# sandyresearch/chipmunk

Hardware: AMD Instinct MI355X
Metric: DiT denoise steps/sec at fixed sparsity (higher is better)
Workload: dtype bf16

## Files before the change

### chipmunk_amd/_native.py

```python
from __future__ import annotations

import ctypes
import os

_HERE = os.path.dirname(os.path.abspath(__file__))
LIB_PATH = os.environ.get("CHIPMUNK_HIP_LIB") or os.path.join(_HERE, "lib", "libchipmunk_hip.so")

SYMBOLS = [
    "chipmunk_last_error", "chipmunk_abi_version", "chipmunk_set_option", "chipmunk_set_random_seed",
    "chipmunk_csp_attn", "chipmunk_csp_attn_out", "chipmunk_csp_128_attn", "chipmunk_dense_attn", "chipmunk_dense_colsum_attn",
    "chipmunk_csp_mlp_mm1", "chipmunk_csp_mlp_mm1_scatter", "chipmunk_csp_mlp_mm1_fp8", "chipmunk_csp_mlp_mm2_and_scatter_add", "chipmunk_csp_scatter_add", "chipmunk_csp_mlp_mm2",
    "chipmunk_csp_mlp_mm1_ragged", "chipmunk_csp_mlp_mm1_scatter_ragged", "chipmunk_csp_mlp_mm1_fp8_ragged", "chipmunk_csp_mlp_mm2_ragged",
    "chipmunk_csp_mlp_mm2_and_scatter_add_ragged", "chipmunk_csp_scatter_add_ragged", "chipmunk_block_mean_ragged", "chipmunk_transpose16_pitched",
    "chipmunk_csp_mlp_mm1_batched", "chipmunk_csp_mlp_mm1_scatter_batched", "chipmunk_csp_mlp_mm1_fp8_batched", "chipmunk_csp_mlp_mm2_batched",
    "chipmunk_csp_mlp_mm2_and_scatter_add_batched", "chipmunk_csp_scatter_add_batched",
    "chipmunk_csp_mlp_mm1_glu", "chipmunk_csp_mlp_mm1_glu_batched", "chipmunk_csp_mlp_mm1_glu_fp8", "chipmunk_csp_mlp_mm1_glu_fp8_batched",
    "chipmunk_csp_mlp_mm1_act", "chipmunk_csp_mlp_mm1_act_batched", "chipmunk_csp_mlp_mm1_fp8_act", "chipmunk_csp_mlp_mm1_fp8_act_batched",
    "chipmunk_csp_mlp_mm2_w8", "chipmunk_csp_mlp_mm2_w8_batched",
    "chipmunk_csp_mlp_mm1_fp8_act_rs", "chipmunk_csp_mlp_mm1_fp8_act_rs_batched", "chipmunk_quantize_fp8_rowwise",
    "chipmunk_topk_indices", "chipmunk_topk_delta_indices", "chipmunk_topk_indices_p", "chipmunk_topk_delta_indices_p", "chipmunk_topk_mask", "chipmunk_topk_mask_p", "chipmunk_dense_colsum_topk_mask_p_strided", "chipmunk_mask_to_indices", "chipmunk_mask_to_sorted_indices", "chipmunk_packed_mask_to_indices", "chipmunk_mask_row_counts", "chipmunk_mask_to_ragged_indices", "chipmunk_copy_indices",
    "chipmunk_bitpack", "chipmunk_bitunpack", "chipmunk_transpose16", "chipmunk_block_mean", "chipmunk_quantize_fp8", "chipmunk_gather_rows", "chipmunk_qkv_split_norm", "chipmunk_split_heads_rownorm", "chipmunk_dense_colsum_topk_mask", "chipmunk_dense_attn_strided", "chipmunk_csp_attn_out_ragged", "chipmunk_compact_indices", "chipmunk_residual_ln_modulate", "chipmunk_dense_colsum_attn_strided", "chipmunk_dense_colsum_topk_mask_strided", "chipmunk_release_scratch", "chipmunk_big_scratch_fallbacks",
    "chipmunk_dense_attn_varlen", "chipmunk_dense_colsum_attn_varlen", "chipmunk_dense_colsum_topk_mask_varlen",
    "chipmunk_dense_colsum_topk_mask_p_varlen", "chipmunk_topk_mask_varlen", "chipmunk_topk_mask_p_varlen",
    "chipmunk_host_alloc", "chipmunk_host_free", "chipmunk_copy_d2h_async", "chipmunk_copy_h2d_async", "chipmunk_host_bytes",
]

_lib = None


def lib() -> ctypes.CDLL:
    global _lib
    if _lib is None:
        if not os.path.exists(LIB_PATH):
            raise ImportError(
                f"{LIB_PATH} is missing: build it with `python -m chipmunk_amd.build` (hipcc --offload-arch=gfx950). "
                "chipmunk_amd has no CPU fallback.")
        _lib = ctypes.CDLL(LIB_PATH)
        _lib.chipmunk_last_error.restype = ctypes.c_char_p
        _lib.chipmunk_abi_version.restype = ctypes.c_int
        for item in filter(None, os.environ.get("CHIPMUNK_AMD_OPTIONS", "").split(",")):
            name, _, val = item.partition("=")
            if _lib.chipmunk_set_option(name.strip().encode(), int(val)) != 0:
                raise ValueError(f"CHIPMUNK_AMD_OPTIONS: {_lib.chipmunk_last_error().decode()}")
    return _lib


def last_error() -> str:
    return lib().chipmunk_last_error().decode()


def check(rc: int, what: str) -> None:
    if rc != 0:
        raise RuntimeError(f"{what}: {last_error()}")


def set_option(name: str, value: int) -> None:
    check(lib().chipmunk_set_option(name.encode(), int(value)), "chipmunk_set_option")


def manual_seed(seed: int) -> None:
    check(lib().chipmunk_set_random_seed(ctypes.c_uint64(int(seed) & 0xFFFFFFFFFFFFFFFF)), "chipmunk_set_random_seed")


class HostBuffer:

    def __init__(self, numel: int, dtype) -> None:
        import torch
        self.dtype = dtype
        self._numel = int(numel)
        self._itemsize = torch.empty(0, dtype=dtype).element_size()
        self.nbytes = self._numel * self._itemsize
        p = ctypes.c_void_p()
        check(lib().chipmunk_host_alloc(ctypes.c_size_t(max(self.nbytes, 1)), ctypes.byref(p)), "chipmunk_host_alloc")
        self.ptr = p.value

    def numel(self) -> int:
# ... 35 lines not shown
```

### chipmunk_amd/csrc/attn.hip

```cpp
#include "common.h"
#include "attn_params.h"
#include <type_traits>

namespace {

constexpr int QG = 192;
constexpr int QW = 48;
constexpr int KVT = 32;
constexpr int NST = 4;
constexpr int KRING = 8;
constexpr int HD = 128;
constexpr int TILE_BYTES = KVT * HD * 2;
constexpr float SCALE_LOG2E = 0.08838834764f * 1.44269504089f;
constexpr int NSTV = NST + 1;
constexpr int KEY_RING_OFF = (NST + NSTV) * TILE_BYTES;
constexpr int CS_OFF = KEY_RING_OFF + KRING * 256;
constexpr int ATTN_LDS_BYTES = CS_OFF + 2 * 2 * 4 * KVT * 4;

__device__ __forceinline__ f32x4 mfma16(bf16x8 a, bf16x8 b, f32x4 c) {
    return __builtin_amdgcn_mfma_f32_16x16x32_bf16(a, b, c, 0, 0, 0);
}

#ifdef ATTN_PROF
__device__ unsigned long long g_attn_prof[8 * 8];
// ... 1197 lines not shown
                for (int b = 0; b < B; ++b)
                    for (int h0 = 0; h0 < H; h0 += hc) {
                        AttnParams c = p;
                        const int hn = H - h0 < hc ? H - h0 : hc;
                        const int64_t bh0 = (int64_t)b * H + h0;
                        c.q += b * p.qs[0] + h0 * p.qs[1], c.k += b * p.ks[0] + h0 * p.ks[1], c.v += b * p.vs[0] + h0 * p.vs[1];
                        c.o += b * p.os[0] + h0 * p.os[1];
                        c.l_out += bh0 * Nq, c.p_in += bh0 * Nq, c.cs += bh0 * p.G * (int64_t)cs_stride;
                        c.B = 1, c.H = hn;
                        if (c.klens) c.klens += b;
                        if (int e = chipmunk_dense64_colsum_launch(c, part, st)) return e;
                    }
                return CHIPMUNK_OK;
            }
        }
        rc = chipmunk_dense64_launch(q, k, v, o, l, p.qs, p.ks, p.vs, p.os, B, H, Nq, Nk, st, klens);
    } else {
        rc = launch_attn<false, false, true>(p, st);
    }
    if (rc != CHIPMUNK_OK) return rc;
    if (use_colsum64(B, H, Nq, Nk)) return chipmunk_colsum64_launch(p, st);
    return launch_attn<false, false, false, true>(p, st);
}

extern "C" int chipmunk_dense_colsum_attn_strided(const void *q, const void *k, const void *v, const int64_t q_strides[3],
                                                  const int64_t k_strides[3], const int64_t v_strides[3], const float *pin,
                                                  void *o, const int64_t *o_strides, void *cs, float *l, int B, int H, int Nq,
                                                  int Nk, int cs_stride, void *stream) {
    return dense_colsum_attn_impl(q, k, v, q_strides, k_strides, v_strides, pin, o, o_strides, cs, l, nullptr, B, H, Nq, Nk, cs_stride,
                                  stream);
}

extern "C" int chipmunk_dense_colsum_attn_varlen(const void *q, const void *k, const void *v, const int64_t q_strides[3],
                                                 const int64_t k_strides[3], const int64_t v_strides[3], const float *pin,
                                                 void *o, const int64_t *o_strides, void *cs, float *l, const int32_t *k_lens, int B,
                                                 int H, int Nq, int Nk, int cs_stride, void *stream) {
    return dense_colsum_attn_impl(q, k, v, q_strides, k_strides, v_strides, pin, o, o_strides, cs, l, k_lens, B, H, Nq, Nk, cs_stride,
                                  stream);
}

extern "C" int chipmunk_dense_colsum_attn(const void *q, const void *k, const void *v, const int64_t q_strides[3],
                                          const int64_t k_strides[3], const int64_t v_strides[3], const float *pin,
                                          void *o, void *cs, float *l, int B, int H, int Nq, int Nk, int cs_stride,
                                          void *stream) {
    return chipmunk_dense_colsum_attn_strided(q, k, v, q_strides, k_strides, v_strides, pin, o, nullptr, cs, l, B, H, Nq, Nk,
                                              cs_stride, stream);
}

static int dense_colsum_topk_mask_impl(const void *q, const void *k, const void *v, const int64_t q_strides[3],
                                       const int64_t k_strides[3], const int64_t v_strides[3], const float *pin, void *o,
                                       const int64_t *o_strides, float *l, int B, int H, int Nq, int Nk, const void *static_mask,
                                       int64_t static_stride, int static_rows, const void *group_flags, void *mask,
                                       int topk, double random_amount, bool mass, double top_p, int k_min, void *stream,
                                       const int32_t *klens = nullptr) {
    if (int e = check_common(q, k, v, o, B, H, Nq, Nk)) return e;
    CM_CHECK(l && pin && mask, "dense_colsum_topk_mask: p / l / mask missing");
    if (int e = check_strides(q_strides, "q")) return e;
    if (int e = check_strides(k_strides, "k")) return e;
    if (int e = check_strides(v_strides, "v")) return e;
    hipStream_t st = (hipStream_t)stream;
    if (!use_dense64(B, H, Nq, Nk) || chipmunk_get_option("attn_fused_colsum") == 2 || (Nk & 3) || Nk > CHIPMUNK_TOPK_MASK_MAX_N)
        return CHIPMUNK_ERR_UNSUPPORTED;
    AttnParams p = {};
    p.q = (const uint16_t *)q, p.k = (const uint16_t *)k, p.v = (const uint16_t *)v, p.o = (uint16_t *)o;
    for (int i = 0; i < 3; ++i) p.qs[i] = q_strides[i], p.ks[i] = k_strides[i], p.vs[i] = v_strides[i];
    CM_CHECK((int64_t)Nk * p.ks[2] * 2 < (1ll << 32) && (int64_t)Nk * p.vs[2] * 2 < (1ll << 32),
             "attention: one head's K or V spans more than 4 GiB (32-bit DMA offsets)");
    if (int e = output_strides(p.os, o_strides, H, Nq)) return e;
    p.l_out = l, p.p_in = pin, p.cs = nullptr, p.cs_stride = 0, p.klens = klens;
    p.B = B, p.H = H, p.Nq = Nq, p.Nk = Nk, p.G = (Nq + QG - 1) / QG;
    p.o_scale = 1.f;
    uint16_t *part = (uint16_t *)chipmunk_big_scratch(st, chipmunk_colsum_part_bytes(B, H, Nq, Nk));
    if (!part) return CHIPMUNK_ERR_UNSUPPORTED;
    if (int e = chipmunk_dense64_colsum_launch(p, part, st)) return e;
    const int nrb = ((Nq + 255) / 256) * 2;
    if (mass)
        return chipmunk_topk_mask_p_parts(part, chipmunk_colsum_part_stride(Nk), nrb, p.G, Nq, static_mask, static_stride, static_rows, group_flags, mask,
                                          B * H * p.G, Nk, topk, top_p, k_min, random_amount, st, klens, H * p.G);
    return chipmunk_topk_mask_parts(part, chipmunk_colsum_part_stride(Nk), nrb, p.G, Nq, static_mask, static_stride, static_rows, group_flags, mask, B * H * p.G, Nk,
                                    topk, random_amount, st, klens, H * p.G);
}

extern "C" int chipmunk_dense_colsum_topk_mask_strided(const void *q, const void *k, const void *v, const int64_t q_strides[3],
                                               const int64_t k_strides[3], const int64_t v_strides[3], const float *pin, void *o,
                                               const int64_t *o_strides, float *l, int B, int H, int Nq, int Nk, const void *static_mask,
                                               int64_t static_stride, int static_rows, const void *group_flags, void *mask,
                                               int topk, double random_amount, void *stream) {
    return dense_colsum_topk_mask_impl(q, k, v, q_strides, k_strides, v_strides, pin, o, o_strides, l, B, H, Nq, Nk, static_mask, static_stride,
                                       static_rows, group_flags, mask, topk, random_amount, false, 0.0, 0, stream);
}

extern "C" int chipmunk_dense_colsum_topk_mask_p_strided(const void *q, const void *k, const void *v, const int64_t q_strides[3],
                                                 const int64_t k_strides[3], const int64_t v_strides[3], const float *pin, void *o,
                                                 const int64_t *o_strides, float *l, int B, int H, int Nq, int Nk, const void *static_mask,
                                                 int64_t static_stride, int static_rows, const void *group_flags, void *mask,
                                                 int topk, double random_amount, double top_p, int k_min, void *stream) {
    CM_CHECK(top_p > 0.0 && top_p <= 1.0, "dense_colsum_topk_mask_p: top_p must be in (0, 1] (got %g)", top_p);
    CM_CHECK(k_min >= 0, "dense_colsum_topk_mask_p: k_min must be >= 0 (got %d)", k_min);
    return dense_colsum_topk_mask_impl(q, k, v, q_strides, k_strides, v_strides, pin, o, o_strides, l, B, H, Nq, Nk, static_mask, static_stride,
                                       static_rows, group_flags, mask, topk, random_amount, true, top_p, k_min, stream);
}

extern "C" int chipmunk_dense_colsum_topk_mask(const void *q, const void *k, const void *v, const int64_t q_strides[3],
                                               const int64_t k_strides[3], const int64_t v_strides[3], const float *pin, void *o,
                                               float *l, int B, int H, int Nq, int Nk, const void *static_mask,
                                               int64_t static_stride, int static_rows, const void *group_flags, void *mask,
                                               int topk, double random_amount, void *stream) {
    return chipmunk_dense_colsum_topk_mask_strided(q, k, v, q_strides, k_strides, v_strides, pin, o, nullptr, l, B, H, Nq, Nk,
                                                   static_mask, static_stride, static_rows, group_flags, mask, topk, random_amount,
                                                   stream);
}

extern "C" int chipmunk_dense_colsum_topk_mask_varlen(const void *q, const void *k, const void *v, const int64_t q_strides[3],
                                                      const int64_t k_strides[3], const int64_t v_strides[3], const float *pin, void *o,
                                                      const int64_t *o_strides, float *l, const int32_t *k_lens, int B, int H, int Nq,
                                                      int Nk, const void *static_mask, int64_t static_stride, int static_rows,
                                                      const void *group_flags, void *mask, int topk, double random_amount, void *stream) {
    return dense_colsum_topk_mask_impl(q, k, v, q_strides, k_strides, v_strides, pin, o, o_strides, l, B, H, Nq, Nk, static_mask, static_stride,
                                       static_rows, group_flags, mask, topk, random_amount, false, 0.0, 0, stream, k_lens);
}

extern "C" int chipmunk_dense_colsum_topk_mask_p_varlen(const void *q, const void *k, const void *v, const int64_t q_strides[3],
                                                        const int64_t k_strides[3], const int64_t v_strides[3], const float *pin, void *o,
                                                        const int64_t *o_strides, float *l, const int32_t *k_lens, int B, int H, int Nq,
                                                        int Nk, const void *static_mask, int64_t static_stride, int static_rows,
                                                        const void *group_flags, void *mask, int topk, double random_amount, double top_p,
                                                        int k_min, void *stream) {
    CM_CHECK(top_p > 0.0 && top_p <= 1.0, "dense_colsum_topk_mask_p: top_p must be in (0, 1] (got %g)", top_p);
    CM_CHECK(k_min >= 0, "dense_colsum_topk_mask_p: k_min must be >= 0 (got %d)", k_min);
    return dense_colsum_topk_mask_impl(q, k, v, q_strides, k_strides, v_strides, pin, o, o_strides, l, B, H, Nq, Nk, static_mask, static_stride,
                                       static_rows, group_flags, mask, topk, random_amount, true, top_p, k_min, stream, k_lens);
}
```

### chipmunk_amd/csrc/attn_params.h

```cpp
#pragma once
#include <stdint.h>
#include <hip/hip_runtime.h>

struct AttnParams {
    const uint16_t *q, *k, *v;
    uint16_t *o;
    const uint16_t *o_in;
    int64_t qs[3], ks[3], vs[3], os[3];
    const int32_t *indices, *counts;
    const int64_t *idx_off;
    float *l_out;
    const float *p_in;
    uint16_t *cs;
    int cs_stride;
    int B, H, Nq, Nk, G, idx_stride;
    float o_scale;
    int split_full, nsplit;
    float *ws;
    int32_t *tickets;
    const int32_t *plan;
    int xcd_chunks;
    const float *kmax;
    uint16_t *cs_part;
    int cs_pstride;
    int probe;
    const int32_t *klens;
};

__device__ __forceinline__ int item_nk(const int32_t *klens, int b, int Nk) {
    if (!klens) return Nk;
    const int n = klens[b];
    return n < 1 ? 1 : (n < Nk ? n : Nk);
}


int chipmunk_csp64_launch(const AttnParams &p, int inplace, int grid, hipStream_t stream);
int chipmunk_dense64_colsum_launch(const AttnParams &p, uint16_t *part, hipStream_t stream);
int chipmunk_topk_mask_parts(const uint16_t *part, int part_stride, int nrb, int groups_per_bh, int Nq, const void *static_mask, int64_t static_stride,
                             int static_rows, const void *group_flags, void *mask, int rows, int n, int k, double random_amount,
                             hipStream_t stream, const int32_t *klens = nullptr, int seq_rows = 0);
int chipmunk_topk_mask_p_parts(const uint16_t *part, int part_stride, int nrb, int groups_per_bh, int Nq, const void *static_mask, int64_t static_stride,
                               int static_rows, const void *group_flags, void *mask, int rows, int n, int k, double top_p, int k_min,
                               double random_amount, hipStream_t stream, const int32_t *klens = nullptr, int seq_rows = 0);
size_t chipmunk_colsum_part_bytes(int B, int H, int Nq, int Nk);
int chipmunk_colsum_part_stride(int Nk);
int chipmunk_colsum64_launch(const AttnParams &p, hipStream_t stream);
int chipmunk_csp96_launch(const AttnParams &p, int inplace, int grid, hipStream_t stream);
const float *chipmunk_knorm_max(const uint16_t *k, const int64_t ks[3], int B, int H, int Nk, hipStream_t stream, const int32_t *klens = nullptr);

__host__ __device__ inline int colsum_part_rows(int j, int nwg, int &r0, int &r1) {
    const int a = (3 * j) >> 2, w0 = 3 * j - 4 * a;
    r0 = 2 * a + (w0 ? 1 : 0);
    r1 = 2 * (a + 1);
    return (w0 >= 2 && a + 1 < nwg) ? 2 : 1;
}

struct IndexRow {
    const int32_t *ptr;
    int width;
};
__device__ __forceinline__ IndexRow index_row(const AttnParams &p, int64_t item) {
    if (p.idx_off) {
        const int64_t o = p.idx_off[item];
        return {p.indices + o, (int)(p.idx_off[item + 1] - o)};
    }
    return {p.indices + item * p.idx_stride, p.idx_stride};
}
```

### chipmunk_amd/csrc/common.h

```cpp
#pragma once
#include <hip/hip_runtime.h>
#include <stdint.h>
#include <stdio.h>
#include <stdarg.h>

#include "../../include/chipmunk_hip.h"

typedef __attribute__((ext_vector_type(8))) __bf16 bf16x8;
typedef __attribute__((ext_vector_type(4))) __bf16 bf16x4;
typedef __attribute__((ext_vector_type(2))) __bf16 bf16x2;
typedef __attribute__((ext_vector_type(4))) short s16x4;
typedef __attribute__((ext_vector_type(2))) float f32x2;
typedef __attribute__((ext_vector_type(4))) float f32x4;
typedef __attribute__((ext_vector_type(16))) float f32x16;
typedef __attribute__((ext_vector_type(4))) uint32_t u32x4;
typedef __attribute__((ext_vector_type(2))) uint32_t u32x2;

#define LDS_PTR(p) ((__attribute__((address_space(3))) void *)(p))
#define GLB_PTR(p) ((const __attribute__((address_space(1))) void *)(p))

__device__ __forceinline__ void glds16(const void *gsrc, void *lds_wave_base) {
    __builtin_amdgcn_global_load_lds(GLB_PTR(gsrc), LDS_PTR(lds_wave_base), 16, 0, 0);
}

// ... 54 lines not shown

__device__ __forceinline__ void lane_swap32(float &a, float &b) {
    asm volatile("s_nop 1\n\tv_permlane32_swap_b32 %0, %1" : "+v"(a), "+v"(b));
}
__device__ __forceinline__ void lane_swap16(float &a, float &b) {
    asm volatile("s_nop 1\n\tv_permlane16_swap_b32 %0, %1" : "+v"(a), "+v"(b));
}
__device__ __forceinline__ float max_across_rows(float x) {
    float a = x, b = x;
    lane_swap32(a, b);
    float c = fmaxf(a, b), d = c;
    lane_swap16(c, d);
    return fmaxf(c, d);
}
__device__ __forceinline__ float sum_across_rows(float x) {
    float a = x, b = x;
    lane_swap32(a, b);
    float c = a + b, d = c;
    lane_swap16(c, d);
    return c + d;
}

__device__ __forceinline__ int xcd_remap(int bid, int nblocks) {
    const int NX = 8;
    int xcd = bid % NX, slot = bid / NX;
    int q = nblocks / NX, r = nblocks % NX;
    int base = xcd < r ? xcd * (q + 1) : r * (q + 1) + (xcd - r) * q;
    return base + slot;
}

inline int device_cu_count() {
    static int n = 0;
    if (n == 0) {
        int dev = 0, v = 0;
        if (hipGetDevice(&dev) == hipSuccess &&
            hipDeviceGetAttribute(&v, hipDeviceAttributeMultiprocessorCount, dev) == hipSuccess && v > 0)
            n = v;
        else
            n = 256;
    }
    return n;
}

inline void ensure_dynamic_lds(const void *kernel, int bytes, uint64_t &done) {
    int dev = 0;
    if (hipGetDevice(&dev) != hipSuccess || dev < 0 || dev > 63) dev = 0;
    if (!(done >> dev & 1)) {
        (void)hipFuncSetAttribute(kernel, hipFuncAttributeMaxDynamicSharedMemorySize, bytes);
        done |= uint64_t(1) << dev;
    }
}

#define CHIPMUNK_TOPK_MASK_MAX_N (1024 * 512)

void chipmunk_set_error(const char *fmt, ...);
int chipmunk_get_option(const char *name);
uint32_t chipmunk_next_random_salt();
void *chipmunk_scratch(hipStream_t stream, size_t bytes);
void *chipmunk_big_scratch(hipStream_t stream, size_t bytes);
int chipmunk_dense64_launch(const void *q, const void *k, const void *v, void *o, float *l, const int64_t qs[3],
                            const int64_t ks[3], const int64_t vs[3], const int64_t os[3], int B, int H, int Nq, int Nk,
                            hipStream_t stream, const int32_t *klens = nullptr);
#define CM_CHECK(cond, ...)                    \
    do {                                       \
        if (!(cond)) {                         \
            chipmunk_set_error(__VA_ARGS__);   \
            return CHIPMUNK_ERR_INVALID;       \
        }                                      \
    } while (0)
#define CM_LAUNCH_CHECK()                                                          \
    do {                                                                           \
        hipError_t e__ = hipGetLastError();                                        \
        if (e__ != hipSuccess) {                                                   \
            chipmunk_set_error("HIP launch failed: %s", hipGetErrorString(e__));   \
            return CHIPMUNK_ERR_LAUNCH;                                            \
        }                                                                          \
    } while (0)
```

### chipmunk_amd/csrc/indexed_io.hip

```cpp
#include "common.h"
#include "attn_params.h"

namespace {

__device__ __forceinline__ uint32_t wave_incl_scan(uint32_t x) {
    x += (uint32_t)__builtin_amdgcn_update_dpp(0, (int)x, 0x111, 0xf, 0xf, true);
    x += (uint32_t)__builtin_amdgcn_update_dpp(0, (int)x, 0x112, 0xf, 0xf, true);
    x += (uint32_t)__builtin_amdgcn_update_dpp(0, (int)x, 0x114, 0xf, 0xf, true);
    x += (uint32_t)__builtin_amdgcn_update_dpp(0, (int)x, 0x118, 0xf, 0xf, true);
    x += (uint32_t)__builtin_amdgcn_update_dpp(0, (int)x, 0x142, 0xa, 0xf, false);
    x += (uint32_t)__builtin_amdgcn_update_dpp(0, (int)x, 0x143, 0xc, 0xf, false);
    return x;
}
struct M2IParams {
    const uint8_t *mask;
    int32_t *indices;
    int32_t *counts;
    int n, pad_n, multiple_of;
    const int64_t *offsets;
};

template <bool PACKED, bool SORTED = false, bool RAGGED = false>
__global__ __launch_bounds__(256) void mask_to_indices_kernel(const M2IParams p) {
    extern __shared__ __attribute__((aligned(16))) unsigned char smem[];
// ... 170 lines not shown
        for (int i = 0; i < NI && pos < padded; ++i) {
            uint32_t z = ~bits[i];
            const int rem = n - i * 32;
            if (rem < 32) z &= (1u << rem) - 1u;
            while (z && pos < padded) {
                const int bit = __builtin_ctz(z);
                z &= z - 1;
                put(pos++, i * 32 + bit);
            }
        }
        if constexpr (!RAGGED) p.counts[row] = padded;
    }
}

struct RowCountParams {
    const uint8_t *mask;
    int32_t *counts;
    int64_t *lengths;
    int64_t rows;
    int n, pad_n, multiple_of;
};

template <bool PACKED>
__global__ __launch_bounds__(256) void mask_row_counts_kernel(const RowCountParams p) {
    const int lane = threadIdx.x & 63;
    const int64_t row = (int64_t)blockIdx.x * 4 + (threadIdx.x >> 6);
    if (row >= p.rows) return;
    const int nbytes = PACKED ? p.n >> 3 : p.n;
    const uint8_t *src = p.mask + (PACKED ? (row * p.n) >> 3 : row * p.n);
    auto set_in_byte = [](uint32_t b) { return PACKED ? (uint32_t)__popc(b) : (uint32_t)(b != 0); };
    auto set_in_word = [](uint32_t x) {
        if constexpr (!PACKED) x = (x | (x >> 1) | (x >> 2) | (x >> 3) | (x >> 4) | (x >> 5) | (x >> 6) | (x >> 7)) & 0x01010101u;
        return (uint32_t)__popc(x);
    };
    const int head = min(nbytes, (int)((16 - ((uintptr_t)src & 15)) & 15));
    uint32_t cnt = lane < head ? set_in_byte(src[lane]) : 0u;
    const int nvec = (nbytes - head) >> 4;
    const u32x4 *vec = (const u32x4 *)(src + head);
#pragma unroll 4
    for (int i = lane; i < nvec; i += 64) {
        const u32x4 x = vec[i];
        cnt += set_in_word(x[0]) + set_in_word(x[1]) + set_in_word(x[2]) + set_in_word(x[3]);
    }
    const int tail = head + (nvec << 4) + lane;
    if (tail < nbytes) cnt += set_in_byte(src[tail]);
    const int64_t kept = (uint32_t)__builtin_amdgcn_readlane((int)wave_incl_scan(cnt), 63);
    if (lane == 0) {
        const int64_t padded = ((kept + p.multiple_of - 1) / p.multiple_of) * p.multiple_of;
        p.counts[row] = (int32_t)padded;
        p.lengths[row] = (min(padded, (int64_t)p.pad_n) + 31) / 32 * 32;
    }
}

struct TopkParams {
    const void *act;
    void *cache;
    int32_t *indices;
    int32_t *counts;
    int rows, cols, multiple_of;
    float quantile, random_amount;
    uint32_t salt;
};

template <typename T>
__device__ __forceinline__ float load_as_float(const T *p, int i);
template <>
__device__ __forceinline__ float load_as_float<uint16_t>(const uint16_t *p, int i) { return bf16_bits_to_f32(p[i]); }
template <>
__device__ __forceinline__ float load_as_float<_Float16>(const _Float16 *p, int i) { return (float)p[i]; }
template <>
__device__ __forceinline__ float load_as_float<float>(const float *p, int i) { return p[i]; }

template <typename T>
__device__ __forceinline__ float round_to(float x);
template <>
__device__ __forceinline__ float round_to<uint16_t>(float x) { return round_bf16(x); }
template <>
__device__ __forceinline__ float round_to<_Float16>(float x) { return (float)(_Float16)x; }
template <>
__device__ __forceinline__ float round_to<float>(float x) { return x; }

__device__ __forceinline__ float hash_uniform(uint32_t row, uint32_t col, uint32_t salt) {
    uint32_t x = (row * 0x9E3779B9u ^ (col + 0x7F4A7C15u) * 0x85EBCA6Bu) + salt * 0xC2B2AE35u;
    x ^= x >> 16, x *= 0x7feb352du, x ^= x >> 15, x *= 0x846ca68bu, x ^= x >> 16;
    return (float)(x >> 8) * (1.0f / 16777216.0f);
}

__device__ __forceinline__ int compact_slot(bool keep, int lane, int w, uint32_t *wave_tot, int &base) {
    const unsigned long long bal = __ballot(keep);
    const int before = __popcll(bal & ((1ull << lane) - 1ull));
    if (lane == 0) wave_tot[w] = __popcll(bal);
    __syncthreads();
    int off = base, tot = 0;
#pragma unroll
    for (int i = 0; i < 16; ++i) {
        const int c = wave_tot[i];
        off += i < w ? c : 0;
        tot += c;
    }
    __syncthreads();
    base += tot;
    return keep ? off + before : -1;
}

struct TopkPParams : TopkParams {
    float top_p;
// ... 281 lines not shown
    c = c < idx_stride ? c : (int)idx_stride;
    if ((((uintptr_t)src | (uintptr_t)dst) & 15) == 0) {
        const int c4 = c >> 2;
        for (int i = threadIdx.x; i < c4; i += 256) ((u32x4 *)dst)[i] = ((const u32x4 *)src)[i];
        for (int i = (c4 << 2) + threadIdx.x; i < c; i += 256) dst[i] = src[i];
    } else {
        for (int i = threadIdx.x; i < c; i += 256) dst[i] = src[i];
    }
    for (int i = c + threadIdx.x; i < width; i += 256) dst[i] = 0;
}

size_t m2i_lds_bytes(int n, bool sorted) {
    const int NI = (n + 31) >> 5, NB = (NI + 63) >> 6;
    if (sorted) return (size_t)NB * 64 * 4 + (size_t)(NB + 1) * 4 + 16;
    return (size_t)NB * 64 * 4 + (size_t)32 * NB * 8 + (size_t)32 * NB * 4 + 33 * 4 + 16;
}

template <bool PACKED, bool SORTED = false, bool RAGGED = false>
int launch_m2i(const void *mask, int32_t *indices, int32_t *counts, int64_t rows, int n, int pad_n, int multiple_of,
               void *stream, const int64_t *offsets = nullptr) {
    CM_CHECK(mask && indices && (RAGGED ? (const void *)offsets : (const void *)counts), "mask_to_indices: null pointer");
    CM_CHECK(rows >= 0 && n > 0 && pad_n >= n && multiple_of > 0, "mask_to_indices: bad sizes rows=%lld n=%d pad_n=%d multiple_of=%d",
             (long long)rows, n, pad_n, multiple_of);
    CM_CHECK(rows < (1ll << 31), "mask_to_indices: too many rows");
    if (PACKED) CM_CHECK(n % 8 == 0, "packed_mask_to_indices: n must be a multiple of 8 (got %d)", n);
    const size_t lds = m2i_lds_bytes(n, SORTED);
    CM_CHECK(lds <= 160 * 1024, "mask_to_indices: row length %d needs %zu B of LDS (> 160 KiB)", n, lds);
    if (rows == 0) return CHIPMUNK_OK;
    auto kern = mask_to_indices_kernel<PACKED, SORTED, RAGGED>;
    if (lds > 64 * 1024) (void)hipFuncSetAttribute((const void *)kern, hipFuncAttributeMaxDynamicSharedMemorySize, (int)lds);
    M2IParams p = {(const uint8_t *)mask, indices, counts, n, pad_n, multiple_of, offsets};
    hipLaunchKernelGGL(kern, dim3((unsigned)rows), dim3(256), lds, (hipStream_t)stream, p);
    CM_LAUNCH_CHECK();
    return CHIPMUNK_OK;
}


struct TopkMaskParams {
    const uint16_t *cs;
    const uint8_t *stat;
    const uint8_t *groups;
    uint8_t *mask;
    int64_t cs_stride, stat_stride;
    int rows, n, k, stat_rows;
    float random_amount;
    uint32_t salt;
    const uint16_t *parts;
    int64_t pstride;
    int nrb, ngroups, nq;
    float top_p;
    int k_min;
    const int32_t *klens;
    int seq_rows;
};

__device__ __forceinline__ int topk_mask_row_len(const TopkMaskParams &p, int row) {
    if (!p.klens) return p.n;
    const int v = p.klens[row / p.seq_rows];
    return v < 1 ? 1 : (v < p.n ? v : p.n);
}
struct RowCut {
    int tid, step;
    uint32_t keep0, keep1;
};
__device__ __forceinline__ RowCut row_cut(int nv) {
    const int rem = nv & 3;
    RowCut c;
    c.tid = rem ? ((nv - 1) >> 2) & 1023 : -1;
    c.step = (nv - 1) >> 12;
    c.keep0 = rem == 1 ? 0xffffu : 0xffffffffu;
    c.keep1 = rem == 3 ? 0xffffu : (rem ? 0u : 0xffffffffu);
    return c;
}

__device__ __forceinline__ float key_value(uint32_t key) { return __uint_as_float((key ^ 0x8000u) << 16); }
__device__ __forceinline__ void add_mass2(float &m, uint32_t kw, float flo) {
    const uint32_t kx = kw ^ 0x80008000u;
    const float a = __uint_as_float(kx << 16), b = __uint_as_float(kx & 0xffff0000u);
    m += a >= flo ? a : 0.f;
    m += b >= flo ? b : 0.f;
}

__device__ __forceinline__ int topp_count(float total, float target, float above, int gt, int eq, uint32_t thr, int k, int k_min) {
    int kp = 0;
    if (total > 0.f && target > 0.f) {
        const float v = key_value(thr);
        float t = __builtin_ceilf((target - above) / v);
        t = t >= 1.f ? t : 1.f;
        kp = gt + (t < (float)eq ? (int)t : eq);
    }
    const int s = kp > k_min ? kp : k_min;
    return s < k ? s : k;
}

__device__ __forceinline__ uint32_t bf16_key(uint32_t u) {
    return (u & 0x8000u) ? (~u & 0xffffu) : (u | 0x8000u);
}

template <int KPT, bool ALIGNED, bool PARTS = false, bool MASS = false>
__global__ __launch_bounds__(1024) void topk_mask_kernel(const TopkMaskParams p) {
    constexpr int NV = KPT / 4;
    __shared__ int wave_cnt[16];
    const int tid = threadIdx.x, lane = tid & 63, w = tid >> 6;
    const int row = blockIdx.x;
    const int n = p.n;
    const int nv = topk_mask_row_len(p, row);
    const uint16_t *x = nullptr;
    int prow = 1;
    int64_t row1 = 0;
    if constexpr (PARTS) {
        const int bh = row / p.ngroups, g = row - bh * p.ngroups;
        int r0, r1;
        prow = colsum_part_rows(g, p.nrb / 2, r0, r1);
        x = p.parts + ((int64_t)bh * p.nrb + r0) * p.pstride;
        row1 = (int64_t)(r1 - r0) * p.pstride;
    } else {
        x = p.cs + (int64_t)row * p.cs_stride;
    }
    const uint32_t lane_off8 = 8u * (uint32_t)tid;
    const uint32_t lane_off4 = 4u * (uint32_t)tid;
    uint32_t key[NV][2];
    constexpr int LB = NV % 10 == 0 ? 10 : (NV % 8 == 0 ? 8 : (NV % 6 == 0 ? 6 : 4));
    static_assert(NV % LB == 0, "NV must split into whole load batches");
#pragma unroll
    for (int j0 = 0; j0 < NV; j0 += LB) {
        uint32_t raw[LB][2];
#pragma unroll
        for (int jj = 0; jj < LB; ++jj) {
            const int c = 4 * tid + 4096 * (j0 + jj);
            uint32_t v0 = 0xffffffffu, v1 = 0xffffffffu;
            if constexpr (ALIGNED) {
                if (c < nv) {
                    const u32x2 v = *(const u32x2 *)((const unsigned char *)(x + 4096 * (j0 + jj)) + lane_off8);
                    v0 = v[0], v1 = v[1];
                    if constexpr (PARTS) {
                        if (prow == 2) {
                            float a0 = __uint_as_float(v0 << 16), a1 = __uint_as_float(v0 & 0xffff0000u);
                            float a2 = __uint_as_float(v1 << 16), a3 = __uint_as_float(v1 & 0xffff0000u);
                            const u32x2 y = *(const u32x2 *)((const unsigned char *)(x + row1 + 4096 * (j0 + jj)) + lane_off8);
                            a0 += __uint_as_float(y[0] << 16), a1 += __uint_as_float(y[0] & 0xffff0000u);
                            a2 += __uint_as_float(y[1] << 16), a3 += __uint_as_float(y[1] & 0xffff0000u);
                            v0 = pack_bf16x2(a0, a1), v1 = pack_bf16x2(a2, a3);
                        }
                    }
                }
            } else if (c < nv) {
                v0 = v1 = 0;
#pragma unroll
                for (int e = 0; e < 4; ++e) {
                    const uint32_t u = c + e < nv ? x[c + e] : 0xffffu;
                    if (e < 2) v0 |= u << (16 * e);
                    else v1 |= u << (16 * (e - 2));
                }
// ... 127 lines not shown
    }
    int my_ties = 0;
    if (ties_to_take > 0) {
#pragma unroll
        for (int j = 0; j < NV; ++j)
#pragma unroll
            for (int h = 0; h < 2; ++h) {
                uint32_t kw = key[j][h];
                asm volatile("" : "+v"(kw));
                my_ties += ((kw & 0xffffu) == thr ? 1 : 0) + ((kw >> 16) == thr ? 1 : 0);
            }
    }
    int tie_budget = 0;
    {
        int incl = my_ties;
#pragma unroll
        for (int d = 1; d < 64; d <<= 1) {
            const int o = __shfl_up(incl, d);
            if (lane >= d) incl += o;
        }
        if (lane == 63) wave_cnt[w] = incl;
        __syncthreads();
        int before = incl - my_ties;
#pragma unroll
        for (int i = 0; i < 16; ++i) before += i < w ? wave_cnt[i] : 0;
        __syncthreads();
        tie_budget = ties_to_take - before;
    }
    uint8_t *out = p.mask + (int64_t)row * n;
    const uint8_t *st = p.stat ? p.stat + (int64_t)(row % p.stat_rows) * p.stat_stride : nullptr;
    const bool rnd = active && p.random_amount > 0.f;
    auto combined4 = [&](int c0, uint32_t &v0, uint32_t &v1) {
        const u32x2 v = *(const u32x2 *)(x + c0);
        v0 = v[0], v1 = v[1];
        if constexpr (PARTS) {
            float a0 = __uint_as_float(v0 << 16), a1 = __uint_as_float(v0 & 0xffff0000u);
            float a2 = __uint_as_float(v1 << 16), a3 = __uint_as_float(v1 & 0xffff0000u);
            if (prow == 2) {
                const u32x2 y = *(const u32x2 *)(x + row1 + c0);
                a0 += __uint_as_float(y[0] << 16), a1 += __uint_as_float(y[0] & 0xffff0000u);
                a2 += __uint_as_float(y[1] << 16), a3 += __uint_as_float(y[1] & 0xffff0000u);
            }
            v0 = pack_bf16x2(a0, a1), v1 = pack_bf16x2(a2, a3);
        }
    };
    uint32_t first = x[0];
    if constexpr (PARTS) {
        uint32_t f0, f1;
        combined4(0, f0, f1);
        first = f0 & 0xffffu;
    }
    const uint32_t salt = p.salt ^ (first * 0x27D4EB2Fu);
    const int nsteps = (n + 4095) / 4096;
    auto emit = [&](auto keyed, int c, uint32_t v0, uint32_t v1, uint32_t sb) {
        uint32_t bytes = 0;
        if constexpr (decltype(keyed)::value) asm volatile("" : "+v"(v0), "+v"(v1));
#pragma unroll
        for (int e = 0; e < 4; ++e) {
            const uint32_t half = ((e < 2 ? v0 : v1) >> (16 * (e & 1))) & 0xffffu;
            const uint32_t kv = decltype(keyed)::value ? half : bf16_key(half);
            bool keep = kv > thr;
            const bool tie = kv == thr && tie_budget > 0 && c + e < nv;
            tie_budget -= tie ? 1 : 0;
            keep = keep || tie;
            if (rnd && !keep) keep = hash_uniform(row, c + e, salt) < p.random_amount;
            keep = keep || ((sb >> (8 * e)) & 0xffu) != 0;
            keep = keep && c + e < nv;
            bytes |= (keep ? 1u : 0u) << (8 * e);
        }
        if constexpr (ALIGNED) {
            *(uint32_t *)(out + c) = bytes;
        } else {
#pragma unroll
            for (int e = 0; e < 4; ++e)
                if (c + e < n) out[c + e] = (uint8_t)(bytes >> (8 * e));
        }
    };
    if constexpr (ALIGNED) {
        constexpr int OB = 5;
#pragma unroll
        for (int j0 = 0; j0 < NV; j0 += OB) {
            uint32_t sbv[OB];
#pragma unroll
            for (int jj = 0; jj < OB; ++jj) {
                const int c = 4 * tid + 4096 * (j0 + jj);
                sbv[jj] = (j0 + jj < NV && st && c < n) ? *(const uint32_t *)(st + c) : 0u;
            }
            __builtin_amdgcn_sched_barrier(0);
#pragma unroll
            for (int jj = 0; jj < OB; ++jj) {
                if constexpr (true) {
                    const int c = 4 * tid + 4096 * (j0 + jj);
                    if (j0 + jj < NV && c < n) emit(std::integral_constant<int, 1>{}, c, key[(j0 + jj) < NV ? (j0 + jj) : 0][0], key[(j0 + jj) < NV ? (j0 + jj) : 0][1], sbv[jj]);
                    asm volatile("" ::: "memory");
                }
            }
            __builtin_amdgcn_sched_barrier(0);
        }
    } else {
        for (int j = 0; j < nsteps; ++j) {
            const int c = 4 * tid + 4096 * j;
            if (c >= n) break;
            uint32_t v0 = 0, v1 = 0, sb = 0;
#pragma unroll
            for (int e = 0; e < 4; ++e) {
                const uint32_t u = c + e < nv ? x[c + e] : 0xffffu;
                if (e < 2) v0 |= u << (16 * e);
                else v1 |= u << (16 * (e - 2));
                if (st && c + e < n) sb |= (uint32_t)st[c + e] << (8 * e);
            }
            emit(std::integral_constant<int, 0>{}, c, v0, v1, sb);
        }
    }
}

__device__ __forceinline__ uint32_t bf16_key2(uint32_t u) {
    uint32_t s;
    const uint32_t fifteen2 = 0x000f000fu;
    asm("v_pk_ashrrev_i16 %0, %1, %2" : "=v"(s) : "v"(fifteen2), "v"(u));
    return u ^ (s | 0x80008000u);
}

template <bool ALIGNED, bool PARTS, bool MASS = false>
__global__ __launch_bounds__(1024) void topk_mask_stream_kernel(const TopkMaskParams p) {
    __shared__ int wave_cnt[16];
    const int tid = threadIdx.x, lane = tid & 63, w = tid >> 6;
    const int row = blockIdx.x;
    const int n = p.n;
    const int nv = topk_mask_row_len(p, row);
    const uint16_t *x = nullptr;
    int prow = 1;
    int64_t row1 = 0;
    if constexpr (PARTS) {
        const int bh = row / p.ngroups, g = row - bh * p.ngroups;
        int r0, r1;
        prow = colsum_part_rows(g, p.nrb / 2, r0, r1);
        x = p.parts + ((int64_t)bh * p.nrb + r0) * p.pstride;
        row1 = (int64_t)(r1 - r0) * p.pstride;
    } else {
        x = p.cs + (int64_t)row * p.cs_stride;
    }
    const uint32_t lane_off8 = 8u * (uint32_t)tid;
    const int nsteps = (n + 4095) / 4096;
    const bool active = p.groups == nullptr || p.groups[row] != 0;
    int k = p.k < nv ? p.k : nv;
    const RowCut rc = row_cut(nv);
    const int cut_step = ALIGNED && tid == rc.tid ? rc.step : -1;
    bool select = active && k > 0;
    const bool rnd = active && p.random_amount > 0.f;

    auto combined4 = [&](int c0, uint32_t &v0, uint32_t &v1) {
        const u32x2 v = *(const u32x2 *)(x + c0);
        v0 = v[0], v1 = v[1];
        if constexpr (PARTS) {
            if (prow == 2) {
                float a0 = __uint_as_float(v0 << 16), a1 = __uint_as_float(v0 & 0xffff0000u);
                float a2 = __uint_as_float(v1 << 16), a3 = __uint_as_float(v1 & 0xffff0000u);
                const u32x2 y = *(const u32x2 *)(x + row1 + c0);
                a0 += __uint_as_float(y[0] << 16), a1 += __uint_as_float(y[0] & 0xffff0000u);
                a2 += __uint_as_float(y[1] << 16), a3 += __uint_as_float(y[1] & 0xffff0000u);
                v0 = pack_bf16x2(a0, a1), v1 = pack_bf16x2(a2, a3);
            }
        }
    };
    uint32_t first = 0;
// ... 268 lines not shown
    CM_CHECK(sparsity_amount >= 0.0 && sparsity_amount <= 1.0, "%s: sparsity_amount must be in [0,1]", who);
    CM_CHECK(top_p > 0.0 && top_p <= 1.0, "%s: top_p must be in (0, 1] (got %g)", who, top_p);
    CM_CHECK(min_keys >= 0.0 && min_keys <= 1.0 - sparsity_amount + 1e-9, "%s: min_keys must be in [0, 1 - sparsity_amount] (got %g with sparsity_amount %g)",
             who, min_keys, sparsity_amount);
    if (rows == 0) return CHIPMUNK_OK;
    TopkPParams p;
    p.act = activation, p.cache = cache, p.indices = indices, p.counts = counts;
    p.rows = rows, p.cols = cols, p.multiple_of = multiple_of;
    p.quantile = (float)sparsity_amount, p.random_amount = (float)random_amount;
    p.salt = random_amount > 0.0 ? chipmunk_next_random_salt() : 0u;
    p.top_p = (float)top_p;
    p.k_min = min_keys == 0.0 ? 1024 : std::max((int)(1024 * (float)(1.0 - min_keys)), (int)(1024 * p.quantile));
    hipStream_t s = (hipStream_t)stream;
#define LAUNCH_TOPK_P(T)                                                                                         \
    do {                                                                                                         \
        if (cache) hipLaunchKernelGGL((topk_indices_kernel<T, true, true>), dim3(rows), dim3(1024), 0, s, p);    \
        else hipLaunchKernelGGL((topk_indices_kernel<T, false, true>), dim3(rows), dim3(1024), 0, s, p);         \
    } while (0)
    switch (dtype) {
        case CHIPMUNK_DTYPE_BF16: LAUNCH_TOPK_P(uint16_t); break;
        case CHIPMUNK_DTYPE_FP16: LAUNCH_TOPK_P(_Float16); break;
        case CHIPMUNK_DTYPE_FP32: LAUNCH_TOPK_P(float); break;
        default: CM_CHECK(false, "%s: unsupported dtype code %d", who, dtype);
    }
#undef LAUNCH_TOPK_P
    CM_LAUNCH_CHECK();
    return CHIPMUNK_OK;
}

extern "C" int chipmunk_mask_to_sorted_indices(const void *mask, int packed, int32_t *indices, int32_t *counts,
                                               int64_t rows, int n, int pad_n, int multiple_of, void *stream) {
    return packed ? launch_m2i<true, true>(mask, indices, counts, rows, n, pad_n, multiple_of, stream)
                  : launch_m2i<false, true>(mask, indices, counts, rows, n, pad_n, multiple_of, stream);
}

extern "C" int chipmunk_mask_row_counts(const void *mask, int packed, int32_t *counts, int64_t *lengths, int64_t rows, int n,
                                        int pad_n, int multiple_of, void *stream) {
    CM_CHECK(mask && counts && lengths, "mask_row_counts: null pointer");
    CM_CHECK(rows >= 0 && n > 0 && pad_n >= n && multiple_of > 0, "mask_row_counts: bad sizes rows=%lld n=%d pad_n=%d multiple_of=%d",
             (long long)rows, n, pad_n, multiple_of);
    CM_CHECK(rows < (1ll << 31), "mask_row_counts: too many rows");
    CM_CHECK(!packed || n % 8 == 0, "mask_row_counts: n must be a multiple of 8 for a packed mask (got %d)", n);
    const size_t lds = m2i_lds_bytes(n, true);
    CM_CHECK(lds <= 160 * 1024, "mask_to_indices: row length %d needs %zu B of LDS (> 160 KiB)", n, lds);
    if (rows == 0) return CHIPMUNK_OK;
    RowCountParams p = {(const uint8_t *)mask, counts, lengths, rows, n, pad_n, multiple_of};
    const dim3 grid((unsigned)((rows + 3) / 4));
    if (packed) hipLaunchKernelGGL(mask_row_counts_kernel<true>, grid, dim3(256), 0, (hipStream_t)stream, p);
    else hipLaunchKernelGGL(mask_row_counts_kernel<false>, grid, dim3(256), 0, (hipStream_t)stream, p);
    CM_LAUNCH_CHECK();
    return CHIPMUNK_OK;
}

extern "C" int chipmunk_mask_to_ragged_indices(const void *mask, int packed, int sorted, const int64_t *offsets, int32_t *flat,
                                               int64_t rows, int n, int multiple_of, void *stream) {
    if (packed) return sorted ? launch_m2i<true, true, true>(mask, flat, nullptr, rows, n, n, multiple_of, stream, offsets)
                              : launch_m2i<true, false, true>(mask, flat, nullptr, rows, n, n, multiple_of, stream, offsets);
    return sorted ? launch_m2i<false, true, true>(mask, flat, nullptr, rows, n, n, multiple_of, stream, offsets)
                  : launch_m2i<false, false, true>(mask, flat, nullptr, rows, n, n, multiple_of, stream, offsets);
}

extern "C" int chipmunk_topk_indices(const void *activation, int dtype, int32_t *indices, int32_t *counts, int rows,
                                     int cols, double sparsity_amount, int multiple_of, double random_amount,
                                     void *stream) {
    return launch_topk(activation, nullptr, dtype, indices, counts, rows, cols, sparsity_amount, multiple_of,
                       random_amount, stream);
}

extern "C" int chipmunk_topk_delta_indices(const void *activation, void *cache, int dtype, int32_t *indices,
                                           int32_t *counts, int rows, int cols, double sparsity_amount,
                                           int multiple_of, double random_amount, void *stream) {
    CM_CHECK(cache != nullptr, "topk_delta_indices: cache missing");
    return launch_topk(activation, cache, dtype, indices, counts, rows, cols, sparsity_amount, multiple_of,
                       random_amount, stream);
}

extern "C" int chipmunk_topk_indices_p(const void *activation, int dtype, int32_t *indices, int32_t *counts, int rows, int cols,
                                       double sparsity_amount, double top_p, double min_keys, int multiple_of,
                                       double random_amount, void *stream) {
    return launch_topk_p("topk_indices_p", activation, nullptr, dtype, indices, counts, rows, cols, sparsity_amount, top_p, min_keys,
                         multiple_of, random_amount, stream);
}

extern "C" int chipmunk_topk_delta_indices_p(const void *activation, void *cache, int dtype, int32_t *indices, int32_t *counts,
                                             int rows, int cols, double sparsity_amount, double top_p, double min_keys,
                                             int multiple_of, double random_amount, void *stream) {
    CM_CHECK(cache != nullptr, "topk_delta_indices_p: cache missing");
    return launch_topk_p("topk_delta_indices_p", activation, cache, dtype, indices, counts, rows, cols, sparsity_amount, top_p,
                         min_keys, multiple_of, random_amount, stream);
}

extern "C" int chipmunk_copy_indices(const void *src, void *dst, const int32_t *inds, const int32_t *counts, int B,
                                     int M, int R, int F, int elem_size, void *stream) {
    CM_CHECK(src && dst && inds && counts, "copy_indices: null pointer");
    CM_CHECK(B >= 0 && M > 0 && R > 0 && F > 0, "copy_indices: bad sizes");
    CM_CHECK(elem_size == 2 || elem_size == 4, "copy_indices: element size must be 2 or 4 bytes (got %d)", elem_size);
    const int64_t rows = (int64_t)B * M * R;
    if (rows == 0) return CHIPMUNK_OK;
    CM_CHECK(rows < (1ll << 31), "copy_indices: too many rows");
    hipStream_t s = (hipStream_t)stream;
    if (elem_size == 2)
        hipLaunchKernelGGL(copy_indices_kernel<uint16_t>, dim3((unsigned)rows), dim3(256), 0, s, (const uint16_t *)src,
                           (uint16_t *)dst, inds, counts, M, R, F);
    else
        hipLaunchKernelGGL(copy_indices_kernel<uint32_t>, dim3((unsigned)rows), dim3(256), 0, s, (const uint32_t *)src,
                           (uint32_t *)dst, inds, counts, M, R, F);
// ... 61 lines not shown
#define LAUNCH_GATHER(V)                                                                                              \
    do {                                                                                                              \
        const int64_t cpr = row_bytes / (int64_t)sizeof(V), total = outer * n_out * cpr;                               \
        const int64_t blocks = (total + 255) / 256;                                                                    \
        hipLaunchKernelGGL((gather_rows_kernel<V>), dim3((unsigned)(blocks > 65536 * 16 ? 65536 * 16 : blocks)),       \
                           dim3(256), 0, s, (const V *)src, (V *)dst, map, n_out, n_src, cpr, total);                  \
    } while (0)
    if ((align & 15) == 0) LAUNCH_GATHER(u32x4);
    else if ((align & 3) == 0) LAUNCH_GATHER(uint32_t);
    else if ((align & 1) == 0) LAUNCH_GATHER(uint16_t);
    else LAUNCH_GATHER(uint8_t);
#undef LAUNCH_GATHER
    CM_LAUNCH_CHECK();
    return CHIPMUNK_OK;
}

template <bool MASS>
static int topk_mask_parts_impl(const uint16_t *part, int part_stride, int nrb, int groups_per_bh, int Nq, const void *static_mask, int64_t static_stride,
                                int static_rows, const void *group_flags, void *mask, int rows, int n, int k, double random_amount,
                                double top_p, int k_min, hipStream_t s, const int32_t *klens, int seq_rows) {
    CM_CHECK(!klens || seq_rows > 0, "topk_mask_parts: k_lens without the rows per sequence");
    CM_CHECK(part && mask && rows >= 0 && n > 0 && (n & 3) == 0 && n <= CHIPMUNK_TOPK_MASK_MAX_N && k >= 0 && part_stride >= n && (part_stride & 3) == 0, "topk_mask_parts: bad arguments");
    CM_CHECK(!static_mask || (static_rows > 0 && static_stride >= n && (static_stride & 3) == 0 && ((uintptr_t)static_mask & 3) == 0),
             "topk_mask_parts: bad static mask geometry");
    CM_CHECK(((uintptr_t)mask & 3) == 0 && ((uintptr_t)part & 7) == 0, "topk_mask_parts: unaligned buffers");
    if (rows == 0) return CHIPMUNK_OK;
    TopkMaskParams p = {nullptr, (const uint8_t *)static_mask, (const uint8_t *)group_flags, (uint8_t *)mask, 0, static_stride,
                        rows, n, k, static_mask ? static_rows : 1, (float)random_amount,
                        random_amount > 0.0 ? chipmunk_next_random_salt() : 0u};
    p.parts = part, p.pstride = part_stride, p.nrb = nrb, p.ngroups = groups_per_bh, p.nq = Nq;
    p.top_p = (float)top_p, p.k_min = k_min;
    p.klens = klens, p.seq_rows = seq_rows;
    if (n > 1024 * 120 || chipmunk_get_option("topk_mask_stream") == 1) hipLaunchKernelGGL((topk_mask_stream_kernel<true, true, MASS>), dim3(rows), dim3(1024), 0, s, p);
    else if (n <= 1024 * 16) hipLaunchKernelGGL((topk_mask_kernel<16, true, true, MASS>), dim3(rows), dim3(1024), 0, s, p);
    else if (n <= 1024 * 48) hipLaunchKernelGGL((topk_mask_kernel<48, true, true, MASS>), dim3(rows), dim3(1024), 0, s, p);
    else hipLaunchKernelGGL((topk_mask_kernel<120, true, true, MASS>), dim3(rows), dim3(1024), 0, s, p);
    CM_LAUNCH_CHECK();
    return CHIPMUNK_OK;
}

int chipmunk_topk_mask_parts(const uint16_t *part, int part_stride, int nrb, int groups_per_bh, int Nq, const void *static_mask, int64_t static_stride,
                             int static_rows, const void *group_flags, void *mask, int rows, int n, int k, double random_amount,
                             hipStream_t s, const int32_t *klens, int seq_rows) {
    return topk_mask_parts_impl<false>(part, part_stride, nrb, groups_per_bh, Nq, static_mask, static_stride, static_rows, group_flags, mask, rows, n, k,
                                       random_amount, 0.0, 0, s, klens, seq_rows);
}

int chipmunk_topk_mask_p_parts(const uint16_t *part, int part_stride, int nrb, int groups_per_bh, int Nq, const void *static_mask, int64_t static_stride,
                               int static_rows, const void *group_flags, void *mask, int rows, int n, int k, double top_p, int k_min,
                               double random_amount, hipStream_t s, const int32_t *klens, int seq_rows) {
    CM_CHECK(top_p > 0.0 && top_p <= 1.0 && k_min >= 0, "topk_mask_p_parts: top_p must be in (0, 1] and k_min >= 0 (got %g, %d)", top_p, k_min);
    return topk_mask_parts_impl<true>(part, part_stride, nrb, groups_per_bh, Nq, static_mask, static_stride, static_rows, group_flags, mask, rows, n, k,
                                      random_amount, top_p, k_min, s, klens, seq_rows);
}

__global__ __launch_bounds__(256) void qkv_split_norm_kernel(const uint16_t *qkv, int64_t row_stride, const uint16_t *qw,
                                                             const uint16_t *kw, uint16_t *q, uint16_t *k, uint16_t *v, int64_t n,
                                                             int H, float eps, int64_t segments, const float *fcos, const float *fsin,
                                                             int64_t rope_rows) {
    const int l15 = threadIdx.x & 15;
    u32x4 wq = {0x3f803f80u, 0x3f803f80u, 0x3f803f80u, 0x3f803f80u}, wk = wq;
    if (qw) wq = *(const u32x4 *)(qw + l15 * 8);
    if (kw) wk = *(const u32x4 *)(kw + l15 * 8);
    for (int64_t seg = ((int64_t)blockIdx.x * 256 + threadIdx.x) >> 4; seg < segments; seg += ((int64_t)gridDim.x * 256) >> 4) {
        const int64_t tok = seg / (3 * H);
        const int rem = (int)(seg - tok * 3 * H), which = rem / H, h = rem - which * H;
        u32x4 x = *(const u32x4 *)(qkv + tok * row_stride + (int64_t)rem * 128 + l15 * 8);
        uint16_t *dst = (which == 0 ? q : which == 1 ? k : v) + ((int64_t)h * n + tok) * 128 + l15 * 8;
        if (which < 2) {
            float f[8], ss = 0.f;
#pragma unroll
            for (int e = 0; e < 4; ++e) {
                f[2 * e] = __uint_as_float(x[e] << 16), f[2 * e + 1] = __uint_as_float(x[e] & 0xffff0000u);
                ss = __builtin_fmaf(f[2 * e], f[2 * e], ss);
                ss = __builtin_fmaf(f[2 * e + 1], f[2 * e + 1], ss);
            }
            ss = row16_sum(ss);
            const float r = 1.0f / __builtin_sqrtf(ss * (1.0f / 128.0f) + eps);
            const u32x4 w = which == 0 ? wq : wk;
#pragma unroll
            for (int e = 0; e < 4; ++e) {
                float a = f[2 * e] * r, b = f[2 * e + 1] * r;
                round_bf16_pair(a, b);
                x[e] = pack_bf16x2(a * __uint_as_float(w[e] << 16), b * __uint_as_float(w[e] & 0xffff0000u));
            }
            if (fcos && tok < rope_rows) {
                const f32x4 c0 = *(const f32x4 *)(fcos + tok * 128 + l15 * 8), c1 = *(const f32x4 *)(fcos + tok * 128 + l15 * 8 + 4);
                const f32x4 s0 = *(const f32x4 *)(fsin + tok * 128 + l15 * 8), s1 = *(const f32x4 *)(fsin + tok * 128 + l15 * 8 + 4);
#pragma unroll
                for (int e = 0; e < 4; ++e) {
                    const float re = __uint_as_float(x[e] << 16), im = __uint_as_float(x[e] & 0xffff0000u);
                    const float cr = e < 2 ? c0[2 * e] : c1[2 * e - 4], ci = e < 2 ? c0[2 * e + 1] : c1[2 * e - 3];
                    const float sr = e < 2 ? s0[2 * e] : s1[2 * e - 4], si = e < 2 ? s0[2 * e + 1] : s1[2 * e - 3];
                    x[e] = pack_bf16x2(re * cr + (-im) * sr, im * ci + re * si);
                }
            }
        }
        *(u32x4 *)dst = x;
    }
}

extern "C" int chipmunk_qkv_split_norm(const void *qkv, int64_t row_stride, const void *q_weight, const void *k_weight, void *q,
                                       void *k, void *v, int64_t n, int heads, float eps, const float *freqs_cos,
                                       const float *freqs_sin, int64_t rope_rows, void *stream) {
    CM_CHECK(qkv && q && k && v, "qkv_split_norm: null pointer");
    CM_CHECK(n >= 0 && heads > 0 && row_stride >= (int64_t)3 * heads * 128, "qkv_split_norm: bad sizes");
// ... 26 lines not shown
                        cs_stride, static_stride, rows, n, k, static_mask ? static_rows : 1, (float)random_amount,
                        random_amount > 0.0 ? chipmunk_next_random_salt() : 0u};
    p.top_p = (float)top_p, p.k_min = k_min;
    p.klens = klens, p.seq_rows = seq_rows;
    hipStream_t s = (hipStream_t)stream;
    const bool aligned = n % 4 == 0 && (((uintptr_t)cs) & 7) == 0 && (cs_stride * 2) % 8 == 0 && (((uintptr_t)mask) & 3) == 0 &&
                         (!static_mask || ((((uintptr_t)static_mask) & 3) == 0 && static_stride % 4 == 0));
#define LAUNCH_TM(KPT)                                                                                       \
    do {                                                                                                     \
        if (aligned) hipLaunchKernelGGL((topk_mask_kernel<KPT, true, false, MASS>), dim3(rows), dim3(1024), 0, s, p);     \
        else hipLaunchKernelGGL((topk_mask_kernel<KPT, false, false, MASS>), dim3(rows), dim3(1024), 0, s, p);            \
    } while (0)
    if (n > 1024 * 120 || chipmunk_get_option("topk_mask_stream") == 1) {
        if (aligned) hipLaunchKernelGGL((topk_mask_stream_kernel<true, false, MASS>), dim3(rows), dim3(1024), 0, s, p);
        else hipLaunchKernelGGL((topk_mask_stream_kernel<false, false, MASS>), dim3(rows), dim3(1024), 0, s, p);
    } else if (n <= 1024 * 16) LAUNCH_TM(16);
    else if (n <= 1024 * 48) LAUNCH_TM(48);
    else LAUNCH_TM(120);
#undef LAUNCH_TM
    CM_LAUNCH_CHECK();
    return CHIPMUNK_OK;
}

extern "C" int chipmunk_topk_mask(const void *cs, int64_t cs_stride, const void *static_mask, int64_t static_stride,
                                  int static_rows, const void *group_flags, void *mask, int rows, int n, int k,
                                  double random_amount, void *stream) {
    return topk_mask_impl<false>(cs, cs_stride, static_mask, static_stride, static_rows, group_flags, mask, rows, n, k, random_amount, 0.0, 0, stream);
}

extern "C" int chipmunk_topk_mask_p(const void *cs, int64_t cs_stride, const void *static_mask, int64_t static_stride,
                                    int static_rows, const void *group_flags, void *mask, int rows, int n, int k,
                                    double random_amount, double top_p, int k_min, void *stream) {
    CM_CHECK(top_p > 0.0 && top_p <= 1.0, "topk_mask_p: top_p must be in (0, 1] (got %g)", top_p);
    CM_CHECK(k_min >= 0, "topk_mask_p: k_min must be >= 0 (got %d)", k_min);
    return topk_mask_impl<true>(cs, cs_stride, static_mask, static_stride, static_rows, group_flags, mask, rows, n, k, random_amount, top_p, k_min, stream);
}

extern "C" int chipmunk_topk_mask_varlen(const void *cs, int64_t cs_stride, const void *static_mask, int64_t static_stride,
                                         int static_rows, const void *group_flags, void *mask, const int32_t *k_lens, int seq_rows, int rows,
                                         int n, int k, double random_amount, void *stream) {
    return topk_mask_impl<false>(cs, cs_stride, static_mask, static_stride, static_rows, group_flags, mask, rows, n, k, random_amount, 0.0, 0, stream,
                                 k_lens, seq_rows);
}

extern "C" int chipmunk_topk_mask_p_varlen(const void *cs, int64_t cs_stride, const void *static_mask, int64_t static_stride,
                                           int static_rows, const void *group_flags, void *mask, const int32_t *k_lens, int seq_rows, int rows,
                                           int n, int k, double random_amount, double top_p, int k_min, void *stream) {
    CM_CHECK(top_p > 0.0 && top_p <= 1.0, "topk_mask_p: top_p must be in (0, 1] (got %g)", top_p);
    CM_CHECK(k_min >= 0, "topk_mask_p: k_min must be >= 0 (got %d)", k_min);
    return topk_mask_impl<true>(cs, cs_stride, static_mask, static_stride, static_rows, group_flags, mask, rows, n, k, random_amount, top_p, k_min,
                                stream, k_lens, seq_rows);
}

extern "C" int chipmunk_compact_indices(const int32_t *indices, int64_t idx_stride, const int32_t *counts, const int64_t *offsets,
                                        int32_t *flat, int64_t rows, void *stream) {
    CM_CHECK(indices && counts && offsets && flat, "compact_indices: null pointer");
    CM_CHECK(rows >= 0 && rows < (1ll << 31) && idx_stride > 0, "compact_indices: bad sizes rows=%lld idx_stride=%lld", (long long)rows,
             (long long)idx_stride);
    if (rows == 0) return CHIPMUNK_OK;
    hipLaunchKernelGGL(compact_indices_kernel, dim3((unsigned)rows), dim3(256), 0, (hipStream_t)stream, indices, idx_stride, counts,
                       offsets, flat);
    CM_LAUNCH_CHECK();
    return CHIPMUNK_OK;
}
```

### chipmunk_amd/csrc/torch_registry.cpp

```cpp
#include <ATen/ATen.h>
#include <ATen/hip/impl/HIPStreamMasqueradingAsCUDA.h>
#include <Python.h>
#include <c10/core/DeviceGuard.h>
#include <torch/library.h>

#include <vector>

#include "../../include/chipmunk_hip.h"

extern "C" {
PyObject *PyInit_cuda(void) {
    static struct PyModuleDef module_def = {PyModuleDef_HEAD_INIT, "cuda", NULL, -1, NULL};
    return PyModule_Create(&module_def);
}
}

namespace chipmunk {
namespace {

void *cur_stream(const at::Tensor &t) {
    return (void *)c10::hip::getCurrentHIPStreamMasqueradingAsCUDA(t.device().index()).stream();
}
void check(int rc, const char *op) { TORCH_CHECK(rc == 0, "chipmunk::", op, ": ", chipmunk_last_error()); }

// ... 836 lines not shown
            check(chipmunk_block_mean_ragged(x[b].data_ptr(), out[b].data_ptr(), n, (int)x.size(2), (int)mbm, cur_stream(x)), "block_mean");
    }
    return out;
}

at::Tensor quantize_fp8(at::Tensor x, at::Tensor scale, double max_value) {
    CHECK_DEV(x); CHECK_DEV(scale);
    TORCH_CHECK(x.scalar_type() == at::kBFloat16, "quantize_fp8: x must be bfloat16");
    TORCH_CHECK(scale.scalar_type() == at::kFloat && scale.numel() == 1, "quantize_fp8: scale must be a one-element float32 tensor");
    TORCH_CHECK(x.numel() % 8 == 0, "quantize_fp8: the element count must be a multiple of 8");
    x = x.contiguous();
    c10::DeviceGuard guard(x.device());
    at::Tensor out = at::empty(x.sizes(), x.options().dtype(at::kFloat8_e4m3fn));
    check(chipmunk_quantize_fp8(x.data_ptr(), scale.data_ptr<float>(), out.data_ptr(), x.numel(), (float)max_value, cur_stream(x)), "quantize_fp8");
    return out;
}

std::vector<at::Tensor> quantize_fp8_rowwise(at::Tensor x, double max_value) {
    CHECK_DEV(x);
    TORCH_CHECK(x.scalar_type() == at::kBFloat16, "quantize_fp8_rowwise: x must be bfloat16");
    TORCH_CHECK(x.dim() >= 1 && x.size(-1) > 0 && x.size(-1) % 16 == 0 && x.size(-1) <= CHIPMUNK_QUANTIZE_ROWWISE_MAX_K,
                "quantize_fp8_rowwise: the last dimension must be a positive multiple of 16, at most ", CHIPMUNK_QUANTIZE_ROWWISE_MAX_K);
    x = x.contiguous();
    c10::DeviceGuard guard(x.device());
    const int64_t K = x.size(-1), rows = x.numel() / K;
    at::Tensor out = at::empty(x.sizes(), x.options().dtype(at::kFloat8_e4m3fn));
    at::Tensor recip = at::empty(x.sizes().slice(0, x.dim() - 1), x.options().dtype(at::kFloat));
    check(chipmunk_quantize_fp8_rowwise(x.data_ptr(), out.data_ptr(), recip.data_ptr<float>(), rows, (int)K, (float)max_value, cur_stream(x)),
          "quantize_fp8_rowwise");
    return {out, recip};
}

std::vector<at::Tensor> mask_to_sorted_indices(at::Tensor mask, at::IntArrayRef shape, int64_t multiple_of,
                                               int64_t pad_to_multiple_of) {
    CHECK_DEV(mask);
    const bool packed = mask.scalar_type() == at::kByte;
    TORCH_CHECK(packed || mask.scalar_type() == at::kBool, "mask must be bool, or uint8 bit-packed with a shape");
    mask = mask.contiguous();
    std::vector<int64_t> shp = packed ? shape.vec() : mask.sizes().vec();
    TORCH_CHECK(shp.size() == 4, "shape must be [b, h, m, n]");
    const int64_t b = shp[0], h = shp[1], m = shp[2], n = shp[3];
    if (packed) TORCH_CHECK(n % 8 == 0 && mask.numel() * 8 >= b * h * m * n, "bad packed mask");
    const int64_t pad_n = ((n + pad_to_multiple_of - 1) / pad_to_multiple_of) * pad_to_multiple_of;
    c10::DeviceGuard guard(mask.device());
    at::Tensor indices = at::empty({b, h, m, pad_n}, mask.options().dtype(at::kInt));
    at::Tensor counts = at::empty({b, h, m}, mask.options().dtype(at::kInt));
    check(chipmunk_mask_to_sorted_indices(mask.data_ptr(), packed ? 1 : 0, indices.data_ptr<int>(),
                                          counts.data_ptr<int>(), b * h * m, (int)n, (int)pad_n, (int)multiple_of,
                                          cur_stream(mask)),
          "mask_to_sorted_indices");
    return {indices, counts};
}

std::vector<at::Tensor> mask_to_ragged_indices(at::Tensor mask, at::IntArrayRef shape, int64_t multiple_of, int64_t pad_to_multiple_of,
                                               bool sorted) {
    CHECK_DEV(mask);
    const bool packed = mask.scalar_type() == at::kByte;
    TORCH_CHECK(packed || mask.scalar_type() == at::kBool, "mask must be bool, or uint8 bit-packed with a shape");
    TORCH_CHECK(multiple_of > 0 && pad_to_multiple_of > 0, "multiple_of and pad_to_multiple_of must be positive");
    mask = mask.contiguous();
    std::vector<int64_t> shp = packed ? shape.vec() : mask.sizes().vec();
    TORCH_CHECK(shp.size() == 4, "shape must be [b, h, m, n]");
    const int64_t b = shp[0], h = shp[1], m = shp[2], n = shp[3], rows = b * h * m;
    if (packed) TORCH_CHECK(n % 8 == 0 && mask.numel() * 8 >= rows * n, "bad packed mask");
    const int64_t pad_n = ((n + pad_to_multiple_of - 1) / pad_to_multiple_of) * pad_to_multiple_of;
    TORCH_CHECK(n > 0 && pad_n <= INT_MAX, "rows must have between 1 and 2^31 - 1 columns");
    c10::DeviceGuard guard(mask.device());
    at::Tensor counts = at::empty({b, h, m}, mask.options().dtype(at::kInt));
    at::Tensor len = at::empty({rows}, mask.options().dtype(at::kLong));
    check(chipmunk_mask_row_counts(mask.data_ptr(), packed ? 1 : 0, counts.data_ptr<int>(), len.data_ptr<int64_t>(), rows, (int)n,
                                   (int)pad_n, (int)multiple_of, cur_stream(mask)),
          "mask_to_ragged_indices");
    at::Tensor offsets = at::zeros({rows + 1}, len.options());
    if (rows) offsets.narrow(0, 1, rows).copy_(len.cumsum(0));
    const int64_t total = rows ? offsets[rows].item<int64_t>() : 0;
    at::Tensor flat = at::empty({total + 64}, counts.options());
    flat.narrow(0, total, 64).zero_();
    check(chipmunk_mask_to_ragged_indices(mask.data_ptr(), packed ? 1 : 0, sorted ? 1 : 0, offsets.data_ptr<int64_t>(), flat.data_ptr<int>(),
                                          rows, (int)n, (int)multiple_of, cur_stream(mask)),
          "mask_to_ragged_indices");
    return {flat, offsets, counts};
}

std::vector<at::Tensor> dense_colsum_attn_layout(at::Tensor q, at::Tensor k, at::Tensor v, at::Tensor p, bool token_major_o);
static at::Tensor topk_mask_impl(at::Tensor cs, int64_t k, bool mass, double top_p, int64_t k_min, double random_amount,
                                 const c10::optional<at::Tensor> &groups, const c10::optional<at::Tensor> &static_mask,
                                 const OptTensor &k_lens = c10::nullopt);
static std::vector<at::Tensor> dense_colsum_topk_mask_impl(at::Tensor q, at::Tensor k, at::Tensor v, at::Tensor p, int64_t k_top, bool mass, double top_p,
                                                           int64_t k_min, double random_amount, const c10::optional<at::Tensor> &groups,
                                                           const c10::optional<at::Tensor> &static_mask, bool token_major_o,
                                                           const OptTensor &k_lens = c10::nullopt) {
    const int32_t *kl = klens_ptr(k_lens, q, q.dim() == 4 ? q.size(0) : 0);
    if (mass) TORCH_CHECK(top_p > 0.0 && top_p <= 1.0 && k_min >= 0, "top_p must be in (0, 1] and k_min >= 0 (got ", top_p, ", ", k_min, ")");
    CHECK_DEV(q); CHECK_DEV(k); CHECK_DEV(v); CHECK_DEV(p);
    CHECK_BF16(q); CHECK_BF16(k); CHECK_BF16(v);
    const bool shapes_ok = q.dim() == 4 && k.dim() == 4 && v.dim() == 4 && q.size(3) == 128 && q.stride(3) == 1 && k.stride(3) == 1 &&
                           v.stride(3) == 1 && p.scalar_type() == at::kFloat && p.is_contiguous();
    if (shapes_ok) {
        const int64_t B = q.size(0), H = q.size(1), Nq = q.size(2), Nk = k.size(2), G = (Nq + 191) / 192;
        const void *st = nullptr, *gf = nullptr;
        int64_t st_stride = 0, st_rows = 1;
        at::Tensor stc, gfc;
        bool ok = p.numel() == B * H * Nq;
        if (ok && static_mask.has_value() && static_mask->defined()) {
            stc = *static_mask;
            ok = stc.is_cuda() && stc.scalar_type() == at::kBool && stc.dim() == 4 && stc.size(3) == Nk && stc.size(2) == G && stc.size(1) == H &&
                 (stc.size(0) == 1 || stc.size(0) == B) && stc.stride(3) == 1 && stc.stride(1) == G * stc.stride(2) &&
                 (stc.size(0) == 1 || stc.stride(0) == H * stc.stride(1));
            if (ok) st = stc.data_ptr(), st_stride = stc.stride(2), st_rows = stc.size(0) * H * G;
        }
        if (ok && groups.has_value() && groups->defined()) {
            gfc = *groups;
            ok = gfc.is_cuda() && gfc.scalar_type() == at::kBool && gfc.dim() == 4 && gfc.size(3) == 1 && gfc.size(2) == G && gfc.size(1) == H &&
                 (gfc.size(0) == 1 || gfc.size(0) == B);
            if (ok) {
                gfc = gfc.expand({B, H, G, 1}).contiguous();
                gf = gfc.data_ptr();
            }
        }
        if (ok) {
            c10::DeviceGuard guard(q.device());
            at::Tensor o = alloc_o(q, q, token_major_o);
            const int64_t os[3] = {o.stride(0), o.stride(1), o.stride(2)};
            at::Tensor l = at::empty({B, H, Nq, 1}, q.options().dtype(at::kFloat));
            at::Tensor mask = at::empty({B, H, G, Nk}, q.options().dtype(at::kBool));
            const int64_t qs[3] = {q.stride(0), q.stride(1), q.stride(2)}, ks[3] = {k.stride(0), k.stride(1), k.stride(2)},
                          vs[3] = {v.stride(0), v.stride(1), v.stride(2)};
            const int rc = mass ? chipmunk_dense_colsum_topk_mask_p_varlen(q.data_ptr(), k.data_ptr(), v.data_ptr(), qs, ks, vs, p.data_ptr<float>(), o.data_ptr(),
                                                                           os, l.data_ptr<float>(), kl, (int)B, (int)H, (int)Nq, (int)Nk, st, st_stride, (int)st_rows, gf,
                                                                           mask.data_ptr(), (int)k_top, random_amount, top_p, (int)(k_min > Nk ? Nk : k_min), cur_stream(q))
                                : chipmunk_dense_colsum_topk_mask_varlen(q.data_ptr(), k.data_ptr(), v.data_ptr(), qs, ks, vs, p.data_ptr<float>(), o.data_ptr(),
                                                           os, l.data_ptr<float>(), kl, (int)B, (int)H, (int)Nq, (int)Nk, st, st_stride, (int)st_rows, gf,
                                                           mask.data_ptr(), (int)k_top, random_amount, cur_stream(q));
            if (rc == CHIPMUNK_OK) return {o, mask, l};
            if (rc != CHIPMUNK_ERR_UNSUPPORTED) check(rc, "dense_colsum_topk_mask");
        }
    }
    auto ocl = dense_colsum_attn_klens(q, k, v, p, token_major_o, k_lens);
    at::Tensor cs = ocl[1];
    const int64_t Nk = k.size(2), G = (q.size(2) + 191) / 192;
    if (cs.size(-1) != Nk || cs.size(-2) != G) cs = cs.slice(-2, 0, G).slice(-1, 0, Nk);
    return {ocl[0], topk_mask_impl(cs, k_top, mass, top_p, k_min, random_amount, groups, static_mask, k_lens), ocl[2]};
}

std::vector<at::Tensor> dense_colsum_topk_mask_varlen(at::Tensor q, at::Tensor k, at::Tensor v, at::Tensor p, at::Tensor k_lens, int64_t k_top,
                                                      double random_amount, const c10::optional<at::Tensor> &groups,
                                                      const c10::optional<at::Tensor> &static_mask, bool token_major_o) {
    return dense_colsum_topk_mask_impl(q, k, v, p, k_top, false, 0.0, 0, random_amount, groups, static_mask, token_major_o, k_lens);
}

std::vector<at::Tensor> dense_colsum_topk_mask_p_varlen(at::Tensor q, at::Tensor k, at::Tensor v, at::Tensor p, at::Tensor k_lens, int64_t k_top,
                                                        double top_p, int64_t k_min, double random_amount, const c10::optional<at::Tensor> &groups,
                                                        const c10::optional<at::Tensor> &static_mask, bool token_major_o) {
    return dense_colsum_topk_mask_impl(q, k, v, p, k_top, true, top_p, k_min, random_amount, groups, static_mask, token_major_o, k_lens);
}

std::vector<at::Tensor> dense_colsum_topk_mask(at::Tensor q, at::Tensor k, at::Tensor v, at::Tensor p, int64_t k_top, double random_amount,
                                               const c10::optional<at::Tensor> &groups, const c10::optional<at::Tensor> &static_mask,
                                               bool token_major_o) {
    return dense_colsum_topk_mask_impl(q, k, v, p, k_top, false, 0.0, 0, random_amount, groups, static_mask, token_major_o);
}

std::vector<at::Tensor> dense_colsum_topk_mask_p(at::Tensor q, at::Tensor k, at::Tensor v, at::Tensor p, int64_t k_top, double top_p, int64_t k_min,
                                                 double random_amount, const c10::optional<at::Tensor> &groups,
                                                 const c10::optional<at::Tensor> &static_mask, bool token_major_o) {
    return dense_colsum_topk_mask_impl(q, k, v, p, k_top, true, top_p, k_min, random_amount, groups, static_mask, token_major_o);
}

static at::Tensor topk_mask_impl(at::Tensor cs, int64_t k, bool mass, double top_p, int64_t k_min, double random_amount,
                                 const c10::optional<at::Tensor> &groups, const c10::optional<at::Tensor> &static_mask,
                                 const OptTensor &k_lens) {
    CHECK_DEV(cs); CHECK_BF16(cs);
    TORCH_CHECK(cs.dim() == 4 && cs.stride(3) == 1, "cs must be [B, H, G, N] with a contiguous last dim");
    const int64_t B = cs.size(0), H = cs.size(1), G = cs.size(2), N = cs.size(3);
    const int32_t *kl = klens_ptr(k_lens, cs, B);
    if (!(cs.stride(1) == G * cs.stride(2) && (B == 1 || cs.stride(0) == H * cs.stride(1)))) cs = cs.contiguous();
    const int64_t rows = B * H * G;
    c10::DeviceGuard guard(cs.device());
    at::Tensor mask = at::empty({B, H, G, N}, cs.options().dtype(at::kBool));
    const void *st = nullptr, *gf = nullptr;
    int64_t st_stride = 0, st_rows = 1;
    at::Tensor stc, gfc;
    if (static_mask.has_value() && static_mask->defined()) {
        stc = *static_mask;
        CHECK_DEV(stc);
        TORCH_CHECK(stc.scalar_type() == at::kBool && stc.dim() == 4 && stc.size(3) == N && stc.size(2) == G &&
                    stc.size(1) == H && (stc.size(0) == 1 || stc.size(0) == B), "static_mask must be bool [1|B, H, G, N]");
        if (!(stc.stride(3) == 1 && stc.stride(1) == G * stc.stride(2) && (stc.size(0) == 1 || stc.stride(0) == H * stc.stride(1))))
            stc = stc.contiguous();
        st = stc.data_ptr(), st_stride = stc.stride(2), st_rows = stc.size(0) * H * G;
    }
    if (groups.has_value() && groups->defined()) {
        gfc = *groups;
        CHECK_DEV(gfc);
        TORCH_CHECK(gfc.scalar_type() == at::kBool && gfc.dim() == 4 && gfc.size(3) == 1 && gfc.size(2) == G &&
                    gfc.size(1) == H && (gfc.size(0) == 1 || gfc.size(0) == B), "groups must be bool [1|B, H, G, 1]");
        gfc = gfc.expand({B, H, G, 1}).contiguous();
        gf = gfc.data_ptr();
    }
    if (mass)
        check(chipmunk_topk_mask_p_varlen(cs.data_ptr(), cs.stride(2), st, st_stride, (int)st_rows, gf, mask.data_ptr(), kl, (int)(H * G),
                                          (int)rows, (int)N, (int)k, random_amount, top_p, (int)(k_min > N ? N : k_min), cur_stream(cs)),
              "topk_mask_p");
    else
        check(chipmunk_topk_mask_varlen(cs.data_ptr(), cs.stride(2), st, st_stride, (int)st_rows, gf, mask.data_ptr(), kl, (int)(H * G),
                                        (int)rows, (int)N, (int)k, random_amount, cur_stream(cs)),
              "topk_mask");
    return mask;
}

at::Tensor topk_mask_varlen(at::Tensor cs, at::Tensor k_lens, int64_t k, double random_amount, const c10::optional<at::Tensor> &groups,
                            const c10::optional<at::Tensor> &static_mask) {
    return topk_mask_impl(cs, k, false, 0.0, 0, random_amount, groups, static_mask, k_lens);
}

at::Tensor topk_mask_p_varlen(at::Tensor cs, at::Tensor k_lens, int64_t k, double top_p, int64_t k_min, double random_amount,
                              const c10::optional<at::Tensor> &groups, const c10::optional<at::Tensor> &static_mask) {
    return topk_mask_impl(cs, k, true, top_p, k_min, random_amount, groups, static_mask, k_lens);
}
// ... 122 lines not shown
    at::Tensor dst = at::empty(sizes, src.options());
    if (dst.numel() == 0) return dst;
    check(chipmunk_gather_rows(src.data_ptr(), dst.data_ptr(), map.data_ptr<int>(), outer, n_src, n_out,
                               d * (int64_t)src.element_size(), cur_stream(src)),
          "gather_rows");
    return dst;
}

}

TORCH_LIBRARY(chipmunk, m) {
    m.def("csp_mlp_mm1(Tensor a, Tensor b_colmajor, Tensor(c!) c, Tensor bias, Tensor pa_cache_colmajor, Tensor indices, Tensor indices_counts) -> ()");
    m.def("csp_mlp_mm2_and_scatter_add(Tensor packed, Tensor(unpacked_colmajor!) unpacked_colmajor, Tensor sp_inds, Tensor sp_counts, Tensor mma_a, Tensor mma_b, Tensor mma_c, int num_sms_scatter_add, int matmul_kernel) -> ()");

    m.def("csp_attn(Tensor q, Tensor k, Tensor v, Tensor o, Tensor indices, Tensor indices_counts, int o_scale) -> ()");
    m.def("csp_128_attn(Tensor q, Tensor k, Tensor v, Tensor indices, Tensor indices_counts) -> Tensor");
    m.def("dense_attn(Tensor q, Tensor k, Tensor v) -> Tensor[]");
    m.def("dense_colsum_attn(Tensor q, Tensor k, Tensor v, Tensor p) -> Tensor[]");

    m.def("copy_indices(Tensor bmfc1, Tensor(bm_mid_cache!) bm_mid_cache, Tensor sp_inds, Tensor sp_counts) -> ()");
    m.def("topk_indices(Tensor activation, Tensor(indices!) indices, Tensor counts, float sparsity_amount, int multiple_of, float random_amount) -> ()");
    m.def("csp_scatter_add(Tensor packed, Tensor(unpacked_colmajor!) unpacked_colmajor, Tensor sp_inds, Tensor sp_counts, int num_sms) -> ()");
    m.def("mask_to_indices(Tensor mask, int multiple_of, int pad_to_multiple_of) -> Tensor[]");

    m.def("csp_attn_out(Tensor q, Tensor k, Tensor v, Tensor o_in, Tensor indices, Tensor indices_counts, int o_scale) -> Tensor");
    m.def("csp_mlp_mm1_scatter(Tensor a, Tensor b_colmajor, Tensor(c!) c, Tensor bias, Tensor(pa_cache_colmajor!) pa_cache_colmajor, Tensor indices, Tensor indices_counts) -> ()");
    m.def("csp_mlp_mm2(Tensor mma_a, Tensor mma_b, Tensor indices, Tensor counts, Tensor(mma_c!) mma_c) -> ()");
    m.def("csp_mlp_mm2_w8(Tensor mma_a, Tensor mma_b, Tensor scale_b, Tensor indices, Tensor counts, Tensor(mma_c!) mma_c) -> ()");
    m.def("csp_mlp_mm1_fp8(Tensor a, Tensor b, Tensor(c!) c, Tensor bias, Tensor(pa_cache_colmajor!) pa_cache_colmajor, Tensor indices, Tensor indices_counts, Tensor scale_a, Tensor scale_b, bool update_cache) -> ()");
    m.def("csp_mlp_mm1_fp8_scatter(Tensor a, Tensor b, Tensor(c!) c, Tensor bias, Tensor(pa_cache_colmajor!) pa_cache_colmajor, Tensor indices, Tensor indices_counts, Tensor scale_a, Tensor scale_b) -> ()");
    m.def("csp_mlp_mm1_glu(Tensor a, Tensor b_gate, Tensor b_up, Tensor(c!) c, Tensor? bias_gate, Tensor? bias_up, Tensor(pa_cache_colmajor!) pa_cache_colmajor, Tensor indices, Tensor indices_counts, str act, bool update_cache) -> ()");
    m.def("csp_mlp_mm1_glu_fp8(Tensor a, Tensor b_gate, Tensor b_up, Tensor(c!) c, Tensor? bias_gate, Tensor? bias_up, Tensor(pa_cache_colmajor!) pa_cache_colmajor, Tensor indices, Tensor indices_counts, Tensor scale_a, Tensor scale_b_gate, Tensor scale_b_up, str act, bool update_cache) -> ()");
    m.def("csp_mlp_mm1_act(Tensor a, Tensor b, Tensor(c!) c, Tensor? bias, Tensor(pa!) pa_cache, Tensor indices, Tensor counts, str act, bool update_cache) -> ()");
    m.def("csp_mlp_mm1_fp8_act(Tensor a, Tensor b, Tensor(c!) c, Tensor? bias, Tensor(pa!) pa_cache, Tensor indices, Tensor counts, Tensor scale_a, Tensor scale_b, str act, int update_cache) -> ()");
    m.def("topk_delta_indices(Tensor activation, Tensor(cache!) cache, Tensor(indices!) indices, Tensor(counts!) counts, float sparsity_amount, int multiple_of, float random_amount) -> ()");
    m.def("topk_indices_p(Tensor activation, Tensor(indices!) indices, Tensor(counts!) counts, float sparsity_amount, float top_p, float min_keys, int multiple_of, float random_amount) -> ()");
    m.def("topk_delta_indices_p(Tensor activation, Tensor(cache!) cache, Tensor(indices!) indices, Tensor(counts!) counts, float sparsity_amount, float top_p, float min_keys, int multiple_of, float random_amount) -> ()");
    m.def("packed_mask_to_indices(Tensor packed, int[] shape, int multiple_of, int pad_to_multiple_of) -> Tensor[]");
    m.def("mask_to_sorted_indices(Tensor mask, int[] shape, int multiple_of, int pad_to_multiple_of) -> Tensor[]");
    m.def("topk_mask(Tensor cs, int k, float random_amount, Tensor? groups, Tensor? static_mask) -> Tensor");
    m.def("dense_colsum_topk_mask(Tensor q, Tensor k, Tensor v, Tensor p, int k_top, float random_amount, Tensor? groups, Tensor? static_mask, bool token_major_o=False) -> Tensor[]");
    m.def("topk_mask_p(Tensor cs, int k, float top_p, int k_min, float random_amount, Tensor? groups, Tensor? static_mask) -> Tensor");
    m.def("dense_colsum_topk_mask_p(Tensor q, Tensor k, Tensor v, Tensor p, int k_top, float top_p, int k_min, float random_amount, Tensor? groups, Tensor? static_mask, bool token_major_o=False) -> Tensor[]");
    m.def("dense_attn_layout(Tensor q, Tensor k, Tensor v, bool token_major_o) -> Tensor[]");
    m.def("dense_colsum_attn_layout(Tensor q, Tensor k, Tensor v, Tensor p, bool token_major_o) -> Tensor[]");
    m.def("dense_attn_varlen(Tensor q, Tensor k, Tensor v, Tensor k_lens, bool token_major_o=False) -> Tensor[]");
    m.def("dense_colsum_attn_varlen(Tensor q, Tensor k, Tensor v, Tensor p, Tensor k_lens, bool token_major_o=False) -> Tensor[]");
    m.def("topk_mask_varlen(Tensor cs, Tensor k_lens, int k, float random_amount, Tensor? groups, Tensor? static_mask) -> Tensor");
    m.def("topk_mask_p_varlen(Tensor cs, Tensor k_lens, int k, float top_p, int k_min, float random_amount, Tensor? groups, Tensor? static_mask) -> Tensor");
    m.def("dense_colsum_topk_mask_varlen(Tensor q, Tensor k, Tensor v, Tensor p, Tensor k_lens, int k_top, float random_amount, Tensor? groups, Tensor? static_mask, bool token_major_o=False) -> Tensor[]");
    m.def("dense_colsum_topk_mask_p_varlen(Tensor q, Tensor k, Tensor v, Tensor p, Tensor k_lens, int k_top, float top_p, int k_min, float random_amount, Tensor? groups, Tensor? static_mask, bool token_major_o=False) -> Tensor[]");
    m.def("compact_indices(Tensor indices, Tensor counts) -> Tensor[]");
    m.def("mask_to_ragged_indices(Tensor mask, int[] shape, int multiple_of, int pad_to_multiple_of, bool sorted) -> Tensor[]");
    m.def("csp_attn_out_ragged(Tensor q, Tensor k, Tensor v, Tensor o_in, Tensor indices, Tensor offsets, Tensor indices_counts, int o_scale) -> Tensor");
    m.def("residual_ln_modulate(Tensor x, Tensor? y, Tensor? gate, Tensor shift, Tensor scale, float eps) -> Tensor[]");
    m.def("transpose_last2(Tensor x) -> Tensor");
    m.def("transpose_last2_pitched(Tensor x, int ld) -> Tensor");
    m.def("block_mean(Tensor x, int mbm) -> Tensor");
    m.def("quantize_fp8(Tensor x, Tensor scale, float max_value) -> Tensor");
    m.def("quantize_fp8_rowwise(Tensor x, float max_value) -> Tensor[]");
    m.def("csp_mlp_mm1_fp8_act_rs(Tensor a, Tensor b, Tensor(c!) c, Tensor? bias, Tensor(pa!) pa_cache, Tensor indices, Tensor counts, Tensor scale_a, Tensor scale_b, str act, int update_cache) -> ()");
    m.def("bitpack(Tensor mask) -> Tensor");
    m.def("bitunpack(Tensor packed, int[] shape) -> Tensor");
    m.def("gather_rows(Tensor src, Tensor map) -> Tensor");
    m.def("qkv_split_norm(Tensor qkv, Tensor? q_weight, Tensor? k_weight, int heads, float eps, Tensor? freqs_cos=None, Tensor? freqs_sin=None) -> Tensor[]");
    m.def("split_heads_rownorm(Tensor x, int heads, int parts, Tensor? w0, Tensor? w1, Tensor? w2, int norm_mask, int rope_mask, float eps, Tensor? freqs_cos=None, Tensor? freqs_sin=None) -> Tensor[]");
}

TORCH_LIBRARY_IMPL(chipmunk, CUDA, m) {
    m.impl("qkv_split_norm", &qkv_split_norm);
    m.impl("split_heads_rownorm", &split_heads_rownorm);
    m.impl("csp_mlp_mm1_fp8_scatter", &csp_mlp_mm1_fp8_scatter);
    m.impl("dense_colsum_topk_mask", &dense_colsum_topk_mask);
    m.impl("dense_colsum_topk_mask_p", &dense_colsum_topk_mask_p);
    m.impl("csp_mlp_mm1", &csp_mlp_mm1);
    m.impl("csp_mlp_mm2_and_scatter_add", &csp_mlp_mm2_and_scatter_add);
    m.impl("copy_indices", &copy_indices);
    m.impl("topk_indices", &topk_indices);
    m.impl("csp_scatter_add", &csp_scatter_add);
    m.impl("mask_to_indices", &mask_to_indices);
    m.impl("csp_attn", &csp_attn);
    m.impl("csp_128_attn", &csp_128_attn);
    m.impl("dense_attn", &dense_attn);
    m.impl("dense_colsum_attn", &dense_colsum_attn);
    m.impl("compact_indices", &compact_indices);
    m.impl("residual_ln_modulate", &residual_ln_modulate);
    m.impl("csp_attn_out_ragged", &csp_attn_out_ragged);
    m.impl("dense_attn_varlen", &dense_attn_varlen);
    m.impl("dense_colsum_attn_varlen", &dense_colsum_attn_varlen);
    m.impl("topk_mask_varlen", &topk_mask_varlen);
    m.impl("topk_mask_p_varlen", &topk_mask_p_varlen);
    m.impl("dense_colsum_topk_mask_varlen", &dense_colsum_topk_mask_varlen);
    m.impl("dense_colsum_topk_mask_p_varlen", &dense_colsum_topk_mask_p_varlen);
    m.impl("dense_attn_layout", &dense_attn_layout);
    m.impl("dense_colsum_attn_layout", &dense_colsum_attn_layout);
    m.impl("csp_attn_out", &csp_attn_out);
    m.impl("csp_mlp_mm1_scatter", &csp_mlp_mm1_scatter);
    m.impl("csp_mlp_mm2", &csp_mlp_mm2);
    m.impl("csp_mlp_mm2_w8", &csp_mlp_mm2_w8);
    m.impl("csp_mlp_mm1_fp8", &csp_mlp_mm1_fp8);
    m.impl("csp_mlp_mm1_glu", &csp_mlp_mm1_glu);
    m.impl("csp_mlp_mm1_glu_fp8", &csp_mlp_mm1_glu_fp8);
    m.impl("csp_mlp_mm1_act", &csp_mlp_mm1_act);
    m.impl("csp_mlp_mm1_fp8_act", &csp_mlp_mm1_fp8_act);
    m.impl("topk_delta_indices", &topk_delta_indices);
    m.impl("topk_indices_p", &topk_indices_p);
    m.impl("topk_delta_indices_p", &topk_delta_indices_p);
    m.impl("packed_mask_to_indices", &packed_mask_to_indices);
    m.impl("mask_to_sorted_indices", &mask_to_sorted_indices);
    m.impl("mask_to_ragged_indices", &mask_to_ragged_indices);
    m.impl("topk_mask", &topk_mask);
    m.impl("topk_mask_p", &topk_mask_p);
    m.impl("transpose_last2", &transpose_last2);
    m.impl("transpose_last2_pitched", &transpose_last2_pitched);
    m.impl("block_mean", &block_mean);
    m.impl("quantize_fp8", &quantize_fp8);
    m.impl("quantize_fp8_rowwise", &quantize_fp8_rowwise);
    m.impl("csp_mlp_mm1_fp8_act_rs", &csp_mlp_mm1_fp8_act_rs);
    m.impl("bitpack", &bitpack);
    m.impl("bitunpack", &bitunpack);
    m.impl("gather_rows", &gather_rows);
}

}
```

### chipmunk_amd/modules/attn.py

```python
from __future__ import annotations

from typing import Optional, Tuple

import torch
import torch.nn.functional as F
from torch import Tensor, nn

from .. import ops
from ..ops.voxel import get_local_indices_with_text
from ..util.config import GLOBAL_CONFIG, amd_key
from ..util.layer_counter import LayerCounter
from ..util.storage import AttnStorage
from ..util.storage.offloaded_tensor import release_kept_offloaded, release_resident, reserve_kept_offloaded, reserve_resident

singleton_static_mask: Optional[Tensor] = None
singleton_video_query_groups: Optional[Tensor] = None


def _cdiv(a: int, b: int) -> int:
    return (a + b - 1) // b


def _dense_attn_raw(q: Tensor, k: Tensor, v: Tensor, token_major_o: bool, k_lens: Optional[Tensor] = None):
    if k_lens is not None:
# ... 93 lines not shown
        if kept[4]:
            release_kept_offloaded(kept[3])

    def __del__(self):
        try:
            self.release_kept_indices()
        except Exception:
            pass

    @torch.compiler.disable
    def _remember_indices(self, inds: Optional[Tensor], counts: Tensor, ragged=None) -> None:
        inv = self.layer_counter.cur_model_invocation_per_step
        old, self._unpacked[inv] = self._unpacked[inv], None
        if old is not None:
            self._release_kept(old)
        self.storage.indices.suppress_current(False)
        if not (counts.is_cuda and amd_key("attn", "keep_unpacked_indices") and amd_key("attn", "fused_residual")
                and (self.storage.indices.is_resident() or amd_key("attn", "keep_unpacked_indices_offloaded"))):
            return
        if not reserve_resident(0):
            return
        flat, offsets = ragged if ragged is not None else ops.compact_indices(inds, counts)
        nbytes = 4 * flat.numel() + 8 * offsets.numel() + 4 * counts.numel()
        off_mode = not self.storage.indices.is_resident()
        if off_mode and not reserve_kept_offloaded(nbytes):
            return
        if not reserve_resident(nbytes):
            if off_mode:
                release_kept_offloaded(nbytes)
            return
        self._unpacked[inv] = (flat, offsets, counts, nbytes, off_mode)
        self.storage.indices.suppress_current(off_mode and bool(GLOBAL_CONFIG["attn"]["recompute_mask"]))

    def _kept_indices(self):
        kept = self._unpacked[self.layer_counter.cur_model_invocation_per_step]
        if kept is not None and GLOBAL_CONFIG["attn"]["should_compress_indices"] and (
                self.storage.indices.is_resident() or amd_key("attn", "keep_unpacked_indices_offloaded")):
            return kept[:3]
        return None

    def _stored_mask(self):
        if self.storage.indices.is_suppressed():
            self.storage.indices.suppress_current(False)
            self.storage.indices.load_async()
            self.storage.indices.load_async_wait()
        return self.storage.get_indices(), self.mask_shape[self.layer_counter.cur_model_invocation_per_step]

    @staticmethod
    def _ragged_enabled(x: Tensor) -> bool:
        return bool(x.is_cuda and GLOBAL_CONFIG["attn"]["should_compress_indices"] and amd_key("attn", "fused_residual")
                    and amd_key("attn", "fused_packed_mask_to_indices") and amd_key("attn", "ragged_mask_to_indices"))

    @torch.compiler.disable
    def _ragged_indices(self, packed: Tensor, shape, multiple_of: int, bm: int, mask: Optional[Tensor] = None):
        if shape[-1] % 8 != 0:
            packed = mask if mask is not None else ops.bitunpack(packed, shape)
        return ops.mask_to_ragged_indices(packed, shape, multiple_of, bm, bool(amd_key("attn", "sorted_indices")))

    def _stored_indices(self, multiple_of: int, bm: int):
        cfg = GLOBAL_CONFIG["attn"]
        if cfg["should_compress_indices"]:
            packed, shape = self._stored_mask()
            if amd_key("attn", "fused_packed_mask_to_indices") and packed.is_cuda and shape[-1] % 8 == 0:
                if amd_key("attn", "sorted_indices"):
                    return ops.mask_to_sorted_indices(packed, shape, multiple_of, bm)
                return ops.packed_mask_to_indices(packed, shape, multiple_of, bm)
            return ops.mask_to_indices(ops.bitunpack(packed, shape), multiple_of, bm)
        return self.storage.get_indices(), self.storage.get_counts()

    def _fast_attention(self, q: Tensor, k: Tensor, v: Tensor, inference_step: int, do_full_step: bool,
                        k_lens: Optional[Tensor] = None) -> Tensor:
        cfg = GLOBAL_CONFIG["attn"]
        bm = cfg["mbm"]
        assert bm == 192, "The kernel was written for BM=192. You may need to change the kernel."
        do_padding = cfg["pad_qkv_before_kernel"]
        multiple_of = 128 if do_padding else cfg["counts_multiple_of"]

        tm = bool(q.is_cuda and amd_key("attn", "token_major_output"))
        use_ragged = self._ragged_enabled(q)
        if self.layer_num < cfg["first_n_dense_layers"]:
            o, _ = ops.dense_attn(q, k, v, tm, k_lens)
            return o

        if do_full_step:
            if inference_step == 0:
                o, lse = ops.dense_attn(q, k, v, tm, k_lens) if do_padding else _dense_attn_raw(q, k, v, tm, k_lens)
                lse[..., k.shape[-2]:, :] = 0
                self.storage.set_lse_constants(lse)
                return o

            ragged = None
            if inference_step == 1 or cfg["recompute_mask"]:
                prev_lse = self.storage.get_lse_constants()
                tk = int(multiple_of * round((cfg["top_keys"] * k.shape[-2]) / multiple_of))
                top_p, k_min = self._top_p(k.shape[-2], multiple_of)
                mask = bs = None
                if (q.is_cuda and cfg["should_compress_indices"] and tk > 0 and amd_key("attn", "fused_colsum_topk")
                        and amd_key("attn", "fused_topk_mask") and k.shape[-2] <= ops.TOPK_MASK_MAX_N):
                    static, groups = self._static(q.shape[1], _cdiv(q.shape[-2], bm), k.shape[-2])
                    if top_p > 0.0:
                        o, mask, lse = ops.dense_colsum_topk_mask_p(q, k, v, prev_lse, tk, top_p, k_min, 0.01, groups, static, tm, k_lens)
                    else:
                        o, mask, lse = ops.dense_colsum_topk_mask(q, k, v, prev_lse, tk, 0.01, groups, static, tm, k_lens)
                elif do_padding:
                    o, bs, lse = ops.dense_colsum_attn(q, k, v, prev_lse, tm, k_lens)
                elif k_lens is not None:
                    o, bs, lse = torch.ops.chipmunk.dense_colsum_attn_varlen(q, k, v, prev_lse, k_lens, tm)
                else:
                    o, bs, lse = (torch.ops.chipmunk.dense_colsum_attn_layout(q, k, v, prev_lse, True) if tm else
                                  torch.ops.chipmunk.dense_colsum_attn(q, k, v, prev_lse))
                lse[..., k.shape[-2]:, :] = 0
                self.storage.set_lse_constants(lse)
                if cfg["should_compress_indices"]:
                    if mask is not None:
                        pass
                    elif tk > 0:
                        mask = self.random_and_topk(bs, tk, top_p, k_min, k_lens)
                    else:
                        mask = self._static(bs.shape[1], bs.shape[-2], bs.shape[-1])[0]
                        if k_lens is not None:
                            mask = mask & _valid_keys(k_lens, mask.shape[-1])
                    packed, mask_shape = ops.bitpack(mask)
                    self.mask_shape[self.layer_counter.cur_model_invocation_per_step] = mask_shape
                    self.storage.set_indices(packed)
                    if use_ragged:
                        ragged = self._ragged_indices(packed, mask_shape, multiple_of, bm, mask)
                        ragged = (ragged[0], ragged[1], _cap_counts(ragged[2], k_lens))
                        self._remember_indices(None, ragged[2], ragged[:2])
                    else:
                        if mask.is_cuda and amd_key("attn", "fused_packed_mask_to_indices") and amd_key("attn", "sorted_indices"):
                            inds, counts = ops.mask_to_sorted_indices(mask, mask.shape, multiple_of, bm)
                        else:
                            inds, counts = ops.mask_to_indices(mask, multiple_of, bm)
                        counts = _cap_counts(counts, k_lens)
                        self._remember_indices(inds, counts)
                else:
                    kseq = k.shape[-2]
                    bs = bs[..., :_cdiv(kseq, bm), :kseq]
                    if k_lens is not None:
                        bs = bs.masked_fill(~_valid_keys(k_lens, kseq), torch.finfo(bs.dtype).min)
                    inds = torch.topk(bs, k=tk, dim=-1).indices
                    counts = torch.full((q.shape[0], q.shape[1], _cdiv(q.shape[-2], bm)), tk, device=q.device,
                                        dtype=torch.int32)
                    pad = torch.empty((*counts.shape, q.shape[-2] - tk), device=q.device, dtype=torch.int32)
                    inds = torch.cat([inds, pad], dim=-1).to(torch.int32)
                    self.storage.set_indices(inds)
                    self.storage.set_counts(counts)
            else:
                o, _ = ops.dense_attn(q, k, v, tm, k_lens)

            if use_ragged:
                if ragged is None:
                    ragged = self._ragged_indices(*self._stored_mask(), multiple_of, bm)
                    ragged = (ragged[0], ragged[1], _cap_counts(ragged[2], k_lens))
            elif not (inference_step == 1 or cfg["recompute_mask"]):
                inds, counts = self._stored_indices(multiple_of, bm)
                if cfg["should_compress_indices"]:
                    counts = _cap_counts(counts, k_lens)

            if ragged is not None:
                o_cache = ops.csp_attn_out_ragged(q, k, v, o, ragged[0], ragged[1], ragged[2], -1)
            elif o.is_cuda and amd_key("attn", "fused_residual"):
                o_cache = ops.csp_attn_out(q, k, v, o, inds, counts, -1)
            elif do_padding:
                o_cache = o - ops.csp_attn(q, k, v, inds, counts)
            else:
                o_cache = o.clone()
                ops.csp_attn_inplace(q, k, v, o_cache, inds, counts, -1)
            self.storage.set_out_cache(o_cache)
            return o

        o = self.storage.get_out_cache()
        kept = self._kept_indices() if (o.is_cuda and amd_key("attn", "fused_residual")) else None
        if kept is not None:
            return ops.csp_attn_out_ragged(q, k, v, o, kept[0], kept[1], kept[2], 1)
        if use_ragged:
            flat, offsets, counts = self._ragged_indices(*self._stored_mask(), multiple_of, bm)
            return ops.csp_attn_out_ragged(q, k, v, o, flat, offsets, _cap_counts(counts, k_lens), 1)
        inds, counts = self._stored_indices(multiple_of, bm)
# ... 28 lines not shown
```

### chipmunk_amd/ops/__init__.py

```python
from .mlp import run_e2e as mlp, GLU_ACTS
from .mlp import run_e2e_glu as mlp_glu, run_e2e_glu, mm1_glu
from .mlp import run_e2e_glu_fp8 as mlp_glu_fp8, run_e2e_glu_fp8, mm1_glu_fp8
from .indexed_io import (copy_indices, topk_indices, mask_to_indices, scatter_add, packed_mask_to_indices,
                         mask_to_sorted_indices, mask_to_ragged_indices, topk_mask, topk_mask_p, topk_indices_p, topk_delta_indices_p, manual_seed,
                         TOPK_MASK_MAX_N)
from .attn import compact_indices, csp_attn, csp_attn_inplace, csp_attn_out, csp_attn_out_ragged, dense_attn, dense_colsum_attn, dense_colsum_topk_mask, dense_colsum_topk_mask_p
from .patch import patchify, unpatchify, patchify_rope
from .bitpack import bitpack, bitunpack
from . import voxel
from .qkv import qkv_split_norm, residual_ln_modulate, split_heads_rownorm, wan_rope_table

__all__ = ["mlp", "copy_indices", "topk_indices", "mask_to_indices", "scatter_add", "csp_attn", "dense_attn",
           "dense_colsum_attn", "patchify", "unpatchify", "patchify_rope", "bitpack", "bitunpack",
           "packed_mask_to_indices", "mask_to_sorted_indices", "csp_attn_inplace", "csp_attn_out", "topk_mask", "TOPK_MASK_MAX_N", "voxel", "manual_seed", "qkv_split_norm", "dense_colsum_topk_mask", "compact_indices", "csp_attn_out_ragged", "residual_ln_modulate",
           "split_heads_rownorm", "wan_rope_table", "mask_to_ragged_indices", "mlp_glu", "run_e2e_glu", "mm1_glu",
           "mlp_glu_fp8", "run_e2e_glu_fp8", "mm1_glu_fp8", "topk_mask_p", "dense_colsum_topk_mask_p",
           "topk_indices_p", "topk_delta_indices_p"]

from . import _fake
```

### chipmunk_amd/ops/_fake.py

```python
import torch


def _o_like(q, token_major):
    B, H, N, D = q.shape
    return q.new_empty((B, N, H, D)).permute(0, 2, 1, 3) if token_major else q.new_empty((B, H, N, D))


def _register():
    lib = torch.library

    @lib.register_fake("chipmunk::csp_128_attn")
    def _(q, k, v, indices, indices_counts):
        return torch.empty_like(q)

    @lib.register_fake("chipmunk::csp_attn_out")
    def _(q, k, v, o_in, indices, indices_counts, o_scale):
        return torch.empty_like(o_in)

    @lib.register_fake("chipmunk::residual_ln_modulate")
    def _(x, y, gate, shift, scale, eps):
        return [torch.empty_like(x), torch.empty_like(x)] if y is not None else [torch.empty_like(x)]

    @lib.register_fake("chipmunk::csp_attn_out_ragged")
    def _(q, k, v, o_in, indices, offsets, indices_counts, o_scale):
# ... 64 lines not shown
    @lib.register_fake("chipmunk::gather_rows")
    def _(src, map):
        shape = list(src.shape)
        shape[-2] = map.shape[0]
        return src.new_empty(shape)

    @lib.register_fake("chipmunk::dense_colsum_topk_mask")
    def _(q, k, v, p, k_top, random_amount, groups, static_mask, token_major_o=False):
        B, H, Nq, D = q.shape
        G = (Nq + 191) // 192
        return [_o_like(q, token_major_o), q.new_empty((B, H, G, k.shape[2]), dtype=torch.bool),
                q.new_empty((B, H, Nq, 1), dtype=torch.float32)]

    @lib.register_fake("chipmunk::topk_mask_p")
    def _(cs, k, top_p, k_min, random_amount, groups, static_mask):
        return cs.new_empty(cs.shape, dtype=torch.bool)

    @lib.register_fake("chipmunk::dense_colsum_topk_mask_p")
    def _(q, k, v, p, k_top, top_p, k_min, random_amount, groups, static_mask, token_major_o=False):
        B, H, Nq, D = q.shape
        G = (Nq + 191) // 192
        return [_o_like(q, token_major_o), q.new_empty((B, H, G, k.shape[2]), dtype=torch.bool),
                q.new_empty((B, H, Nq, 1), dtype=torch.float32)]

    def _dense_out(q):
        return q.new_empty((q.shape[0], q.shape[1], q.shape[2], 1), dtype=torch.float32)

    @lib.register_fake("chipmunk::dense_attn_varlen")
    def _(q, k, v, k_lens, token_major_o=False):
        return [_o_like(q, token_major_o), _dense_out(q)]

    @lib.register_fake("chipmunk::dense_colsum_attn_varlen")
    def _(q, k, v, p, k_lens, token_major_o=False):
        groups = (q.shape[2] + 191) // 192
        return [_o_like(q, token_major_o), q.new_empty((q.shape[0], q.shape[1], groups, max(q.shape[2], k.shape[2]))), _dense_out(q)]

    @lib.register_fake("chipmunk::topk_mask_varlen")
    def _(cs, k_lens, k, random_amount, groups, static_mask):
        return cs.new_empty(cs.shape, dtype=torch.bool)

    @lib.register_fake("chipmunk::topk_mask_p_varlen")
    def _(cs, k_lens, k, top_p, k_min, random_amount, groups, static_mask):
        return cs.new_empty(cs.shape, dtype=torch.bool)

    @lib.register_fake("chipmunk::dense_colsum_topk_mask_varlen")
    def _(q, k, v, p, k_lens, k_top, random_amount, groups, static_mask, token_major_o=False):
        G = (q.shape[2] + 191) // 192
        return [_o_like(q, token_major_o), q.new_empty((q.shape[0], q.shape[1], G, k.shape[2]), dtype=torch.bool), _dense_out(q)]

    @lib.register_fake("chipmunk::dense_colsum_topk_mask_p_varlen")
    def _(q, k, v, p, k_lens, k_top, top_p, k_min, random_amount, groups, static_mask, token_major_o=False):
        G = (q.shape[2] + 191) // 192
        return [_o_like(q, token_major_o), q.new_empty((q.shape[0], q.shape[1], G, k.shape[2]), dtype=torch.bool), _dense_out(q)]

    @lib.register_fake("chipmunk::topk_indices_p")
    def _(activation, indices, counts, sparsity_amount, top_p, min_keys, multiple_of, random_amount):
        torch._check(activation.ndim == 3 and activation.shape[-1] >= 1024, lambda: "activation must be [batch, rows, cols] with cols >= 1024")
        torch._check(indices.shape == activation.shape and counts.numel() == activation.shape[0] * activation.shape[1],
                     lambda: "indices must have the shape of activation, counts must be [batch, rows]")
        return None

    @lib.register_fake("chipmunk::topk_delta_indices_p")
    def _(activation, cache, indices, counts, sparsity_amount, top_p, min_keys, multiple_of, random_amount):
        torch._check(activation.ndim == 3 and activation.shape[-1] >= 1024, lambda: "activation must be [batch, rows, cols] with cols >= 1024")
        torch._check(cache.shape == activation.shape and cache.dtype == activation.dtype, lambda: "cache must have the shape and dtype of activation")
        torch._check(indices.shape == activation.shape and counts.numel() == activation.shape[0] * activation.shape[1],
                     lambda: "indices must have the shape of activation, counts must be [batch, rows]")
        return None

    @lib.register_fake("chipmunk::qkv_split_norm")
    def _(qkv, q_weight, k_weight, heads, eps, freqs_cos=None, freqs_sin=None):
        out = qkv.new_empty((3, 1, heads, qkv.shape[0], 128))
        return [out[0], out[1], out[2]]

    @lib.register_fake("chipmunk::split_heads_rownorm")
    def _(x, heads, parts, w0, w1, w2, norm_mask, rope_mask, eps, freqs_cos=None, freqs_sin=None):
        out = x.new_empty((parts, x.shape[0] if x.dim() == 3 else 1, heads, x.shape[-2], 128))
        return [out[p] for p in range(parts)]

    @lib.register_fake("chipmunk::csp_mlp_mm1_glu")
    def _(a, b_gate, b_up, c, bias_gate, bias_up, pa_cache_colmajor, indices, indices_counts, act, update_cache):
        torch._check(a.shape[-1] == b_gate.shape[1] and b_gate.shape == b_up.shape, lambda: "a, b_gate and b_up must share K; b_up the shape of b_gate")
        torch._check(c.shape == a.shape[:-1] + (b_gate.shape[0],), lambda: "c must be [M, F] ([B, M, F] with the batch size of a)")
        torch._check(act in ("gelu_tanh", "silu", "gelu"), lambda: f"csp_mlp_mm1_glu: unknown activation '{act}'")
        return None

    @lib.register_fake("chipmunk::csp_mlp_mm1_glu_fp8")
    def _(a, b_gate, b_up, c, bias_gate, bias_up, pa_cache_colmajor, indices, indices_counts, scale_a, scale_b_gate, scale_b_up, act,
          update_cache):
        f8 = torch.float8_e4m3fn
        torch._check(a.dtype == f8 and b_gate.dtype == f8 and b_up.dtype == f8, lambda: "a, b_gate and b_up must be float8_e4m3fn")
        torch._check(c.dtype == torch.bfloat16 and pa_cache_colmajor.dtype == torch.bfloat16, lambda: "c and pa_cache_colmajor must be bfloat16")
        torch._check(a.shape[-1] == b_gate.shape[1] and b_gate.shape == b_up.shape, lambda: "a, b_gate and b_up must share K; b_up the shape of b_gate")
        torch._check(c.shape == a.shape[:-1] + (b_gate.shape[0],), lambda: "c must be [M, F] ([B, M, F] with the batch size of a)")
        for s in (scale_a, scale_b_gate, scale_b_up):
            torch._check(s.dtype == torch.float32 and s.numel() == 1, lambda: "scale_a, scale_b_gate and scale_b_up must be one-element float32 tensors")
        torch._check(act in ("gelu_tanh", "silu", "gelu"), lambda: f"csp_mlp_mm1_glu_fp8: unknown activation '{act}'")
        return None

    @lib.register_fake("chipmunk::csp_mlp_mm1_act")
    def _(a, b, c, bias, pa_cache, indices, counts, act, update_cache):
        torch._check(a.shape[-1] == b.shape[1], lambda: "a and b must share the K dimension")
        torch._check(c.shape == a.shape[:-1] + (b.shape[0],), lambda: "c must be [M, F] ([B, M, F] with the batch size of a)")
        torch._check(bias is None or bias.numel() == b.shape[0], lambda: "bias must have F entries")
        torch._check(act in ("gelu_tanh", "silu", "gelu"), lambda: f"csp_mlp_mm1_act: unknown activation '{act}'")
        return None
# ... 47 lines not shown
```

### chipmunk_amd/ops/attn.py

```python
from __future__ import annotations

from typing import Optional, Tuple

import torch
import torch.nn.functional as F

PM = 192


def _pad_len(n: int) -> int:
    return ((n + PM - 1) // PM) * PM


def _last_dim_contiguous(t: torch.Tensor) -> torch.Tensor:
    return t if t.stride(-1) == 1 else t.contiguous()


def check_k_lens(k_lens: Optional[torch.Tensor], like: torch.Tensor, who: str) -> Optional[torch.Tensor]:
    if k_lens is None:
        return None
    if not like.is_cuda:
        raise ValueError(f"{who}: k_lens is supported on the GPU only (got {like.device} operands)")
    if not isinstance(k_lens, torch.Tensor) or k_lens.dtype != torch.int32:
        raise ValueError(f"{who}: k_lens must be an int32 tensor (got {getattr(k_lens, 'dtype', type(k_lens))})")
# ... 10 lines not shown
    n = q.shape[-2]
    q, k, v = _last_dim_contiguous(q), _last_dim_contiguous(k), _last_dim_contiguous(v)
    if check_k_lens(k_lens, q, "dense_attn") is not None:
        o, l = torch.ops.chipmunk.dense_attn_varlen(q, k, v, k_lens, token_major_o)
    else:
        o, l = torch.ops.chipmunk.dense_attn_layout(q, k, v, True) if token_major_o else torch.ops.chipmunk.dense_attn(q, k, v)
    padded = _pad_len(n)
    if padded != n:
        l = F.pad(l, (0, 0, 0, padded - n))
    return o, l


def dense_colsum_attn(q: torch.Tensor, k: torch.Tensor, v: torch.Tensor, p: torch.Tensor, token_major_o: bool = False,
                      k_lens: Optional[torch.Tensor] = None) -> Tuple[torch.Tensor, torch.Tensor, torch.Tensor]:
    n = q.shape[-2]
    padded = _pad_len(n)
    assert p.shape[-2] in (n, padded), "p must be the l vector of the previous full step"
    p_rows = p[..., :n, :].contiguous()
    q, k, v = _last_dim_contiguous(q), _last_dim_contiguous(k), _last_dim_contiguous(v)
    if check_k_lens(k_lens, q, "dense_colsum_attn") is not None:
        o, cs, l = torch.ops.chipmunk.dense_colsum_attn_varlen(q, k, v, p_rows, k_lens, token_major_o)
    elif token_major_o:
        o, cs, l = torch.ops.chipmunk.dense_colsum_attn_layout(q, k, v, p_rows, True)
    else:
        o, cs, l = torch.ops.chipmunk.dense_colsum_attn(q, k, v, p_rows)
    if padded != n:
        l = F.pad(l, (0, 0, 0, padded - n))
    kseq = k.shape[-2]
    kgroups = (kseq + PM - 1) // PM
    if cs.shape[-2] != kgroups or cs.shape[-1] != kseq:
        cs = cs[..., :kgroups, :kseq]
    return o, cs, l


def dense_colsum_topk_mask(q: torch.Tensor, k: torch.Tensor, v: torch.Tensor, p: torch.Tensor, k_top: int, random_amount: float,
                           groups, static_mask, token_major_o: bool = False, k_lens: Optional[torch.Tensor] = None
                           ) -> Tuple[torch.Tensor, torch.Tensor, torch.Tensor]:
    n = q.shape[-2]
    padded = _pad_len(n)
    assert p.shape[-2] in (n, padded), "p must be the l vector of the previous full step"
    if check_k_lens(k_lens, q, "dense_colsum_topk_mask") is not None:
        o, mask, l = torch.ops.chipmunk.dense_colsum_topk_mask_varlen(_last_dim_contiguous(q), _last_dim_contiguous(k), _last_dim_contiguous(v),
                                                                      p[..., :n, :].contiguous(), k_lens, k_top, random_amount, groups,
                                                                      static_mask, token_major_o)
    else:
        o, mask, l = torch.ops.chipmunk.dense_colsum_topk_mask(_last_dim_contiguous(q), _last_dim_contiguous(k), _last_dim_contiguous(v),
                                                               p[..., :n, :].contiguous(), k_top, random_amount, groups, static_mask,
                                                               token_major_o)
    if padded != n:
        l = F.pad(l, (0, 0, 0, padded - n))
    return o, mask, l


def dense_colsum_topk_mask_p(q: torch.Tensor, k: torch.Tensor, v: torch.Tensor, p: torch.Tensor, k_top: int, top_p: float, k_min: int,
                             random_amount: float, groups, static_mask, token_major_o: bool = False,
                             k_lens: Optional[torch.Tensor] = None) -> Tuple[torch.Tensor, torch.Tensor, torch.Tensor]:
    check_k_lens(k_lens, q, "dense_colsum_topk_mask_p")
    if not q.is_cuda:
        from .indexed_io import topk_mask_p
        o, cs, l = dense_colsum_attn(q, k, v, p, token_major_o)
        return o, topk_mask_p(cs, k_top, top_p, k_min, random_amount, groups, static_mask), l
    n = q.shape[-2]
    padded = _pad_len(n)
    assert p.shape[-2] in (n, padded), "p must be the l vector of the previous full step"
    if k_lens is not None:
        o, mask, l = torch.ops.chipmunk.dense_colsum_topk_mask_p_varlen(_last_dim_contiguous(q), _last_dim_contiguous(k),
                                                                        _last_dim_contiguous(v), p[..., :n, :].contiguous(), k_lens, k_top,
                                                                        top_p, k_min, random_amount, groups, static_mask, token_major_o)
    else:
        o, mask, l = torch.ops.chipmunk.dense_colsum_topk_mask_p(_last_dim_contiguous(q), _last_dim_contiguous(k), _last_dim_contiguous(v),
                                                                 p[..., :n, :].contiguous(), k_top, top_p, k_min, random_amount, groups,
                                                                 static_mask, token_major_o)
    if padded != n:
        l = F.pad(l, (0, 0, 0, padded - n))
    return o, mask, l


def csp_attn(q: torch.Tensor, k: torch.Tensor, v: torch.Tensor, indices: torch.Tensor,
             indices_counts: torch.Tensor) -> torch.Tensor:
    return torch.ops.chipmunk.csp_128_attn(q.contiguous(), k.contiguous(), v.contiguous(), indices.contiguous(),
                                           indices_counts.contiguous())


def csp_attn_inplace(q: torch.Tensor, k: torch.Tensor, v: torch.Tensor, o: torch.Tensor, indices: torch.Tensor,
                     indices_counts: torch.Tensor, o_scale: int) -> None:
    torch.ops.chipmunk.csp_attn(q, k, v, o, indices, indices_counts, o_scale)


def csp_attn_out(q: torch.Tensor, k: torch.Tensor, v: torch.Tensor, o_in: torch.Tensor, indices: torch.Tensor,
                 indices_counts: torch.Tensor, o_scale: int) -> torch.Tensor:
    return torch.ops.chipmunk.csp_attn_out(q, k, v, o_in, indices, indices_counts, o_scale)


def compact_indices(indices: torch.Tensor, indices_counts: torch.Tensor) -> Tuple[torch.Tensor, torch.Tensor]:
    return tuple(torch.ops.chipmunk.compact_indices(indices.contiguous(), indices_counts.contiguous()))


def csp_attn_out_ragged(q: torch.Tensor, k: torch.Tensor, v: torch.Tensor, o_in: torch.Tensor, indices: torch.Tensor,
                        offsets: torch.Tensor, indices_counts: torch.Tensor, o_scale: int) -> torch.Tensor:
    return torch.ops.chipmunk.csp_attn_out_ragged(q, k, v, o_in, indices, offsets, indices_counts, o_scale)


__all__ = ["csp_attn", "csp_attn_inplace", "csp_attn_out", "csp_attn_out_ragged", "compact_indices", "dense_attn", "dense_colsum_attn",
           "dense_colsum_topk_mask", "dense_colsum_topk_mask_p"]
```

### chipmunk_amd/ops/indexed_io.py

```python
from __future__ import annotations

from typing import List, Optional, Sequence

import torch

TOPK_MASK_MAX_N = 1024 * 512


def copy_indices(bm_fc1: torch.Tensor, bm_mid_cache: torch.Tensor, indices: torch.Tensor, counts: torch.Tensor) -> None:
    torch.ops.chipmunk.copy_indices(bm_fc1, bm_mid_cache, indices, counts)


def topk_indices(activations: torch.Tensor, indices_out: torch.Tensor, counts_out: torch.Tensor,
                 sparsity_amount: float, multiple_of: int, rk: float) -> None:
    torch.ops.chipmunk.topk_indices(activations, indices_out, counts_out, sparsity_amount, multiple_of, rk)


def _check_top_p(who: str, sparsity_amount: float, top_p: float, min_keys: float) -> None:
    if not (0.0 < top_p <= 1.0) or not (0.0 <= sparsity_amount <= 1.0) or not (0.0 <= min_keys <= 1.0 - sparsity_amount + 1e-9):
        raise ValueError(f"{who}: top_p must be in (0, 1], sparsity_amount in [0, 1] and min_keys in [0, 1 - sparsity_amount] "
                         f"(got top_p {top_p}, sparsity_amount {sparsity_amount}, min_keys {min_keys})")


def _f32(x: float) -> float:
    return float(torch.tensor(float(x), dtype=torch.float32))


def _topk_indices_p_cpu(activations: torch.Tensor, indices_out: torch.Tensor, counts_out: torch.Tensor, sparsity_amount: float,
                        top_p: float, min_keys: float, multiple_of: int, rk: float) -> None:
    f = activations.shape[-1]
    if f < 1024:
        raise ValueError(f"topk_indices_p: rows of 1024 columns or more (the quantiles are taken over the first 1024); got {f}")
    rows = activations.reshape(-1, f).double()
    inds, counts = indices_out.view(-1, f), counts_out.view(-1)
    if _f32(sparsity_amount) == 1.0:
        inds.fill_(-1)
        counts.zero_()
        return
    mass = torch.where(rows > 0, rows, torch.zeros_like(rows))
    desc, _ = mass.sort(dim=-1, descending=True)
    csum = desc.cumsum(-1)
    total = csum[:, -1:]
    first = (csum < top_p * total).sum(-1, keepdim=True).clamp(max=f - 1)
    inf = torch.full_like(total, float("inf"))
    thr_p = torch.where(total > 0, desc.gather(-1, first), inf)
    sample = rows[:, :1024].sort(dim=-1).values
    iq = int(1024 * _f32(sparsity_amount))
    thr_q = -inf if sparsity_amount == 0 else sample[:, iq:iq + 1]
    im = 1024 if min_keys == 0 else max(int(1024 * _f32(1.0 - min_keys)), iq)
    thr_min = inf if im >= 1024 else sample[:, im:im + 1]
    thr = torch.minimum(torch.maximum(thr_p, thr_q), thr_min)
    keep = (rows > 0) & (rows >= thr)
    listed = keep | (~keep & (torch.rand(keep.shape) < rk)) if rk > 0 else keep
    cols = torch.arange(f, dtype=torch.int64)
    for r in range(rows.shape[0]):
        on = cols[listed[r]]
        off = cols[~listed[r]]
        last = torch.full((1024,), -1, dtype=torch.int64).scatter_reduce(0, off % 1024, off, "amax")
        pad = (-on.numel()) % multiple_of
        row = torch.cat([on, last[last >= 0][:pad]])
        inds[r, : row.numel()] = row.to(torch.int32)
        counts[r] = on.numel() + pad


def topk_indices_p(activations: torch.Tensor, indices_out: torch.Tensor, counts_out: torch.Tensor, sparsity_amount: float,
                   top_p: float, min_keys: float, multiple_of: int, rk: float) -> None:
    _check_top_p("topk_indices_p", sparsity_amount, top_p, min_keys)
    if not activations.is_cuda:
        return _topk_indices_p_cpu(activations, indices_out, counts_out, sparsity_amount, top_p, min_keys, multiple_of, rk)
    torch.ops.chipmunk.topk_indices_p(activations, indices_out, counts_out, sparsity_amount, top_p, min_keys, multiple_of, rk)


def topk_delta_indices_p(activations: torch.Tensor, cache: torch.Tensor, indices_out: torch.Tensor, counts_out: torch.Tensor,
                         sparsity_amount: float, top_p: float, min_keys: float, multiple_of: int, rk: float) -> None:
    _check_top_p("topk_delta_indices_p", sparsity_amount, top_p, min_keys)
    torch.ops.chipmunk.topk_delta_indices_p(activations, cache, indices_out, counts_out, sparsity_amount, top_p, min_keys, multiple_of, rk)


def scatter_add(packed: torch.Tensor, unpacked: torch.Tensor, indices: torch.Tensor, counts: torch.Tensor,
                num_sms: int) -> None:
    if packed.ndim == 3:
        torch.ops.chipmunk.csp_scatter_add(packed, unpacked, indices, counts, num_sms)
        return
    torch.ops.chipmunk.csp_scatter_add(packed.unsqueeze(0), unpacked.unsqueeze(0), indices.unsqueeze(0),
                                       counts.unsqueeze(0), num_sms)


def mask_to_indices(mask: torch.Tensor, multiple_of: int, pad_to_multiple_of: int) -> List[torch.Tensor]:
    return torch.ops.chipmunk.mask_to_indices(mask, multiple_of, pad_to_multiple_of)


def packed_mask_to_indices(packed: torch.Tensor, shape: Sequence[int], multiple_of: int,
                           pad_to_multiple_of: int) -> List[torch.Tensor]:
    return torch.ops.chipmunk.packed_mask_to_indices(packed, list(shape), multiple_of, pad_to_multiple_of)


def mask_to_sorted_indices(mask: torch.Tensor, shape: Sequence[int], multiple_of: int,
                           pad_to_multiple_of: int) -> List[torch.Tensor]:
    return torch.ops.chipmunk.mask_to_sorted_indices(mask, list(shape), multiple_of, pad_to_multiple_of)


def mask_to_ragged_indices(mask: torch.Tensor, shape: Sequence[int], multiple_of: int, pad_to_multiple_of: int,
                           sorted: bool = True) -> List[torch.Tensor]:
    if mask.is_cuda:
        return torch.ops.chipmunk.mask_to_ragged_indices(mask, list(shape), multiple_of, pad_to_multiple_of, sorted)
    if mask.dtype == torch.uint8:
        from .bitpack import bitunpack
        mask = bitunpack(mask, shape)
    b, h, m, n = mask.shape
    pad_n = (n + pad_to_multiple_of - 1) // pad_to_multiple_of * pad_to_multiple_of
    rows = mask.reshape(-1, n) != 0
    kept = rows.sum(dim=1)
    counts = (kept + multiple_of - 1) // multiple_of * multiple_of
    lengths = (counts.clamp(max=pad_n) + 31) // 32 * 32
    offsets = torch.zeros(rows.shape[0] + 1, dtype=torch.int64)
    offsets[1:] = lengths.cumsum(0)
    flat = torch.zeros(int(offsets[-1]) + 64, dtype=torch.int32)
    cols = torch.arange(n, dtype=torch.int32)
    for r in range(rows.shape[0]):
        true = cols[rows[r]]
        if not sorted:
            true = true[torch.argsort(true % 32, stable=True)]
        row = torch.cat([true, cols[~rows[r]][:int(counts[r] - kept[r])]])
        flat[int(offsets[r]):int(offsets[r]) + row.numel()] = row
    return [flat, offsets, counts.to(torch.int32).view(b, h, m)]


def topk_mask(cs: torch.Tensor, k: int, random_amount: float = 0.0, groups: Optional[torch.Tensor] = None,
              static_mask: Optional[torch.Tensor] = None, k_lens: Optional[torch.Tensor] = None) -> torch.Tensor:
    from .attn import check_k_lens
    if check_k_lens(k_lens, cs, "topk_mask") is not None:
        return torch.ops.chipmunk.topk_mask_varlen(cs, k_lens, k, random_amount, groups, static_mask)
    return torch.ops.chipmunk.topk_mask(cs, k, random_amount, groups, static_mask)


def _bf16_keys(cs: torch.Tensor) -> torch.Tensor:
    bits = cs.contiguous().view(torch.int16).to(torch.int64) & 0xFFFF
    return torch.where((bits & 0x8000) != 0, ~bits & 0xFFFF, bits | 0x8000)


def _topk_mask_p_cpu(cs: torch.Tensor, k: int, top_p: float, k_min: int, random_amount: float,
                     groups: Optional[torch.Tensor], static_mask: Optional[torch.Tensor]) -> torch.Tensor:
    if not (0.0 < top_p <= 1.0) or k_min < 0 or k < 0:
        raise ValueError(f"topk_mask_p: top_p must be in (0, 1], k and k_min >= 0 (got {top_p}, {k}, {k_min})")
    B, H, G, n = cs.shape
    k = min(int(k), n)
    cols = torch.arange(n, dtype=torch.int64)
    rank = (0xFFFF - _bf16_keys(cs).view(-1, n)) * (1 << 30) + ((cols % 4096) // 4) * (1 << 20) + cols
    order = torch.argsort(rank, dim=-1)
    val = cs.reshape(-1, n).double()
    mass = torch.where(val > 0, val, torch.zeros_like(val)).gather(-1, order)
    prefix = mass.cumsum(-1)
    total = prefix[:, -1:]
    k_p = (prefix < top_p * total).sum(-1) + 1
    k_p = torch.where(total[:, 0] > 0, k_p, torch.zeros_like(k_p))
    s = k_p.clamp(min=int(k_min)).clamp(max=k)
    keep = torch.zeros(cs.numel() // n, n, dtype=torch.bool)
    keep.scatter_(-1, order, cols[None, :] < s[:, None])
    keep = keep.view(B, H, G, n)
    if random_amount > 0:
        keep |= torch.rand(keep.shape) < random_amount
    if groups is not None:
        keep &= groups
    if static_mask is not None:
        keep = keep | static_mask
    return keep


def topk_mask_p(cs: torch.Tensor, k: int, top_p: float, k_min: int = 0, random_amount: float = 0.0,
                groups: Optional[torch.Tensor] = None, static_mask: Optional[torch.Tensor] = None,
                k_lens: Optional[torch.Tensor] = None) -> torch.Tensor:
    from .attn import check_k_lens
    check_k_lens(k_lens, cs, "topk_mask_p")
    if not cs.is_cuda:
        return _topk_mask_p_cpu(cs, k, top_p, k_min, random_amount, groups, static_mask)
    if k_lens is not None:
        return torch.ops.chipmunk.topk_mask_p_varlen(cs, k_lens, k, top_p, k_min, random_amount, groups, static_mask)
    return torch.ops.chipmunk.topk_mask_p(cs, k, top_p, k_min, random_amount, groups, static_mask)


def manual_seed(seed: int) -> None:
    from .._native import manual_seed as _seed
    _seed(seed)
```

### chipmunk_amd/util/config.py

```python
from __future__ import annotations

import copy
from typing import Any, Dict

import yaml

BASE_CONFIG: Dict[str, Any] = {
    "num_model_invocations_per_inference_step": 1,
    "should_profile": False,
    "generation_index": 0,
    "steps": 50,
    "world_size": 1,
    "mlp": {
        "is_enabled": True,
        "is_fp8": False,
        "top_keys": "dd",
        "random_keys": 0.05,
        "full_step_every": 10,
        "block_mask_cache": 2,
        "first_n_dense_layers": 2,
        "counts_multiple_of": 256,
        "bm": 128,
        "mbm": 128,
    },
# ... 5 lines not shown
    "attn": {
        "is_enabled": True,
        "top_keys": 0.05,
        "random_keys": 0.01,
        "local_voxels": 0,
        "local_1d_window": 0,
        "first_n_dense_layers": 2,
        "full_step_every": 10,
        "full_step_schedule": None,
        "recompute_mask": True,
        "should_compress_indices": True,
        "counts_multiple_of": 128,
        "pad_qkv_before_kernel": True,
        "mbm": 192,
    },
    "offloading": {
        "global_disable_offloading": False,
        "mlp.out_cache": False,
        "mlp.indices": False,
        "mlp.counts": False,
        "mlp.sparse_act_T": False,
        "mlp.blockmean_mid_cache": False,
        "attn.out_cache": True,
        "attn.indices": True,
        "attn.counts": False,
        "attn.lse_constants": False,
        "text_encoders": True,
    },
    "step_caching": {
        "is_enabled": True,
        "skip_step_schedule": {7, 11, 13, 14, 15, 17, 18, 19, 21, 22, 23, 25, 26, 27, 29, 31, 33, 34, 35, 37, 38, 39,
                               41, 42, 43},
    },
}

AMD_EXTRA_KEYS: Dict[str, Any] = {
    "offloading.keep_resident_if_fits": False,
    "offloading.hbm_budget_gb": 200.0,
    "offloading.native_host_pool": True,
    "attn.fused_packed_mask_to_indices": True,
    "attn.sorted_indices": True,
    "mlp.fused_topk_delta": True,
    "mlp.fused_block_mean": True,
    "mlp.fused_fp8_quantize": True,
    "attn.fused_residual": True,
    "attn.fused_topk_mask": True,
    "attn.fused_colsum_topk": True,
    "mlp.fused_scatter": True,
    "attn.token_major_output": False,
    "attn.keep_unpacked_indices": True,
    "attn.keep_unpacked_indices_offloaded": True,
    "attn.kept_indices_offloaded_budget_gb": 8.0,
    "attn.ragged_mask_to_indices": True,
    "mlp.fp8_fc2": False,
    "attn.top_p": 0.0,
    "attn.top_p_min_keys": 0.0,
    "mlp.top_p": 0.0,
    "mlp.top_p_min_keys": 0.0,
    "mlp.fp8_scaling": "tensor",
}
BASE_CONFIG["offloading"]["keep_resident_if_fits"] = AMD_EXTRA_KEYS["offloading.keep_resident_if_fits"]
BASE_CONFIG["offloading"]["hbm_budget_gb"] = AMD_EXTRA_KEYS["offloading.hbm_budget_gb"]
BASE_CONFIG["offloading"]["native_host_pool"] = AMD_EXTRA_KEYS["offloading.native_host_pool"]
BASE_CONFIG["attn"]["fused_packed_mask_to_indices"] = AMD_EXTRA_KEYS["attn.fused_packed_mask_to_indices"]
BASE_CONFIG["attn"]["sorted_indices"] = AMD_EXTRA_KEYS["attn.sorted_indices"]
BASE_CONFIG["mlp"]["fused_topk_delta"] = AMD_EXTRA_KEYS["mlp.fused_topk_delta"]
BASE_CONFIG["attn"]["fused_residual"] = AMD_EXTRA_KEYS["attn.fused_residual"]
BASE_CONFIG["attn"]["fused_topk_mask"] = AMD_EXTRA_KEYS["attn.fused_topk_mask"]
BASE_CONFIG["attn"]["fused_colsum_topk"] = AMD_EXTRA_KEYS["attn.fused_colsum_topk"]
BASE_CONFIG["mlp"]["fused_scatter"] = AMD_EXTRA_KEYS["mlp.fused_scatter"]
BASE_CONFIG["attn"]["token_major_output"] = AMD_EXTRA_KEYS["attn.token_major_output"]
BASE_CONFIG["attn"]["keep_unpacked_indices"] = AMD_EXTRA_KEYS["attn.keep_unpacked_indices"]
BASE_CONFIG["attn"]["keep_unpacked_indices_offloaded"] = AMD_EXTRA_KEYS["attn.keep_unpacked_indices_offloaded"]
BASE_CONFIG["attn"]["kept_indices_offloaded_budget_gb"] = AMD_EXTRA_KEYS["attn.kept_indices_offloaded_budget_gb"]
BASE_CONFIG["attn"]["ragged_mask_to_indices"] = AMD_EXTRA_KEYS["attn.ragged_mask_to_indices"]
BASE_CONFIG["mlp"]["fp8_fc2"] = AMD_EXTRA_KEYS["mlp.fp8_fc2"]
BASE_CONFIG["attn"]["top_p"] = AMD_EXTRA_KEYS["attn.top_p"]
BASE_CONFIG["attn"]["top_p_min_keys"] = AMD_EXTRA_KEYS["attn.top_p_min_keys"]
BASE_CONFIG["mlp"]["top_p"] = AMD_EXTRA_KEYS["mlp.top_p"]
BASE_CONFIG["mlp"]["top_p_min_keys"] = AMD_EXTRA_KEYS["mlp.top_p_min_keys"]
BASE_CONFIG["mlp"]["fp8_scaling"] = AMD_EXTRA_KEYS["mlp.fp8_scaling"]

GLOBAL_CONFIG: Dict[str, Any] = copy.deepcopy(BASE_CONFIG)


def amd_key(section: str, key: str) -> Any:
    return GLOBAL_CONFIG.get(section, {}).get(key, AMD_EXTRA_KEYS[f"{section}.{key}"])


def update_global_config(config: Dict[str, Any]) -> None:
    GLOBAL_CONFIG.update(config)


def _deep_update(dst: Dict[str, Any], src: Dict[str, Any]) -> None:
    for key, value in src.items():
        if isinstance(value, dict) and isinstance(dst.get(key), dict):
            _deep_update(dst[key], value)
        else:
            dst[key] = value


def load_from_file(config_file: str) -> None:
    with open(config_file, "r") as f:
        loaded = yaml.safe_load(f)
    if loaded:
        _deep_update(GLOBAL_CONFIG, loaded)
# ... 8 lines not shown
```

### include/chipmunk_hip.h

```cpp
#ifndef CHIPMUNK_HIP_H
#define CHIPMUNK_HIP_H

#include <stdint.h>

#ifdef __cplusplus
extern "C" {
#endif

#define CHIPMUNK_OK 0
#define CHIPMUNK_ERR_INVALID 1
#define CHIPMUNK_ERR_LAUNCH 2
#define CHIPMUNK_ERR_UNSUPPORTED 3

#define CHIPMUNK_DTYPE_BF16 0
#define CHIPMUNK_DTYPE_FP16 1
#define CHIPMUNK_DTYPE_FP32 2

const char *chipmunk_last_error(void);
int chipmunk_abi_version(void);
int chipmunk_set_option(const char *name, int value);
int chipmunk_set_random_seed(uint64_t seed);

int chipmunk_csp_attn(const void *q, const void *k, const void *v, void *o, const int64_t q_strides[3],
                      const int64_t k_strides[3], const int64_t v_strides[3], const int64_t o_strides[3],
// ... 151 lines not shown
int chipmunk_topk_indices_p(const void *activation, int dtype, int32_t *indices, int32_t *counts, int rows, int cols,
                            double sparsity_amount, double top_p, double min_keys, int multiple_of, double random_amount,
                            void *stream);

int chipmunk_topk_delta_indices_p(const void *activation, void *cache, int dtype, int32_t *indices, int32_t *counts, int rows,
                                  int cols, double sparsity_amount, double top_p, double min_keys, int multiple_of,
                                  double random_amount, void *stream);

int chipmunk_dense_colsum_topk_mask(const void *q, const void *k, const void *v, const int64_t q_strides[3],
                                    const int64_t k_strides[3], const int64_t v_strides[3], const float *p, void *o, float *l,
                                    int B, int H, int Nq, int Nk, const void *static_mask, int64_t static_stride, int static_rows,
                                    const void *group_flags, void *mask, int k_top, double random_amount, void *stream);

int chipmunk_topk_mask(const void *cs, int64_t cs_stride, const void *static_mask, int64_t static_stride,
                       int static_rows, const void *group_flags, void *mask, int rows, int n, int k,
                       double random_amount, void *stream);

int chipmunk_topk_mask_p(const void *cs, int64_t cs_stride, const void *static_mask, int64_t static_stride,
                         int static_rows, const void *group_flags, void *mask, int rows, int n, int k,
                         double random_amount, double top_p, int k_min, void *stream);

int chipmunk_dense_colsum_topk_mask_p_strided(const void *q, const void *k, const void *v, const int64_t q_strides[3],
                                              const int64_t k_strides[3], const int64_t v_strides[3], const float *p, void *o,
                                              const int64_t *o_strides, float *l, int B, int H, int Nq, int Nk,
                                              const void *static_mask, int64_t static_stride, int static_rows,
                                              const void *group_flags, void *mask, int k_top, double random_amount,
                                              double top_p, int k_min, void *stream);

int chipmunk_dense_attn_varlen(const void *q, const void *k, const void *v, const int64_t q_strides[3],
                               const int64_t k_strides[3], const int64_t v_strides[3], void *o, const int64_t *o_strides,
                               float *l, const int32_t *k_lens, int B, int H, int Nq, int Nk, void *stream);
int chipmunk_dense_colsum_attn_varlen(const void *q, const void *k, const void *v, const int64_t q_strides[3],
                                      const int64_t k_strides[3], const int64_t v_strides[3], const float *p, void *o,
                                      const int64_t *o_strides, void *cs, float *l, const int32_t *k_lens, int B, int H,
                                      int Nq, int Nk, int cs_stride, void *stream);
int chipmunk_dense_colsum_topk_mask_varlen(const void *q, const void *k, const void *v, const int64_t q_strides[3],
                                           const int64_t k_strides[3], const int64_t v_strides[3], const float *p, void *o,
                                           const int64_t *o_strides, float *l, const int32_t *k_lens, int B, int H, int Nq,
                                           int Nk, const void *static_mask, int64_t static_stride, int static_rows,
                                           const void *group_flags, void *mask, int k_top, double random_amount, void *stream);
int chipmunk_dense_colsum_topk_mask_p_varlen(const void *q, const void *k, const void *v, const int64_t q_strides[3],
                                             const int64_t k_strides[3], const int64_t v_strides[3], const float *p, void *o,
                                             const int64_t *o_strides, float *l, const int32_t *k_lens, int B, int H, int Nq,
                                             int Nk, const void *static_mask, int64_t static_stride, int static_rows,
                                             const void *group_flags, void *mask, int k_top, double random_amount,
                                             double top_p, int k_min, void *stream);
int chipmunk_topk_mask_varlen(const void *cs, int64_t cs_stride, const void *static_mask, int64_t static_stride,
                              int static_rows, const void *group_flags, void *mask, const int32_t *k_lens, int seq_rows,
                              int rows, int n, int k, double random_amount, void *stream);
int chipmunk_topk_mask_p_varlen(const void *cs, int64_t cs_stride, const void *static_mask, int64_t static_stride,
                                int static_rows, const void *group_flags, void *mask, const int32_t *k_lens, int seq_rows,
                                int rows, int n, int k, double random_amount, double top_p, int k_min, void *stream);

int chipmunk_mask_to_indices(const void *mask, int32_t *indices, int32_t *counts, int64_t rows, int n, int pad_n,
                             int multiple_of, void *stream);

int chipmunk_packed_mask_to_indices(const void *packed, int32_t *indices, int32_t *counts, int64_t rows, int n,
                                    int pad_n, int multiple_of, void *stream);

int chipmunk_mask_to_sorted_indices(const void *mask, int packed, int32_t *indices, int32_t *counts, int64_t rows,
                                    int n, int pad_n, int multiple_of, void *stream);

int chipmunk_mask_row_counts(const void *mask, int packed, int32_t *counts, int64_t *lengths, int64_t rows, int n, int pad_n,
                             int multiple_of, void *stream);
int chipmunk_mask_to_ragged_indices(const void *mask, int packed, int sorted, const int64_t *offsets, int32_t *flat, int64_t rows,
                                    int n, int multiple_of, void *stream);

int chipmunk_copy_indices(const void *src, void *dst, const int32_t *inds, const int32_t *counts, int B, int M, int R,
                          int F, int elem_size, void *stream);

int chipmunk_transpose16(const void *src, void *dst, int B, int R, int C, void *stream);
int chipmunk_transpose16_pitched(const void *src, void *dst, int B, int R, int C, int ld, void *stream);

int chipmunk_block_mean(const void *x, void *out, int64_t rows, int C, int mbm, void *stream);
int chipmunk_block_mean_ragged(const void *x, void *out, int64_t rows, int C, int mbm, void *stream);

int chipmunk_quantize_fp8(const void *x, const float *scale, void *out, int64_t n, float max_value, void *stream);

#define CHIPMUNK_QUANTIZE_ROWWISE_MAX_K 16384
int chipmunk_quantize_fp8_rowwise(const void *x, void *out, float *scale_recip, int64_t rows, int K, float max_value, void *stream);

int chipmunk_bitpack(const void *mask, void *packed, int64_t n, void *stream);
int chipmunk_bitunpack(const void *packed, void *mask, int64_t n, void *stream);

int chipmunk_gather_rows(const void *src, void *dst, const int32_t *map, int64_t outer, int64_t n_src, int64_t n_out,
                         int64_t row_bytes, void *stream);

int chipmunk_host_alloc(size_t bytes, void **host_ptr);
int chipmunk_host_free(void *host_ptr);
int chipmunk_copy_d2h_async(void *host_dst, const void *dev_src, size_t bytes, void *stream);
int chipmunk_copy_h2d_async(void *dev_dst, const void *host_src, size_t bytes, void *stream);
size_t chipmunk_host_bytes(void);

int chipmunk_release_scratch(void);
int chipmunk_big_scratch_fallbacks(void);

int chipmunk_qkv_split_norm(const void *qkv, int64_t row_stride, const void *q_weight, const void *k_weight, void *q, void *k,
                            void *v, int64_t n, int heads, float eps, const float *freqs_cos, const float *freqs_sin,
                            int64_t rope_rows, void *stream);

int chipmunk_split_heads_rownorm(const void *x, int64_t batch_stride, int64_t row_stride, int parts, const void *w0, int w0_dtype,
                                 const void *w1, int w1_dtype, const void *w2, int w2_dtype, void *out0, void *out1, void *out2,
                                 unsigned norm_mask, unsigned rope_mask, int64_t B, int64_t n, int heads, float eps,
                                 const float *freqs_cos, const float *freqs_sin, int64_t rope_rows, void *stream);

#ifdef __cplusplus
// ... 4 lines not shown
```

Measured before the change: 0.5845.

## Emit bit-packed top-k masks with per-row kept counts from the fused colsum kernel

Adds a BITS variant of the top-k mask kernel that writes one bit per key instead of a byte, assembling nibbles across lanes with DPP and writing packed words directly. It also records per-row kept counts, so the later ragged index conversion can size rows without rescanning the mask. New fused dense-colsum entry points, torch ops and a config flag (on by default) route attention selection through the packed path. This cuts mask write and read traffic and drops a counting pass, in exchange for more code paths and a lower maximum key count.

```diff
diff --git a/chipmunk_amd/_native.py b/chipmunk_amd/_native.py
--- a/chipmunk_amd/_native.py
+++ b/chipmunk_amd/_native.py
@@ -22,6 +22,8 @@
     "chipmunk_bitpack", "chipmunk_bitunpack", "chipmunk_transpose16", "chipmunk_block_mean", "chipmunk_quantize_fp8", "chipmunk_gather_rows", "chipmunk_qkv_split_norm", "chipmunk_split_heads_rownorm", "chipmunk_dense_colsum_topk_mask", "chipmunk_dense_attn_strided", "chipmunk_csp_attn_out_ragged", "chipmunk_compact_indices", "chipmunk_residual_ln_modulate", "chipmunk_dense_colsum_attn_strided", "chipmunk_dense_colsum_topk_mask_strided", "chipmunk_release_scratch", "chipmunk_big_scratch_fallbacks",
     "chipmunk_dense_attn_varlen", "chipmunk_dense_colsum_attn_varlen", "chipmunk_dense_colsum_topk_mask_varlen",
     "chipmunk_dense_colsum_topk_mask_p_varlen", "chipmunk_topk_mask_varlen", "chipmunk_topk_mask_p_varlen",
+    "chipmunk_topk_mask_bits", "chipmunk_topk_mask_bits_varlen", "chipmunk_dense_colsum_topk_bits_strided", "chipmunk_dense_colsum_topk_bits_varlen",
+    "chipmunk_row_counts_to_lengths",
     "chipmunk_host_alloc", "chipmunk_host_free", "chipmunk_copy_d2h_async", "chipmunk_copy_h2d_async", "chipmunk_host_bytes",
 ]
 
diff --git a/chipmunk_amd/csrc/attn.hip b/chipmunk_amd/csrc/attn.hip
--- a/chipmunk_amd/csrc/attn.hip
+++ b/chipmunk_amd/csrc/attn.hip
@@ -1273,15 +1273,16 @@
                                        const int64_t *o_strides, float *l, int B, int H, int Nq, int Nk, const void *static_mask,
                                        int64_t static_stride, int static_rows, const void *group_flags, void *mask,
                                        int topk, double random_amount, bool mass, double top_p, int k_min, void *stream,
-                                       const int32_t *klens = nullptr) {
+                                       const int32_t *klens = nullptr, void *packed = nullptr, int32_t *row_counts = nullptr) {
     if (int e = check_common(q, k, v, o, B, H, Nq, Nk)) return e;
-    CM_CHECK(l && pin && mask, "dense_colsum_topk_mask: p / l / mask missing");
+    CM_CHECK(l && pin && (packed ? row_counts != nullptr && !mass : mask != nullptr), "dense_colsum_topk_mask: p / l / mask missing");
     if (int e = check_strides(q_strides, "q")) return e;
     if (int e = check_strides(k_strides, "k")) return e;
     if (int e = check_strides(v_strides, "v")) return e;
     hipStream_t st = (hipStream_t)stream;
     if (!use_dense64(B, H, Nq, Nk) || chipmunk_get_option("attn_fused_colsum") == 2 || (Nk & 3) || Nk > CHIPMUNK_TOPK_MASK_MAX_N)
         return CHIPMUNK_ERR_UNSUPPORTED;
+    if (packed && ((Nk & 7) || Nk > CHIPMUNK_TOPK_MASK_BITS_MAX_N || chipmunk_get_option("topk_mask_stream") == 1)) return CHIPMUNK_ERR_UNSUPPORTED;
     AttnParams p = {};
     p.q = (const uint16_t *)q, p.k = (const uint16_t *)k, p.v = (const uint16_t *)v, p.o = (uint16_t *)o;
     for (int i = 0; i < 3; ++i) p.qs[i] = q_strides[i], p.ks[i] = k_strides[i], p.vs[i] = v_strides[i];
@@ -1295,6 +1296,9 @@
     if (!part) return CHIPMUNK_ERR_UNSUPPORTED;
     if (int e = chipmunk_dense64_colsum_launch(p, part, st)) return e;
     const int nrb = ((Nq + 255) / 256) * 2;
+    if (packed)
+        return chipmunk_topk_mask_bits_parts(part, chipmunk_colsum_part_stride(Nk), nrb, p.G, Nq, static_mask, static_stride, static_rows, group_flags, packed,
+                                             row_counts, B * H * p.G, Nk, topk, random_amount, st, klens, H * p.G);
     if (mass)
         return chipmunk_topk_mask_p_parts(part, chipmunk_colsum_part_stride(Nk), nrb, p.G, Nq, static_mask, static_stride, static_rows, group_flags, mask,
                                           B * H * p.G, Nk, topk, top_p, k_min, random_amount, st, klens, H * p.G);
@@ -1330,6 +1334,26 @@
     return chipmunk_dense_colsum_topk_mask_strided(q, k, v, q_strides, k_strides, v_strides, pin, o, nullptr, l, B, H, Nq, Nk,
                                                    static_mask, static_stride, static_rows, group_flags, mask, topk, random_amount,
                                                    stream);
+}
+
+extern "C" int chipmunk_dense_colsum_topk_bits_strided(const void *q, const void *k, const void *v, const int64_t q_strides[3],
+                                                       const int64_t k_strides[3], const int64_t v_strides[3], const float *pin, void *o,
+                                                       const int64_t *o_strides, float *l, int B, int H, int Nq, int Nk, const void *static_mask,
+                                                       int64_t static_stride, int static_rows, const void *group_flags, void *packed,
+                                                       int32_t *row_counts, int topk, double random_amount, void *stream) {
+    CM_CHECK(packed && row_counts, "dense_colsum_topk_bits: packed / row_counts missing");
+    return dense_colsum_topk_mask_impl(q, k, v, q_strides, k_strides, v_strides, pin, o, o_strides, l, B, H, Nq, Nk, static_mask, static_stride,
+                                       static_rows, group_flags, nullptr, topk, random_amount, false, 0.0, 0, stream, nullptr, packed, row_counts);
+}
+
+extern "C" int chipmunk_dense_colsum_topk_bits_varlen(const void *q, const void *k, const void *v, const int64_t q_strides[3],
+                                                      const int64_t k_strides[3], const int64_t v_strides[3], const float *pin, void *o,
+                                                      const int64_t *o_strides, float *l, const int32_t *k_lens, int B, int H, int Nq, int Nk,
+                                                      const void *static_mask, int64_t static_stride, int static_rows, const void *group_flags,
+                                                      void *packed, int32_t *row_counts, int topk, double random_amount, void *stream) {
+    CM_CHECK(packed && row_counts, "dense_colsum_topk_bits: packed / row_counts missing");
+    return dense_colsum_topk_mask_impl(q, k, v, q_strides, k_strides, v_strides, pin, o, o_strides, l, B, H, Nq, Nk, static_mask, static_stride,
+                                       static_rows, group_flags, nullptr, topk, random_amount, false, 0.0, 0, stream, k_lens, packed, row_counts);
 }
 
 extern "C" int chipmunk_dense_colsum_topk_mask_varlen(const void *q, const void *k, const void *v, const int64_t q_strides[3],
diff --git a/chipmunk_amd/csrc/attn_params.h b/chipmunk_amd/csrc/attn_params.h
--- a/chipmunk_amd/csrc/attn_params.h
+++ b/chipmunk_amd/csrc/attn_params.h
@@ -42,6 +42,9 @@
 int chipmunk_topk_mask_p_parts(const uint16_t *part, int part_stride, int nrb, int groups_per_bh, int Nq, const void *static_mask, int64_t static_stride,
                                int static_rows, const void *group_flags, void *mask, int rows, int n, int k, double top_p, int k_min,
                                double random_amount, hipStream_t stream, const int32_t *klens = nullptr, int seq_rows = 0);
+int chipmunk_topk_mask_bits_parts(const uint16_t *part, int part_stride, int nrb, int groups_per_bh, int Nq, const void *static_mask, int64_t static_stride,
+                                  int static_rows, const void *group_flags, void *packed, int32_t *row_counts, int rows, int n, int k,
+                                  double random_amount, hipStream_t stream, const int32_t *klens = nullptr, int seq_rows = 0);
 size_t chipmunk_colsum_part_bytes(int B, int H, int Nq, int Nk);
 int chipmunk_colsum_part_stride(int Nk);
 int chipmunk_colsum64_launch(const AttnParams &p, hipStream_t stream);
diff --git a/chipmunk_amd/csrc/common.h b/chipmunk_amd/csrc/common.h
--- a/chipmunk_amd/csrc/common.h
+++ b/chipmunk_amd/csrc/common.h
@@ -130,6 +130,7 @@
 }
 
 #define CHIPMUNK_TOPK_MASK_MAX_N (1024 * 512)
+#define CHIPMUNK_TOPK_MASK_BITS_MAX_N (1024 * 120)
 
 void chipmunk_set_error(const char *fmt, ...);
 int chipmunk_get_option(const char *name);
diff --git a/chipmunk_amd/csrc/indexed_io.hip b/chipmunk_amd/csrc/indexed_io.hip
--- a/chipmunk_amd/csrc/indexed_io.hip
+++ b/chipmunk_amd/csrc/indexed_io.hip
@@ -246,6 +246,15 @@
     }
 }
 
+__global__ __launch_bounds__(256) void row_counts_to_lengths_kernel(const int32_t *kept, int32_t *counts, int64_t *lengths, int64_t rows,
+                                                                    int pad_n, int multiple_of) {
+    const int64_t row = (int64_t)blockIdx.x * 256 + threadIdx.x;
+    if (row >= rows) return;
+    const int64_t padded = (((int64_t)kept[row] + multiple_of - 1) / multiple_of) * multiple_of;
+    counts[row] = (int32_t)padded;
+    lengths[row] = (min(padded, (int64_t)pad_n) + 31) / 32 * 32;
+}
+
 struct TopkParams {
     const void *act;
     void *cache;
@@ -633,6 +642,8 @@
     int k_min;
     const int32_t *klens;
     int seq_rows;
+    uint8_t *packed;
+    int32_t *row_counts;
 };
 
 __device__ __forceinline__ int topk_mask_row_len(const TopkMaskParams &p, int row) {
@@ -678,8 +689,9 @@
     return (u & 0x8000u) ? (~u & 0xffffu) : (u | 0x8000u);
 }
 
-template <int KPT, bool ALIGNED, bool PARTS = false, bool MASS = false>
+template <int KPT, bool ALIGNED, bool PARTS = false, bool MASS = false, bool BITS = false>
 __global__ __launch_bounds__(1024) void topk_mask_kernel(const TopkMaskParams p) {
+    static_assert(!BITS || ALIGNED, "the packed output needs the aligned form");
     constexpr int NV = KPT / 4;
     __shared__ int wave_cnt[16];
     const int tid = threadIdx.x, lane = tid & 63, w = tid >> 6;
@@ -913,6 +925,7 @@
     }
     const uint32_t salt = p.salt ^ (first * 0x27D4EB2Fu);
     const int nsteps = (n + 4095) / 4096;
+    constexpr int OSH = BITS ? 1 : 8;
     auto emit = [&](auto keyed, int c, uint32_t v0, uint32_t v1, uint32_t sb) {
         uint32_t bytes = 0;
         if constexpr (decltype(keyed)::value) asm volatile("" : "+v"(v0), "+v"(v1));
@@ -927,16 +940,22 @@
             if (rnd && !keep) keep = hash_uniform(row, c + e, salt) < p.random_amount;
             keep = keep || ((sb >> (8 * e)) & 0xffu) != 0;
             keep = keep && c + e < nv;
-            bytes |= (keep ? 1u : 0u) << (8 * e);
-        }
-        if constexpr (ALIGNED) {
+            bytes |= (keep ? 1u : 0u) << (OSH * e);
+        }
+        if constexpr (BITS) {
+            return bytes;
+        } else if constexpr (ALIGNED) {
             *(uint32_t *)(out + c) = bytes;
         } else {
 #pragma unroll
             for (int e = 0; e < 4; ++e)
                 if (c + e < n) out[c + e] = (uint8_t)(bytes >> (8 * e));
         }
+        return 0u;
     };
+    int kept = 0;
+    uint8_t *prow_bits = BITS ? p.packed + (((int64_t)row * n) >> 3) : nullptr;
+    const uint32_t lane_offb = (uint32_t)tid >> 1;
     if constexpr (ALIGNED) {
         constexpr int OB = 5;
 #pragma unroll
@@ -950,9 +969,29 @@
             __builtin_amdgcn_sched_barrier(0);
 #pragma unroll
             for (int jj = 0; jj < OB; ++jj) {
-                if constexpr (true) {
+                if constexpr (!BITS) {
                     const int c = 4 * tid + 4096 * (j0 + jj);
                     if (j0 + jj < NV && c < n) emit(std::integral_constant<int, 1>{}, c, key[(j0 + jj) < NV ? (j0 + jj) : 0][0], key[(j0 + jj) < NV ? (j0 + jj) : 0][1], sbv[jj]);
+                    asm volatile("" ::: "memory");
+                } else if (j0 + jj < NV) {
+                    const int c = 4 * tid + 4096 * (j0 + jj);
+                    uint32_t nib = 0;
+                    if (c < n) nib = emit(std::integral_constant<int, 1>{}, c, key[(j0 + jj) < NV ? (j0 + jj) : 0][0], key[(j0 + jj) < NV ? (j0 + jj) : 0][1], sbv[jj]);
+                    kept += __popc(nib);
+                    uint32_t d = nib | ((uint32_t)__builtin_amdgcn_update_dpp(0, (int)nib, 0xB1, 0xf, 0xf, true) << 4);
+                    d |= (uint32_t)__builtin_amdgcn_update_dpp(0, (int)d, 0x4E, 0xf, 0xf, true) << 8;
+                    d |= (uint32_t)__builtin_amdgcn_update_dpp(0, (int)d, 0x104, 0xf, 0xf, true) << 16;
+                    if ((tid & 7) == 0 && c < n) {
+                        unsigned char *dst = (unsigned char *)(prow_bits + 512 * (j0 + jj)) + lane_offb;
+                        if (c + 32 <= n) {
+                            __builtin_memcpy(dst, &d, 4);
+                        } else {
+                            const int rb = (n & 31) >> 3;
+                            dst[0] = (uint8_t)d;
+                            if (rb >= 2) dst[1] = (uint8_t)(d >> 8);
+                            if (rb == 3) dst[2] = (uint8_t)(d >> 16);
+                        }
+                    }
                     asm volatile("" ::: "memory");
                 }
             }
@@ -972,6 +1011,10 @@
             }
             emit(std::integral_constant<int, 0>{}, c, v0, v1, sb);
         }
+    }
+    if constexpr (BITS) {
+        const int total = block_count(kept);
+        if (tid == 0) p.row_counts[row] = total;
     }
 }
 
@@ -1346,6 +1389,21 @@
     return CHIPMUNK_OK;
 }
 
+extern "C" int chipmunk_row_counts_to_lengths(const int32_t *row_counts, int32_t *counts, int64_t *lengths, int64_t rows, int n, int pad_n,
+                                              int multiple_of, void *stream) {
+    CM_CHECK(row_counts && counts && lengths, "row_counts_to_lengths: null pointer");
+    CM_CHECK(rows >= 0 && n > 0 && pad_n >= n && multiple_of > 0, "row_counts_to_lengths: bad sizes rows=%lld n=%d pad_n=%d multiple_of=%d",
+             (long long)rows, n, pad_n, multiple_of);
+    CM_CHECK(rows < (1ll << 31), "row_counts_to_lengths: too many rows");
+    const size_t lds = m2i_lds_bytes(n, true);
+    CM_CHECK(lds <= 160 * 1024, "mask_to_indices: row length %d needs %zu B of LDS (> 160 KiB)", n, lds);
+    if (rows == 0) return CHIPMUNK_OK;
+    hipLaunchKernelGGL(row_counts_to_lengths_kernel, dim3((unsigned)((rows + 255) / 256)), dim3(256), 0, (hipStream_t)stream, row_counts, counts,
+                       lengths, rows, pad_n, multiple_of);
+    CM_LAUNCH_CHECK();
+    return CHIPMUNK_OK;
+}
+
 extern "C" int chipmunk_mask_to_ragged_indices(const void *mask, int packed, int sorted, const int64_t *offsets, int32_t *flat,
                                                int64_t rows, int n, int multiple_of, void *stream) {
     if (packed) return sorted ? launch_m2i<true, true, true>(mask, flat, nullptr, rows, n, n, multiple_of, stream, offsets)
@@ -1513,6 +1571,30 @@
     CM_CHECK(top_p > 0.0 && top_p <= 1.0 && k_min >= 0, "topk_mask_p_parts: top_p must be in (0, 1] and k_min >= 0 (got %g, %d)", top_p, k_min);
     return topk_mask_parts_impl<true>(part, part_stride, nrb, groups_per_bh, Nq, static_mask, static_stride, static_rows, group_flags, mask, rows, n, k,
                                       random_amount, top_p, k_min, s, klens, seq_rows);
+}
+
+int chipmunk_topk_mask_bits_parts(const uint16_t *part, int part_stride, int nrb, int groups_per_bh, int Nq, const void *static_mask, int64_t static_stride,
+                                  int static_rows, const void *group_flags, void *packed, int32_t *row_counts, int rows, int n, int k,
+                                  double random_amount, hipStream_t s, const int32_t *klens, int seq_rows) {
+    CM_CHECK(!klens || seq_rows > 0, "topk_mask_bits_parts: k_lens without the rows per sequence");
+    CM_CHECK(part && packed && row_counts && rows >= 0 && n > 0 && (n & 7) == 0 && n <= CHIPMUNK_TOPK_MASK_BITS_MAX_N && k >= 0 && part_stride >= n &&
+                 (part_stride & 3) == 0, "topk_mask_bits_parts: bad arguments");
+    CM_CHECK(!static_mask || (static_rows > 0 && static_stride >= n && (static_stride & 3) == 0 && ((uintptr_t)static_mask & 3) == 0),
+             "topk_mask_bits_parts: bad static mask geometry");
+    CM_CHECK(((uintptr_t)part & 7) == 0, "topk_mask_bits_parts: unaligned buffers");
+    if (rows == 0) return CHIPMUNK_OK;
+    TopkMaskParams p = {nullptr, (const uint8_t *)static_mask, (const uint8_t *)group_flags, nullptr, 0, static_stride,
+                        rows, n, k, static_mask ? static_rows : 1, (float)random_amount,
+                        random_amount > 0.0 ? chipmunk_next_random_salt() : 0u};
+    p.parts = part, p.pstride = part_stride, p.nrb = nrb, p.ngroups = groups_per_bh, p.nq = Nq;
+    p.top_p = 0.f, p.k_min = 0;
+    p.klens = klens, p.seq_rows = seq_rows;
+    p.packed = (uint8_t *)packed, p.row_counts = row_counts;
+    if (n <= 1024 * 16) hipLaunchKernelGGL((topk_mask_kernel<16, true, true, false, true>), dim3(rows), dim3(1024), 0, s, p);
+    else if (n <= 1024 * 48) hipLaunchKernelGGL((topk_mask_kernel<48, true, true, false, true>), dim3(rows), dim3(1024), 0, s, p);
+    else hipLaunchKernelGGL((topk_mask_kernel<120, true, true, false, true>), dim3(rows), dim3(1024), 0, s, p);
+    CM_LAUNCH_CHECK();
+    return CHIPMUNK_OK;
 }
 
 __global__ __launch_bounds__(256) void qkv_split_norm_kernel(const uint16_t *qkv, int64_t row_stride, const uint16_t *qw,
@@ -1645,6 +1727,47 @@
                                 stream, k_lens, seq_rows);
 }
 
+static int topk_mask_bits_impl(const void *cs, int64_t cs_stride, const void *static_mask, int64_t static_stride, int static_rows,
+                               const void *group_flags, void *packed, int32_t *row_counts, int rows, int n, int k, double random_amount,
+                               void *stream, const int32_t *klens, int seq_rows) {
+    CM_CHECK(cs && packed && row_counts, "topk_mask_bits: null pointer");
+    CM_CHECK(!klens || (seq_rows > 0 && rows % seq_rows == 0), "topk_mask_bits: %d rows are no whole sequences of %d rows", rows, seq_rows);
+    CM_CHECK(rows >= 0 && n > 0 && k >= 0, "topk_mask_bits: bad sizes (rows=%d n=%d k=%d)", rows, n, k);
+    CM_CHECK(n % 8 == 0, "topk_mask_bits: n must be a multiple of 8 (got %d)", n);
+    CM_CHECK(cs_stride >= n, "topk_mask_bits: cs row stride %lld < n %d", (long long)cs_stride, n);
+    CM_CHECK(n <= CHIPMUNK_TOPK_MASK_BITS_MAX_N, "topk_mask_bits: rows of more than %d columns are not supported (got %d)", CHIPMUNK_TOPK_MASK_BITS_MAX_N, n);
+    CM_CHECK(!static_mask || (static_rows > 0 && static_stride >= n), "topk_mask_bits: bad static mask geometry");
+    CM_CHECK(random_amount >= 0.0 && random_amount <= 1.0, "topk_mask_bits: random_amount must be in [0,1]");
+    if ((((uintptr_t)cs) & 7) != 0 || (cs_stride * 2) % 8 != 0 || (static_mask && ((((uintptr_t)static_mask) & 3) != 0 || static_stride % 4 != 0)))
+        return CHIPMUNK_ERR_UNSUPPORTED;
+    if (rows == 0) return CHIPMUNK_OK;
+    TopkMaskParams p = {(const uint16_t *)cs, (const uint8_t *)static_mask, (const uint8_t *)group_flags, nullptr,
+                        cs_stride, static_stride, rows, n, k, static_mask ? static_rows : 1, (float)random_amount,
+                        random_amount > 0.0 ? chipmunk_next_random_salt() : 0u};
+    p.klens = klens, p.seq_rows = seq_rows;
+    p.packed = (uint8_t *)packed, p.row_counts = row_counts;
+    hipStream_t s = (hipStream_t)stream;
+    if (n <= 1024 * 16) hipLaunchKernelGGL((topk_mask_kernel<16, true, false, false, true>), dim3(rows), dim3(1024), 0, s, p);
+    else if (n <= 1024 * 48) hipLaunchKernelGGL((topk_mask_kernel<48, true, false, false, true>), dim3(rows), dim3(1024), 0, s, p);
+    else hipLaunchKernelGGL((topk_mask_kernel<120, true, false, false, true>), dim3(rows), dim3(1024), 0, s, p);
+    CM_LAUNCH_CHECK();
+    return CHIPMUNK_OK;
+}
+
+extern "C" int chipmunk_topk_mask_bits(const void *cs, int64_t cs_stride, const void *static_mask, int64_t static_stride, int static_rows,
+                                       const void *group_flags, void *packed, int32_t *row_counts, int rows, int n, int k,
+                                       double random_amount, void *stream) {
+    return topk_mask_bits_impl(cs, cs_stride, static_mask, static_stride, static_rows, group_flags, packed, row_counts, rows, n, k, random_amount,
+                               stream, nullptr, 0);
+}
+
+extern "C" int chipmunk_topk_mask_bits_varlen(const void *cs, int64_t cs_stride, const void *static_mask, int64_t static_stride, int static_rows,
+                                              const void *group_flags, void *packed, int32_t *row_counts, const int32_t *k_lens, int seq_rows,
+                                              int rows, int n, int k, double random_amount, void *stream) {
+    return topk_mask_bits_impl(cs, cs_stride, static_mask, static_stride, static_rows, group_flags, packed, row_counts, rows, n, k, random_amount,
+                               stream, k_lens, seq_rows);
+}
+
 extern "C" int chipmunk_compact_indices(const int32_t *indices, int64_t idx_stride, const int32_t *counts, const int64_t *offsets,
                                         int32_t *flat, int64_t rows, void *stream) {
     CM_CHECK(indices && counts && offsets && flat, "compact_indices: null pointer");
diff --git a/chipmunk_amd/csrc/torch_registry.cpp b/chipmunk_amd/csrc/torch_registry.cpp
--- a/chipmunk_amd/csrc/torch_registry.cpp
+++ b/chipmunk_amd/csrc/torch_registry.cpp
@@ -912,8 +912,8 @@
     return {indices, counts};
 }
 
-std::vector<at::Tensor> mask_to_ragged_indices(at::Tensor mask, at::IntArrayRef shape, int64_t multiple_of, int64_t pad_to_multiple_of,
-                                               bool sorted) {
+static std::vector<at::Tensor> mask_to_ragged_indices_impl(at::Tensor mask, at::IntArrayRef shape, int64_t multiple_of, int64_t pad_to_multiple_of,
+                                                           bool sorted, const OptTensor &row_counts) {
     CHECK_DEV(mask);
     const bool packed = mask.scalar_type() == at::kByte;
     TORCH_CHECK(packed || mask.scalar_type() == at::kBool, "mask must be bool, or uint8 bit-packed with a shape");
@@ -928,9 +928,19 @@
     c10::DeviceGuard guard(mask.device());
     at::Tensor counts = at::empty({b, h, m}, mask.options().dtype(at::kInt));
     at::Tensor len = at::empty({rows}, mask.options().dtype(at::kLong));
-    check(chipmunk_mask_row_counts(mask.data_ptr(), packed ? 1 : 0, counts.data_ptr<int>(), len.data_ptr<int64_t>(), rows, (int)n,
-                                   (int)pad_n, (int)multiple_of, cur_stream(mask)),
-          "mask_to_ragged_indices");
+    if (row_counts.has_value() && row_counts->defined()) {
+        at::Tensor rc = *row_counts;
+        CHECK_DEV(rc);
+        TORCH_CHECK(rc.scalar_type() == at::kInt && rc.numel() == rows && rc.device() == mask.device(), "row_counts must be int32 with one entry per mask row");
+        rc = rc.contiguous();
+        check(chipmunk_row_counts_to_lengths(rc.data_ptr<int>(), counts.data_ptr<int>(), len.data_ptr<int64_t>(), rows, (int)n, (int)pad_n,
+                                             (int)multiple_of, cur_stream(mask)),
+              "mask_to_ragged_indices");
+    } else {
+        check(chipmunk_mask_row_counts(mask.data_ptr(), packed ? 1 : 0, counts.data_ptr<int>(), len.data_ptr<int64_t>(), rows, (int)n,
+                                       (int)pad_n, (int)multiple_of, cur_stream(mask)),
+              "mask_to_ragged_indices");
+    }
     at::Tensor offsets = at::zeros({rows + 1}, len.options());
     if (rows) offsets.narrow(0, 1, rows).copy_(len.cumsum(0));
     const int64_t total = rows ? offsets[rows].item<int64_t>() : 0;
@@ -942,14 +952,28 @@
     return {flat, offsets, counts};
 }
 
+std::vector<at::Tensor> mask_to_ragged_indices(at::Tensor mask, at::IntArrayRef shape, int64_t multiple_of, int64_t pad_to_multiple_of,
+                                               bool sorted) {
+    return mask_to_ragged_indices_impl(mask, shape, multiple_of, pad_to_multiple_of, sorted, c10::nullopt);
+}
+
+std::vector<at::Tensor> mask_to_ragged_indices_counted(at::Tensor mask, at::Tensor row_counts, at::IntArrayRef shape, int64_t multiple_of,
+                                                       int64_t pad_to_multiple_of, bool sorted) {
+    return mask_to_ragged_indices_impl(mask, shape, multiple_of, pad_to_multiple_of, sorted, row_counts);
+}
+
 std::vector<at::Tensor> dense_colsum_attn_layout(at::Tensor q, at::Tensor k, at::Tensor v, at::Tensor p, bool token_major_o);
 static at::Tensor topk_mask_impl(at::Tensor cs, int64_t k, bool mass, double top_p, int64_t k_min, double random_amount,
                                  const c10::optional<at::Tensor> &groups, const c10::optional<at::Tensor> &static_mask,
                                  const OptTensor &k_lens = c10::nullopt);
+static std::vector<at::Tensor> topk_mask_bits_impl(at::Tensor cs, int64_t k, double random_amount, const c10::optional<at::Tensor> &groups,
+                                                   const c10::optional<at::Tensor> &static_mask, const OptTensor &k_lens = c10::nullopt);
 static std::vector<at::Tensor> dense_colsum_topk_mask_impl(at::Tensor q, at::Tensor k, at::Tensor v, at::Tensor p, int64_t k_top, bool mass, double top_p,
                                                            int64_t k_min, double random_amount, const c10::optional<at::Tensor> &groups,
                                                            const c10::optional<at::Tensor> &static_mask, bool token_major_o,
-                                                           const OptTensor &k_lens = c10::nullopt) {
+                                                           const OptTensor &k_lens = c10::nullopt, bool bits = false) {
+    if (bits) TORCH_CHECK(!mass && k.dim() == 4 && k.size(2) % 8 == 0 && k.size(2) <= 1024 * 120,
+                          "dense_colsum_topk_bits: the key count must be a multiple of 8 and at most 122880");
     const int32_t *kl = klens_ptr(k_lens, q, q.dim() == 4 ? q.size(0) : 0);
     if (mass) TORCH_CHECK(top_p > 0.0 && top_p <= 1.0 && k_min >= 0, "top_p must be in (0, 1] and k_min >= 0 (got ", top_p, ", ", k_min, ")");
     CHECK_DEV(q); CHECK_DEV(k); CHECK_DEV(v); CHECK_DEV(p);
@@ -983,16 +1007,25 @@
             at::Tensor o = alloc_o(q, q, token_major_o);
             const int64_t os[3] = {o.stride(0), o.stride(1), o.stride(2)};
             at::Tensor l = at::empty({B, H, Nq, 1}, q.options().dtype(at::kFloat));
-            at::Tensor mask = at::empty({B, H, G, Nk}, q.options().dtype(at::kBool));
+            at::Tensor mask, packed, row_counts;
+            if (bits) {
+                packed = at::empty({B * H * G * Nk / 8}, q.options().dtype(at::kByte));
+                row_counts = at::empty({B, H, G}, q.options().dtype(at::kInt));
+            } else {
+                mask = at::empty({B, H, G, Nk}, q.options().dtype(at::kBool));
+            }
             const int64_t qs[3] = {q.stride(0), q.stride(1), q.stride(2)}, ks[3] = {k.stride(0), k.stride(1), k.stride(2)},
                           vs[3] = {v.stride(0), v.stride(1), v.stride(2)};
-            const int rc = mass ? chipmunk_dense_colsum_topk_mask_p_varlen(q.data_ptr(), k.data_ptr(), v.data_ptr(), qs, ks, vs, p.data_ptr<float>(), o.data_ptr(),
+            const int rc = bits ? chipmunk_dense_colsum_topk_bits_varlen(q.data_ptr(), k.data_ptr(), v.data_ptr(), qs, ks, vs, p.data_ptr<float>(), o.data_ptr(),
+                                                                         os, l.data_ptr<float>(), kl, (int)B, (int)H, (int)Nq, (int)Nk, st, st_stride, (int)st_rows, gf,
+                                                                         packed.data_ptr(), row_counts.data_ptr<int>(), (int)k_top, random_amount, cur_stream(q))
+                           : mass ? chipmunk_dense_colsum_topk_mask_p_varlen(q.data_ptr(), k.data_ptr(), v.data_ptr(), qs, ks, vs, p.data_ptr<float>(), o.data_ptr(),
                                                                            os, l.data_ptr<float>(), kl, (int)B, (int)H, (int)Nq, (int)Nk, st, st_stride, (int)st_rows, gf,
                                                                            mask.data_ptr(), (int)k_top, random_amount, top_p, (int)(k_min > Nk ? Nk : k_min), cur_stream(q))
                                 : chipmunk_dense_colsum_topk_mask_varlen(q.data_ptr(), k.data_ptr(), v.data_ptr(), qs, ks, vs, p.data_ptr<float>(), o.data_ptr(),
                                                            os, l.data_ptr<float>(), kl, (int)B, (int)H, (int)Nq, (int)Nk, st, st_stride, (int)st_rows, gf,
                                                            mask.data_ptr(), (int)k_top, random_amount, cur_stream(q));
-            if (rc == CHIPMUNK_OK) return {o, mask, l};
+            if (rc == CHIPMUNK_OK) return bits ? std::vector<at::Tensor>{o, packed, row_counts, l} : std::vector<at::Tensor>{o, mask, l};
             if (rc != CHIPMUNK_ERR_UNSUPPORTED) check(rc, "dense_colsum_topk_mask");
         }
     }
@@ -1000,6 +1033,10 @@
     at::Tensor cs = ocl[1];
     const int64_t Nk = k.size(2), G = (q.size(2) + 191) / 192;
     if (cs.size(-1) != Nk || cs.size(-2) != G) cs = cs.slice(-2, 0, G).slice(-1, 0, Nk);
+    if (bits) {
+        auto pr = topk_mask_bits_impl(cs, k_top, random_amount, groups, static_mask, k_lens);
+        return {ocl[0], pr[0], pr[1], ocl[2]};
+    }
     return {ocl[0], topk_mask_impl(cs, k_top, mass, top_p, k_min, random_amount, groups, static_mask, k_lens), ocl[2]};
 }
 
@@ -1025,6 +1062,69 @@
                                                  double random_amount, const c10::optional<at::Tensor> &groups,
                                                  const c10::optional<at::Tensor> &static_mask, bool token_major_o) {
     return dense_colsum_topk_mask_impl(q, k, v, p, k_top, true, top_p, k_min, random_amount, groups, static_mask, token_major_o);
+}
+
+std::vector<at::Tensor> dense_colsum_topk_bits(at::Tensor q, at::Tensor k, at::Tensor v, at::Tensor p, int64_t k_top, double random_amount,
+                                               const c10::optional<at::Tensor> &groups, const c10::optional<at::Tensor> &static_mask,
+                                               bool token_major_o) {
+    return dense_colsum_topk_mask_impl(q, k, v, p, k_top, false, 0.0, 0, random_amount, groups, static_mask, token_major_o, c10::nullopt, true);
+}
+
+std::vector<at::Tensor> dense_colsum_topk_bits_varlen(at::Tensor q, at::Tensor k, at::Tensor v, at::Tensor p, at::Tensor k_lens, int64_t k_top,
+                                                      double random_amount, const c10::optional<at::Tensor> &groups,
+                                                      const c10::optional<at::Tensor> &static_mask, bool token_major_o) {
+    return dense_colsum_topk_mask_impl(q, k, v, p, k_top, false, 0.0, 0, random_amount, groups, static_mask, token_major_o, k_lens, true);
+}
+
+static std::vector<at::Tensor> topk_mask_bits_impl(at::Tensor cs, int64_t k, double random_amount, const c10::optional<at::Tensor> &groups,
+                                                   const c10::optional<at::Tensor> &static_mask, const OptTensor &k_lens) {
+    CHECK_DEV(cs); CHECK_BF16(cs);
+    TORCH_CHECK(cs.dim() == 4 && cs.stride(3) == 1, "cs must be [B, H, G, N] with a contiguous last dim");
+    const int64_t B = cs.size(0), H = cs.size(1), G = cs.size(2), N = cs.size(3);
+    TORCH_CHECK(N % 8 == 0 && N <= 1024 * 120, "topk_mask_bits: rows must have a multiple of 8 and at most 122880 columns (got ", N, ")");
+    const int32_t *kl = klens_ptr(k_lens, cs, B);
+    if (!(cs.stride(1) == G * cs.stride(2) && (B == 1 || cs.stride(0) == H * cs.stride(1)) && cs.stride(2) % 4 == 0 &&
+          ((uintptr_t)cs.data_ptr() & 7) == 0))
+        cs = cs.contiguous();
+    const int64_t rows = B * H * G;
+    c10::DeviceGuard guard(cs.device());
+    at::Tensor packed = at::empty({rows * N / 8}, cs.options().dtype(at::kByte));
+    at::Tensor row_counts = at::empty({B, H, G}, cs.options().dtype(at::kInt));
+    const void *st = nullptr, *gf = nullptr;
+    int64_t st_stride = 0, st_rows = 1;
+    at::Tensor stc, gfc;
+    if (static_mask.has_value() && static_mask->defined()) {
+        stc = *static_mask;
+        CHECK_DEV(stc);
+        TORCH_CHECK(stc.scalar_type() == at::kBool && stc.dim() == 4 && stc.size(3) == N && stc.size(2) == G &&
+                    stc.size(1) == H && (stc.size(0) == 1 || stc.size(0) == B), "static_mask must be bool [1|B, H, G, N]");
+        if (!(stc.stride(3) == 1 && stc.stride(1) == G * stc.stride(2) && (stc.size(0) == 1 || stc.stride(0) == H * stc.stride(1)) &&
+              stc.stride(2) % 4 == 0 && ((uintptr_t)stc.data_ptr() & 3) == 0))
+            stc = stc.contiguous();
+        st = stc.data_ptr(), st_stride = stc.stride(2), st_rows = stc.size(0) * H * G;
+    }
+    if (groups.has_value() && groups->defined()) {
+        gfc = *groups;
+        CHECK_DEV(gfc);
+        TORCH_CHECK(gfc.scalar_type() == at::kBool && gfc.dim() == 4 && gfc.size(3) == 1 && gfc.size(2) == G &&
+                    gfc.size(1) == H && (gfc.size(0) == 1 || gfc.size(0) == B), "groups must be bool [1|B, H, G, 1]");
+        gfc = gfc.expand({B, H, G, 1}).contiguous();
+        gf = gfc.data_ptr();
+    }
+    check(chipmunk_topk_mask_bits_varlen(cs.data_ptr(), cs.stride(2), st, st_stride, (int)st_rows, gf, packed.data_ptr(), row_counts.data_ptr<int>(),
+                                         kl, (int)(H * G), (int)rows, (int)N, (int)k, random_amount, cur_stream(cs)),
+          "topk_mask_bits");
+    return {packed, row_counts};
+}
+
+std::vector<at::Tensor> topk_mask_bits(at::Tensor cs, int64_t k, double random_amount, const c10::optional<at::Tensor> &groups,
+                                       const c10::optional<at::Tensor> &static_mask) {
+    return topk_mask_bits_impl(cs, k, random_amount, groups, static_mask);
+}
+
+std::vector<at::Tensor> topk_mask_bits_varlen(at::Tensor cs, at::Tensor k_lens, int64_t k, double random_amount,
+                                              const c10::optional<at::Tensor> &groups, const c10::optional<at::Tensor> &static_mask) {
+    return topk_mask_bits_impl(cs, k, random_amount, groups, static_mask, k_lens);
 }
 
 static at::Tensor topk_mask_impl(at::Tensor cs, int64_t k, bool mass, double top_p, int64_t k_min, double random_amount,
@@ -1253,6 +1353,11 @@
     m.def("dense_colsum_topk_mask_p_varlen(Tensor q, Tensor k, Tensor v, Tensor p, Tensor k_lens, int k_top, float top_p, int k_min, float random_amount, Tensor? groups, Tensor? static_mask, bool token_major_o=False) -> Tensor[]");
     m.def("compact_indices(Tensor indices, Tensor counts) -> Tensor[]");
     m.def("mask_to_ragged_indices(Tensor mask, int[] shape, int multiple_of, int pad_to_multiple_of, bool sorted) -> Tensor[]");
+    m.def("topk_mask_bits(Tensor cs, int k, float random_amount, Tensor? groups, Tensor? static_mask) -> Tensor[]");
+    m.def("topk_mask_bits_varlen(Tensor cs, Tensor k_lens, int k, float random_amount, Tensor? groups, Tensor? static_mask) -> Tensor[]");
+    m.def("dense_colsum_topk_bits(Tensor q, Tensor k, Tensor v, Tensor p, int k_top, float random_amount, Tensor? groups, Tensor? static_mask, bool token_major_o=False) -> Tensor[]");
+    m.def("dense_colsum_topk_bits_varlen(Tensor q, Tensor k, Tensor v, Tensor p, Tensor k_lens, int k_top, float random_amount, Tensor? groups, Tensor? static_mask, bool token_major_o=False) -> Tensor[]");
+    m.def("mask_to_ragged_indices_counted(Tensor mask, Tensor row_counts, int[] shape, int multiple_of, int pad_to_multiple_of, bool sorted) -> Tensor[]");
     m.def("csp_attn_out_ragged(Tensor q, Tensor k, Tensor v, Tensor o_in, Tensor indices, Tensor offsets, Tensor indices_counts, int o_scale) -> Tensor");
     m.def("residual_ln_modulate(Tensor x, Tensor? y, Tensor? gate, Tensor shift, Tensor scale, float eps) -> Tensor[]");
     m.def("transpose_last2(Tensor x) -> Tensor");
@@ -1310,6 +1415,11 @@
     m.impl("packed_mask_to_indices", &packed_mask_to_indices);
     m.impl("mask_to_sorted_indices", &mask_to_sorted_indices);
     m.impl("mask_to_ragged_indices", &mask_to_ragged_indices);
+    m.impl("topk_mask_bits", &topk_mask_bits);
+    m.impl("topk_mask_bits_varlen", &topk_mask_bits_varlen);
+    m.impl("dense_colsum_topk_bits", &dense_colsum_topk_bits);
+    m.impl("dense_colsum_topk_bits_varlen", &dense_colsum_topk_bits_varlen);
+    m.impl("mask_to_ragged_indices_counted", &mask_to_ragged_indices_counted);
     m.impl("topk_mask", &topk_mask);
     m.impl("topk_mask_p", &topk_mask_p);
     m.impl("transpose_last2", &transpose_last2);
diff --git a/chipmunk_amd/modules/attn.py b/chipmunk_amd/modules/attn.py
--- a/chipmunk_amd/modules/attn.py
+++ b/chipmunk_amd/modules/attn.py
@@ -169,10 +169,11 @@
                     and amd_key("attn", "fused_packed_mask_to_indices") and amd_key("attn", "ragged_mask_to_indices"))
 
     @torch.compiler.disable
-    def _ragged_indices(self, packed: Tensor, shape, multiple_of: int, bm: int, mask: Optional[Tensor] = None):
+    def _ragged_indices(self, packed: Tensor, shape, multiple_of: int, bm: int, mask: Optional[Tensor] = None,
+                        row_counts: Optional[Tensor] = None):
         if shape[-1] % 8 != 0:
             packed = mask if mask is not None else ops.bitunpack(packed, shape)
-        return ops.mask_to_ragged_indices(packed, shape, multiple_of, bm, bool(amd_key("attn", "sorted_indices")))
+        return ops.mask_to_ragged_indices(packed, shape, multiple_of, bm, bool(amd_key("attn", "sorted_indices")), row_counts)
 
     def _stored_indices(self, multiple_of: int, bm: int):
         cfg = GLOBAL_CONFIG["attn"]
@@ -211,11 +212,15 @@
                 prev_lse = self.storage.get_lse_constants()
                 tk = int(multiple_of * round((cfg["top_keys"] * k.shape[-2]) / multiple_of))
                 top_p, k_min = self._top_p(k.shape[-2], multiple_of)
-                mask = bs = None
+                mask = bs = packed = row_counts = None
                 if (q.is_cuda and cfg["should_compress_indices"] and tk > 0 and amd_key("attn", "fused_colsum_topk")
                         and amd_key("attn", "fused_topk_mask") and k.shape[-2] <= ops.TOPK_MASK_MAX_N):
                     static, groups = self._static(q.shape[1], _cdiv(q.shape[-2], bm), k.shape[-2])
-                    if top_p > 0.0:
+                    if (amd_key("attn", "packed_selection") and use_ragged and top_p == 0.0 and k.shape[-2] % 8 == 0
+                            and k.shape[-2] <= ops.TOPK_MASK_BITS_MAX_N):
+                        o, packed, row_counts, lse = ops.dense_colsum_topk_bits(q, k, v, prev_lse, tk, 0.01, groups, static, tm, k_lens)
+                        mask_shape = torch.Size((q.shape[0], q.shape[1], _cdiv(q.shape[-2], bm), k.shape[-2]))
+                    elif top_p > 0.0:
                         o, mask, lse = ops.dense_colsum_topk_mask_p(q, k, v, prev_lse, tk, top_p, k_min, 0.01, groups, static, tm, k_lens)
                     else:
                         o, mask, lse = ops.dense_colsum_topk_mask(q, k, v, prev_lse, tk, 0.01, groups, static, tm, k_lens)
@@ -229,7 +234,7 @@
                 lse[..., k.shape[-2]:, :] = 0
                 self.storage.set_lse_constants(lse)
                 if cfg["should_compress_indices"]:
-                    if mask is not None:
+                    if mask is not None or packed is not None:
                         pass
                     elif tk > 0:
                         mask = self.random_and_topk(bs, tk, top_p, k_min, k_lens)
@@ -237,11 +242,12 @@
                         mask = self._static(bs.shape[1], bs.shape[-2], bs.shape[-1])[0]
                         if k_lens is not None:
                             mask = mask & _valid_keys(k_lens, mask.shape[-1])
-                    packed, mask_shape = ops.bitpack(mask)
+                    if packed is None:
+                        packed, mask_shape = ops.bitpack(mask)
                     self.mask_shape[self.layer_counter.cur_model_invocation_per_step] = mask_shape
                     self.storage.set_indices(packed)
                     if use_ragged:
-                        ragged = self._ragged_indices(packed, mask_shape, multiple_of, bm, mask)
+                        ragged = self._ragged_indices(packed, mask_shape, multiple_of, bm, mask, row_counts)
                         ragged = (ragged[0], ragged[1], _cap_counts(ragged[2], k_lens))
                         self._remember_indices(None, ragged[2], ragged[:2])
                     else:
diff --git a/chipmunk_amd/ops/__init__.py b/chipmunk_amd/ops/__init__.py
--- a/chipmunk_amd/ops/__init__.py
+++ b/chipmunk_amd/ops/__init__.py
@@ -3,8 +3,8 @@
 from .mlp import run_e2e_glu_fp8 as mlp_glu_fp8, run_e2e_glu_fp8, mm1_glu_fp8
 from .indexed_io import (copy_indices, topk_indices, mask_to_indices, scatter_add, packed_mask_to_indices,
                          mask_to_sorted_indices, mask_to_ragged_indices, topk_mask, topk_mask_p, topk_indices_p, topk_delta_indices_p, manual_seed,
-                         TOPK_MASK_MAX_N)
-from .attn import compact_indices, csp_attn, csp_attn_inplace, csp_attn_out, csp_attn_out_ragged, dense_attn, dense_colsum_attn, dense_colsum_topk_mask, dense_colsum_topk_mask_p
+                         TOPK_MASK_MAX_N, TOPK_MASK_BITS_MAX_N, topk_mask_bits)
+from .attn import compact_indices, csp_attn, csp_attn_inplace, csp_attn_out, csp_attn_out_ragged, dense_attn, dense_colsum_attn, dense_colsum_topk_mask, dense_colsum_topk_mask_p, dense_colsum_topk_bits
 from .patch import patchify, unpatchify, patchify_rope
 from .bitpack import bitpack, bitunpack
 from . import voxel
@@ -15,6 +15,6 @@
            "packed_mask_to_indices", "mask_to_sorted_indices", "csp_attn_inplace", "csp_attn_out", "topk_mask", "TOPK_MASK_MAX_N", "voxel", "manual_seed", "qkv_split_norm", "dense_colsum_topk_mask", "compact_indices", "csp_attn_out_ragged", "residual_ln_modulate",
            "split_heads_rownorm", "wan_rope_table", "mask_to_ragged_indices", "mlp_glu", "run_e2e_glu", "mm1_glu",
            "mlp_glu_fp8", "run_e2e_glu_fp8", "mm1_glu_fp8", "topk_mask_p", "dense_colsum_topk_mask_p",
-           "topk_indices_p", "topk_delta_indices_p"]
+           "topk_indices_p", "topk_delta_indices_p", "topk_mask_bits", "dense_colsum_topk_bits", "TOPK_MASK_BITS_MAX_N"]
 
 from . import _fake
diff --git a/chipmunk_amd/ops/_fake.py b/chipmunk_amd/ops/_fake.py
--- a/chipmunk_amd/ops/_fake.py
+++ b/chipmunk_amd/ops/_fake.py
@@ -140,6 +140,31 @@
     def _(q, k, v, p, k_lens, k_top, top_p, k_min, random_amount, groups, static_mask, token_major_o=False):
         G = (q.shape[2] + 191) // 192
         return [_o_like(q, token_major_o), q.new_empty((q.shape[0], q.shape[1], G, k.shape[2]), dtype=torch.bool), _dense_out(q)]
+
+    def _bits_out(ref, B, H, G, n):
+        return [ref.new_empty((B * H * G * n // 8,), dtype=torch.uint8), ref.new_empty((B, H, G), dtype=torch.int32)]
+
+    @lib.register_fake("chipmunk::topk_mask_bits")
+    def _(cs, k, random_amount, groups, static_mask):
+        torch._check(cs.ndim == 4 and cs.shape[-1] % 8 == 0, lambda: "cs must be [B, H, G, N] with N a multiple of 8")
+        return _bits_out(cs, *cs.shape)
+
+    @lib.register_fake("chipmunk::topk_mask_bits_varlen")
+    def _(cs, k_lens, k, random_amount, groups, static_mask):
+        torch._check(cs.ndim == 4 and cs.shape[-1] % 8 == 0, lambda: "cs must be [B, H, G, N] with N a multiple of 8")
+        return _bits_out(cs, *cs.shape)
+
+    @lib.register_fake("chipmunk::dense_colsum_topk_bits")
+    def _(q, k, v, p, k_top, random_amount, groups, static_mask, token_major_o=False):
+        torch._check(k.shape[2] % 8 == 0, lambda: "the key count must be a multiple of 8")
+        packed, row_counts = _bits_out(q, q.shape[0], q.shape[1], (q.shape[2] + 191) // 192, k.shape[2])
+        return [_o_like(q, token_major_o), packed, row_counts, _dense_out(q)]
+
+    @lib.register_fake("chipmunk::dense_colsum_topk_bits_varlen")
+    def _(q, k, v, p, k_lens, k_top, random_amount, groups, static_mask, token_major_o=False):
+        torch._check(k.shape[2] % 8 == 0, lambda: "the key count must be a multiple of 8")
+        packed, row_counts = _bits_out(q, q.shape[0], q.shape[1], (q.shape[2] + 191) // 192, k.shape[2])
+        return [_o_like(q, token_major_o), packed, row_counts, _dense_out(q)]
 
     @lib.register_fake("chipmunk::topk_indices_p")
     def _(activation, indices, counts, sparsity_amount, top_p, min_keys, multiple_of, random_amount):
diff --git a/chipmunk_amd/ops/attn.py b/chipmunk_amd/ops/attn.py
--- a/chipmunk_amd/ops/attn.py
+++ b/chipmunk_amd/ops/attn.py
@@ -86,6 +86,25 @@
     return o, mask, l
 
 
+def dense_colsum_topk_bits(q: torch.Tensor, k: torch.Tensor, v: torch.Tensor, p: torch.Tensor, k_top: int, random_amount: float,
+                           groups, static_mask, token_major_o: bool = False, k_lens: Optional[torch.Tensor] = None
+                           ) -> Tuple[torch.Tensor, torch.Tensor, torch.Tensor, torch.Tensor]:
+    n = q.shape[-2]
+    padded = _pad_len(n)
+    assert p.shape[-2] in (n, padded), "p must be the l vector of the previous full step"
+    if check_k_lens(k_lens, q, "dense_colsum_topk_bits") is not None:
+        o, packed, row_counts, l = torch.ops.chipmunk.dense_colsum_topk_bits_varlen(
+            _last_dim_contiguous(q), _last_dim_contiguous(k), _last_dim_contiguous(v), p[..., :n, :].contiguous(), k_lens, k_top, random_amount,
+            groups, static_mask, token_major_o)
+    else:
+        o, packed, row_counts, l = torch.ops.chipmunk.dense_colsum_topk_bits(
+            _last_dim_contiguous(q), _last_dim_contiguous(k), _last_dim_contiguous(v), p[..., :n, :].contiguous(), k_top, random_amount, groups,
+            static_mask, token_major_o)
+    if padded != n:
+        l = F.pad(l, (0, 0, 0, padded - n))
+    return o, packed, row_counts, l
+
+
 def dense_colsum_topk_mask_p(q: torch.Tensor, k: torch.Tensor, v: torch.Tensor, p: torch.Tensor, k_top: int, top_p: float, k_min: int,
                              random_amount: float, groups, static_mask, token_major_o: bool = False,
                              k_lens: Optional[torch.Tensor] = None) -> Tuple[torch.Tensor, torch.Tensor, torch.Tensor]:
@@ -136,4 +155,4 @@
 
 
 __all__ = ["csp_attn", "csp_attn_inplace", "csp_attn_out", "csp_attn_out_ragged", "compact_indices", "dense_attn", "dense_colsum_attn",
-           "dense_colsum_topk_mask", "dense_colsum_topk_mask_p"]
+           "dense_colsum_topk_mask", "dense_colsum_topk_mask_p", "dense_colsum_topk_bits"]
diff --git a/chipmunk_amd/ops/indexed_io.py b/chipmunk_amd/ops/indexed_io.py
--- a/chipmunk_amd/ops/indexed_io.py
+++ b/chipmunk_amd/ops/indexed_io.py
@@ -1,10 +1,11 @@
 from __future__ import annotations
 
-from typing import List, Optional, Sequence
+from typing import List, Optional, Sequence, Tuple
 
 import torch
 
 TOPK_MASK_MAX_N = 1024 * 512
+TOPK_MASK_BITS_MAX_N = 1024 * 120
 
 
 def copy_indices(bm_fc1: torch.Tensor, bm_mid_cache: torch.Tensor, indices: torch.Tensor, counts: torch.Tensor) -> None:
@@ -101,8 +102,10 @@
 
 
 def mask_to_ragged_indices(mask: torch.Tensor, shape: Sequence[int], multiple_of: int, pad_to_multiple_of: int,
-                           sorted: bool = True) -> List[torch.Tensor]:
+                           sorted: bool = True, row_counts: Optional[torch.Tensor] = None) -> List[torch.Tensor]:
     if mask.is_cuda:
+        if row_counts is not None:
+            return torch.ops.chipmunk.mask_to_ragged_indices_counted(mask, row_counts, list(shape), multiple_of, pad_to_multiple_of, sorted)
         return torch.ops.chipmunk.mask_to_ragged_indices(mask, list(shape), multiple_of, pad_to_multiple_of, sorted)
     if mask.dtype == torch.uint8:
         from .bitpack import bitunpack
@@ -110,7 +113,7 @@
     b, h, m, n = mask.shape
     pad_n = (n + pad_to_multiple_of - 1) // pad_to_multiple_of * pad_to_multiple_of
     rows = mask.reshape(-1, n) != 0
-    kept = rows.sum(dim=1)
+    kept = rows.sum(dim=1) if row_counts is None else row_counts.reshape(-1).to(torch.int64)
     counts = (kept + multiple_of - 1) // multiple_of * multiple_of
     lengths = (counts.clamp(max=pad_n) + 31) // 32 * 32
     offsets = torch.zeros(rows.shape[0] + 1, dtype=torch.int64)
@@ -132,6 +135,16 @@
     if check_k_lens(k_lens, cs, "topk_mask") is not None:
         return torch.ops.chipmunk.topk_mask_varlen(cs, k_lens, k, random_amount, groups, static_mask)
     return torch.ops.chipmunk.topk_mask(cs, k, random_amount, groups, static_mask)
+
+
+def topk_mask_bits(cs: torch.Tensor, k: int, random_amount: float = 0.0, groups: Optional[torch.Tensor] = None,
+                   static_mask: Optional[torch.Tensor] = None, k_lens: Optional[torch.Tensor] = None) -> Tuple[torch.Tensor, torch.Tensor]:
+    from .attn import check_k_lens
+    if check_k_lens(k_lens, cs, "topk_mask_bits") is not None:
+        packed, row_counts = torch.ops.chipmunk.topk_mask_bits_varlen(cs, k_lens, k, random_amount, groups, static_mask)
+    else:
+        packed, row_counts = torch.ops.chipmunk.topk_mask_bits(cs, k, random_amount, groups, static_mask)
+    return packed, row_counts
 
 
 def _bf16_keys(cs: torch.Tensor) -> torch.Tensor:
diff --git a/chipmunk_amd/util/config.py b/chipmunk_amd/util/config.py
--- a/chipmunk_amd/util/config.py
+++ b/chipmunk_amd/util/config.py
@@ -81,6 +81,7 @@
     "attn.keep_unpacked_indices_offloaded": True,
     "attn.kept_indices_offloaded_budget_gb": 8.0,
     "attn.ragged_mask_to_indices": True,
+    "attn.packed_selection": True,
     "mlp.fp8_fc2": False,
     "attn.top_p": 0.0,
     "attn.top_p_min_keys": 0.0,
diff --git a/include/chipmunk_hip.h b/include/chipmunk_hip.h
--- a/include/chipmunk_hip.h
+++ b/include/chipmunk_hip.h
@@ -227,6 +227,25 @@
                                 int static_rows, const void *group_flags, void *mask, const int32_t *k_lens, int seq_rows,
                                 int rows, int n, int k, double random_amount, double top_p, int k_min, void *stream);
 
+int chipmunk_topk_mask_bits(const void *cs, int64_t cs_stride, const void *static_mask, int64_t static_stride, int static_rows,
+                            const void *group_flags, void *packed, int32_t *row_counts, int rows, int n, int k, double random_amount,
+                            void *stream);
+int chipmunk_topk_mask_bits_varlen(const void *cs, int64_t cs_stride, const void *static_mask, int64_t static_stride, int static_rows,
+                                   const void *group_flags, void *packed, int32_t *row_counts, const int32_t *k_lens, int seq_rows,
+                                   int rows, int n, int k, double random_amount, void *stream);
+int chipmunk_dense_colsum_topk_bits_strided(const void *q, const void *k, const void *v, const int64_t q_strides[3],
+                                            const int64_t k_strides[3], const int64_t v_strides[3], const float *p, void *o,
+                                            const int64_t *o_strides, float *l, int B, int H, int Nq, int Nk, const void *static_mask,
+                                            int64_t static_stride, int static_rows, const void *group_flags, void *packed,
+                                            int32_t *row_counts, int k_top, double random_amount, void *stream);
+int chipmunk_dense_colsum_topk_bits_varlen(const void *q, const void *k, const void *v, const int64_t q_strides[3],
+                                           const int64_t k_strides[3], const int64_t v_strides[3], const float *p, void *o,
+                                           const int64_t *o_strides, float *l, const int32_t *k_lens, int B, int H, int Nq, int Nk,
+                                           const void *static_mask, int64_t static_stride, int static_rows, const void *group_flags,
+                                           void *packed, int32_t *row_counts, int k_top, double random_amount, void *stream);
+int chipmunk_row_counts_to_lengths(const int32_t *row_counts, int32_t *counts, int64_t *lengths, int64_t rows, int n, int pad_n,
+                                   int multiple_of, void *stream);
+
 int chipmunk_mask_to_indices(const void *mask, int32_t *indices, int32_t *counts, int64_t rows, int n, int pad_n,
                              int multiple_of, void *stream);
 
```

Result: no change. 0.5844 (-0.0%).
